# soham97/mellow

Hardware: AMD Instinct MI355X
Metric: audio-pair responses/sec (v0 167M, 2x10s clips, max_len=64, greedy) (higher is better)
Workload: dtype f32 (encoder/prefill GEMM operands split EXACTLY into 3 bf16 terms, 6 bf16 MFMA products per fp32 product, f32 accumulate: fp32-accurate, parity suite green; mel included, the STFT is an fp32 FFT; attentions and decode on exact fp32 MFMA / VALU)

## Files before the change

mellow_amd/csrc/beam.hip:

```cpp
#include "common.h"
#include "kernels.h"

namespace mellow {

namespace {

constexpr int BM_THREADS = 1024, BM_WAVES = BM_THREADS / 64;
constexpr int BM_NV4 = SAMPLE_MAX_V / 4 / BM_THREADS;
static_assert(BM_NV4 * 4 * BM_THREADS == SAMPLE_MAX_V, "row tiling");
static_assert(BEAM_MAX_K * BEAM_MAX_K <= 64, "one wave ranks an example's survivors");

__device__ __forceinline__ int64_t f32_idx(int rb, int K8, int m, int k) {
    return ((int64_t)rb * K8 + (k >> 3)) * 64 + m + 32 * ((k >> 2) & 1);
}

__device__ __forceinline__ uint32_t ckey(float c) {
    if (c != c) return 0xFFFFFFFFu;
    const uint32_t u = __float_as_uint(c);
    return (u & 0x80000000u) ? ~u : (u | 0x80000000u);
}

__device__ __forceinline__ float opaque(float x) {
    asm volatile("" : "+v"(x));
    return x;
}

template <typename T, typename Op>
__device__ __forceinline__ T block_reduce(T v, Op op, T* red) {
    const int tid = threadIdx.x;
#pragma unroll
    for (int off = 32; off > 0; off >>= 1) v = op(v, __shfl_xor(v, off, 64));
    if ((tid & 63) == 0) red[tid >> 6] = v;
    __syncthreads();
    T r = red[0];
    for (int w = 1; w < BM_WAVES; ++w) r = op(r, red[w]);
    __syncthreads();
    return r;
}

__global__ __launch_bounds__(BM_THREADS) void beam_rows_kernel(const BeamArgs g, const int32_t* __restrict__ params) {
    __shared__ float red_f[BM_WAVES];
    __shared__ unsigned long long red_u[BM_WAVES];
    const int r = blockIdx.x, tid = threadIdx.x;
    const float cum = g.cum_in[r];
    float* cc = g.cand_c + (int64_t)r * BEAM_MAX_K;
    float* cl = g.cand_lp + (int64_t)r * BEAM_MAX_K;
    int32_t* ct = g.cand_tok + (int64_t)r * BEAM_MAX_K;
    if (g.fin_in[r] != 0) {
        if (tid == 0) {
            g.cand_n[r] = 1;
            cc[0] = cum + 0.0f; ct[0] = params ? params[1] : g.stop_id; cl[0] = 0.f;
        }
        return;
    }
    const float* __restrict__ lrow = g.logits + (int64_t)r * g.ld;
    float l[BM_NV4][4];
    float m = -INFINITY;
#pragma unroll
    for (int k = 0; k < BM_NV4; ++k) {
        const float4 v = reinterpret_cast<const float4*>(lrow)[k * BM_THREADS + tid];
        l[k][0] = v.x; l[k][1] = v.y; l[k][2] = v.z; l[k][3] = v.w;
#pragma unroll
        for (int j = 0; j < 4; ++j) m = fmaxf(m, l[k][j]);
    }
    const float M = block_reduce(m, [](float a, float b) { return fmaxf(a, b); }, red_f);
    float s = 0.f;
#pragma unroll
    for (int k = 0; k < BM_NV4; ++k)
#pragma unroll
        for (int j = 0; j < 4; ++j) s += expf(l[k][j] - M);
    const float S = block_reduce(s, [](float a, float b) { return a + b; }, red_f);
    const float lse = (M - M == 0.f) ? M + (float)log((double)S) : __builtin_nanf("");
    unsigned long long prev = ~0ull;
    if (tid == 0) g.cand_n[r] = g.k;
#pragma unroll 1
    for (int jr = 0; jr < g.k; ++jr) {
        const uint32_t pkey = (uint32_t)(prev >> 32), pinv = (uint32_t)prev;
        uint32_t bkey = 0u, binv = 0u;
#pragma unroll
        for (int k = 0; k < BM_NV4; ++k)
#pragma unroll
            for (int j = 0; j < 4; ++j) {
                const uint32_t key = ckey(cum + (opaque(l[k][j]) - lse) + 0.0f);
                const uint32_t inv = (uint32_t)(0x7fffffff - (4 * (k * BM_THREADS + tid) + j));
                if ((key < pkey || (key == pkey && inv < pinv)) && (key > bkey || (key == bkey && inv > binv))) { bkey = key; binv = inv; }
            }
        unsigned long long best = ((unsigned long long)bkey << 32) | binv;
        best = block_reduce(best, [](unsigned long long a, unsigned long long b) { return a > b ? a : b; }, red_u);
        if (tid == 0) {
            int idx = 0x7fffffff - (int)(uint32_t)(best & 0xffffffffull);
            idx = min(max(idx, 0), SAMPLE_MAX_V - 1);
            const float lp = lrow[idx] - lse;
            cc[jr] = cum + lp + 0.0f; ct[jr] = idx; cl[jr] = lp;
        }
        prev = best;
    }
}

template <bool LOOP>
__global__ __launch_bounds__(64) void beam_merge_kernel(const BeamArgs g, const DecArgs a, int32_t* __restrict__ tokens,
                                                        const float* __restrict__ embed, const LoopArgs lp) {
    __shared__ int sel_par[BEAM_MAX_K], sel_tok[BEAM_MAX_K];
    __shared__ float sel_c[BEAM_MAX_K], sel_lp[BEAM_MAX_K];
    const int b = blockIdx.x, lane = threadIdx.x, k = g.k;
    const int par = lane / k, slot = lane - par * k;
    bool valid = false;
    float c = 0.f, inc = 0.f;
    int tok = 0;
    if (par < k) {
        const int row = b * k + par;
        valid = slot < g.cand_n[row];
        if (valid) {
            c = g.cand_c[(int64_t)row * BEAM_MAX_K + slot];
            tok = g.cand_tok[(int64_t)row * BEAM_MAX_K + slot];
            inc = g.cand_lp[(int64_t)row * BEAM_MAX_K + slot];
        }
    }
    const uint32_t key = ckey(c);
    int rank = 0;
    for (int t = 0; t < k * k; ++t) {
        const uint32_t ok = __shfl(key, t, 64);
        const int ot = __shfl(tok, t, 64), ov = __shfl((int)valid, t, 64), op = t / k;
        const bool before = ok > key || (ok == key && (op < par || (op == par && ot < tok)));
        rank += (ov && before) ? 1 : 0;
    }
    if (valid && rank < k) { sel_par[rank] = par; sel_tok[rank] = tok; sel_c[rank] = c; sel_lp[rank] = inc; }
    __syncthreads();
    if constexpr (!LOOP) {
        if (lane < k) {
            const int row = b * k + lane;
            g.out_parent[row] = sel_par[lane]; g.out_token[row] = sel_tok[lane]; g.out_cum[row] = sel_c[lane]; g.out_lp[row] = sel_lp[lane];
        }
        return;
    } else {
        const int max_len = lp.params[0], stop_id = lp.params[1];
        const int step = *a.d_pos - lp.T0 + 1;
        int fin = 0;
        if (lane < k) {
            const int row = b * k + lane;
            fin = sel_tok[lane] == stop_id ? 1 : 0;
            g.cum_state[row] = sel_c[lane];
            g.fin_state[row] = fin;
            tokens[row] = min(max(sel_tok[lane], 0), SAMPLE_MAX_V - 1);
            if (step >= 0 && step < max_len) {
                const int64_t o = (int64_t)step * g.N + row;
                g.out_parent[o] = sel_par[lane]; g.out_token[o] = sel_tok[lane]; g.out_lp[o] = sel_lp[lane]; g.out_cum[o] = sel_c[lane];
            }
        }
        const int nfin = __popcll(__ballot(fin));
        if (lane == 0) {
            if (nfin) atomicAdd(lp.n_seen, nfin);
            asm volatile("s_waitcnt vmcnt(0)" ::: "memory");
            if (atomicAdd(lp.arrive, 1) == (int)gridDim.x - 1) {
                *lp.arrive = 0;
                const int t = *lp.ticket + 1;
                *lp.ticket = t;
                const int ns = atomicExch(lp.n_seen, 0);
                __hip_atomic_store(lp.host_progress, ((unsigned long long)(unsigned)t << 32) | (unsigned)ns, __ATOMIC_RELAXED,
                                   __HIP_MEMORY_SCOPE_SYSTEM);
            }
        }
        for (int j = 0; j < k; ++j) {
            const int row = b * k + j, t = min(max(sel_tok[j], 0), SAMPLE_MAX_V - 1);
            for (int i = lane; i < 144; i += 64) {
                const float4 e = reinterpret_cast<const float4*>(embed + (int64_t)t * 576)[i];
                reinterpret_cast<float4*>(a.xmidF)[f32_idx(row >> 5, 72, row & 31, i * 4)] = e;
            }
        }
    }
}

template <bool GATHER>
__global__ __launch_bounds__(256) void beam_kv_move_kernel(float4* __restrict__ kpages, float4* __restrict__ vpages, float4* __restrict__ kst,
                                                           float4* __restrict__ vst, const int32_t* __restrict__ parent_tab,
                                                           const int32_t* __restrict__ d_pos, const int32_t* __restrict__ params, int T0,
                                                           int layers, int N, int k, int Bp, int Tmax) {
    const int max_len = params[0], step = *d_pos - T0 + 1;
    if (step <= 0 || step >= max_len || T0 + step > Tmax) return;
    const int64_t c16 = (int64_t)step * 16, ML16 = (int64_t)max_len * 16, Tmax16 = (int64_t)Tmax * 16;
    const int64_t total = (int64_t)layers * N * 3 * c16;
    const int32_t* __restrict__ par = parent_tab + (int64_t)step * N;
    for (int64_t i = (int64_t)blockIdx.x * 256 + threadIdx.x; i < total; i += (int64_t)gridDim.x * 256) {
        const int64_t pg = i / c16, q = i - pg * c16;
        const int64_t lr = pg / 3, h = pg - lr * 3, l = lr / N;
        const int r = (int)(lr - l * N);
        const int pr = r / k * k + min(max(par[r], 0), k - 1);
        if (pr == r) continue;
        const int64_t st = pg * ML16 + q;
        if constexpr (GATHER) {
            const int64_t src = ((l * Bp + pr) * 3 + h) * Tmax16 + (int64_t)T0 * 16 + q;
            kst[st] = kpages[src];
            vst[st] = vpages[src];
        } else {
            const int64_t dst = ((l * Bp + r) * 3 + h) * Tmax16 + (int64_t)T0 * 16 + q;
            kpages[dst] = kst[st];
            vpages[dst] = vst[st];
        }
    }
}

}

void launch_beam_select(const BeamArgs& g, int B, const DecArgs& a, int32_t* tokens, const float* embed, const LoopArgs* loop, hipStream_t s) {
    if (B <= 0 || g.k < 1 || g.k > BEAM_MAX_K || g.ld != SAMPLE_MAX_V) return;
    hipLaunchKernelGGL(beam_rows_kernel, dim3(B * g.k), dim3(BM_THREADS), 0, s, g, loop ? loop->params : nullptr);
    if (loop) hipLaunchKernelGGL(beam_merge_kernel<true>, dim3(B), dim3(64), 0, s, g, a, tokens, embed, *loop);
    else hipLaunchKernelGGL(beam_merge_kernel<false>, dim3(B), dim3(64), 0, s, g, a, tokens, embed, LoopArgs());
}

void launch_beam_reorder(float* k_pages, float* v_pages, float* k_stage, float* v_stage, const int32_t* parent_tab, const int32_t* d_pos,
                         const int32_t* params, int T0, int layers, int N, int k, int Bp, int Tmax, hipStream_t s) {
    if (layers <= 0 || N <= 0 || k < 2 || N % k != 0 || N > Bp) return;
    constexpr int blocks = 1024;
    hipLaunchKernelGGL(beam_kv_move_kernel<true>, dim3(blocks), dim3(256), 0, s, reinterpret_cast<float4*>(k_pages), reinterpret_cast<float4*>(v_pages),
                       reinterpret_cast<float4*>(k_stage), reinterpret_cast<float4*>(v_stage), parent_tab, d_pos, params, T0, layers, N, k, Bp, Tmax);
    hipLaunchKernelGGL(beam_kv_move_kernel<false>, dim3(blocks), dim3(256), 0, s, reinterpret_cast<float4*>(k_pages), reinterpret_cast<float4*>(v_pages),
                       reinterpret_cast<float4*>(k_stage), reinterpret_cast<float4*>(v_stage), parent_tab, d_pos, params, T0, layers, N, k, Bp, Tmax);
}

}
```

mellow_amd/csrc/build.py:

```python
#!/usr/bin/env python3
from __future__ import annotations

import argparse
import concurrent.futures as cf
import os
import subprocess
import sys

HERE = os.path.dirname(os.path.abspath(__file__))
PKG = os.path.dirname(HERE)
LIBDIR = os.path.join(PKG, "lib")
OBJDIR = os.path.join(HERE, "build")
LIB = os.path.join(LIBDIR, "libmellow_hip.so")
SOURCES = ["gemm_f32.hip", "gemm_fp8.hip", "gemm_bf16x3.hip", "decode.hip", "prefill_attn.hip", "encoder.hip", "stft_fft.hip", "sample.hip", "score.hip", "beam.hip", "logit_rules.hip", "guidance.hip", "engine.cpp", "engine_weights.cpp", "engine_encoder.cpp", "engine_lm.cpp", "engine_generate.cpp", "engine_dev.cpp"]
HEADERS = ["common.h", "kernels.h", "gemm_epilogue.h", "prefill_attn_f32.inc", "engine_internal.h", os.path.join("..", "..", "include", "mellow_hip.h")]
ARCH = "gfx950"
FLAGS = (["-DMELLOW_KDEBUG"] if os.environ.get("MELLOW_KDEBUG") else []) + os.environ.get("MELLOW_EXTRA_FLAGS", "").split() + ["-O3", "-std=c++17", "-fPIC", "-fvisibility=hidden", f"--offload-arch={ARCH}", "-Wall", "-Wno-unused-function",
         "-Wno-unused-variable", "-x", "hip"]


def _hipcc():
    for c in (os.environ.get("HIPCC"), "/opt/rocm/bin/hipcc", "hipcc"):
        if c and (os.path.isabs(c) and os.path.exists(c) or not os.path.isabs(c)):
            return c
    raise RuntimeError("hipcc not found")


def _stale(target, deps):
    if not os.path.exists(target):
        return True
    t = os.path.getmtime(target)
    return any(os.path.getmtime(d) > t for d in deps)


VGPR_FORM = ["-mllvm", "-amdgpu-mfma-vgpr-form=1"]
FILE_FLAGS = {name: VGPR_FORM for name in os.environ.get("MELLOW_VGPR_FORM_FILES", "gemm_bf16x3.hip gemm_fp8.hip prefill_attn.hip encoder.hip").split()}
KERNARG_PRELOAD = [] if os.environ.get("MELLOW_KERNARG_PRELOAD", "14") == "0" else ["-mllvm", "-amdgpu-kernarg-preload-count=" + os.environ.get("MELLOW_KERNARG_PRELOAD", "14")]
FILE_FLAGS["decode.hip"] = FILE_FLAGS.get("decode.hip", []) + KERNARG_PRELOAD


def build(force=False, verbose=False, out=None, objdir=None):
    lib = os.path.abspath(out) if out else LIB
    objdir = os.path.abspath(objdir) if objdir else OBJDIR
    os.makedirs(os.path.dirname(lib), exist_ok=True)
    os.makedirs(objdir, exist_ok=True)
    hipcc = _hipcc()
    hdrs = [os.path.join(HERE, h) for h in HEADERS] + [os.path.abspath(__file__)]
    jobs = []
    objs = []
    for src in SOURCES:
        sp = os.path.join(HERE, src)
        op = os.path.join(objdir, src + ".o")
        objs.append(op)
        if force or _stale(op, [sp] + hdrs):
            jobs.append((sp, op))

    def cc(job):
        sp, op = job
        cmd = [hipcc] + FLAGS + FILE_FLAGS.get(os.path.basename(sp), []) + ["-c", sp, "-o", op]
        if verbose:
            print(" ".join(cmd), flush=True)
        r = subprocess.run(cmd, capture_output=True, text=True)
        return sp, r

    with cf.ThreadPoolExecutor(max_workers=max(1, min(len(jobs), os.cpu_count() or 1))) as ex:
        for sp, r in ex.map(cc, jobs):
            if r.returncode != 0:
                sys.stderr.write(r.stdout + r.stderr)
                raise RuntimeError(f"hipcc failed on {sp}")
            if verbose and r.stderr.strip():
                sys.stderr.write(r.stderr)
    if force or jobs or _stale(lib, objs):
        cmd = [hipcc, "-shared", "-fPIC", f"--offload-arch={ARCH}", "-o", lib] + objs
        if verbose:
            print(" ".join(cmd), flush=True)
        r = subprocess.run(cmd, capture_output=True, text=True)
        if r.returncode != 0:
            sys.stderr.write(r.stdout + r.stderr)
            raise RuntimeError("link failed")
    return lib


if __name__ == "__main__":
    ap = argparse.ArgumentParser()
    ap.add_argument("--force", action="store_true")
    ap.add_argument("--verbose", action="store_true")
    ap.add_argument("--out", metavar="PATH", help="write the library here instead of mellow_amd/lib/libmellow_hip.so")
    ap.add_argument("--objdir", metavar="DIR", help="object cache of this build instead of mellow_amd/csrc/build/")
    a = ap.parse_args()
    print(build(a.force, a.verbose, a.out, a.objdir))
```

mellow_amd/csrc/decode.hip:

```cpp
#include "common.h"
#include "kernels.h"
#include <cstdio>
#include <mutex>
#include <set>
#include <type_traits>
#include <utility>

namespace mellow {

__device__ uint64_t* g_kdbg = nullptr;
#ifdef MELLOW_KDEBUG
__device__ __forceinline__ void kstamp(int slot, int idx, bool who) {
    if (g_kdbg && who) g_kdbg[slot * 8 + idx] = __builtin_readcyclecounter();
}
__device__ __forceinline__ void kspan(int seq, int end) {
    if (g_kdbg && seq >= 0 && seq < 480 && threadIdx.x == 0) {
        const unsigned long long t = wall_clock64();
        if (end) atomicMax(reinterpret_cast<unsigned long long*>(g_kdbg) + 64 + 2 * seq + 1, t);
        else atomicMin(reinterpret_cast<unsigned long long*>(g_kdbg) + 64 + 2 * seq, t);
    }
}
#else
#define kstamp(slot, idx, who) ((void)0)
#define kspan(seq, end) ((void)0)
#endif
void set_kernel_debug_buffer(uint64_t* p) { (void)hipMemcpyToSymbol(HIP_SYMBOL(g_kdbg), &p, sizeof(p)); }

__device__ __forceinline__ float fast_exp(float x) { return __builtin_amdgcn_exp2f(x * 1.44269504088896340736f); }
#ifdef MELLOW_NO_BLK_EXIT
#define MELLOW_BLK_EXIT(RB)
#else
#define MELLOW_BLK_EXIT(RB) if (BLK) { if (a.blk_live[RB] == 0) return; }
#endif
__device__ __forceinline__ float4 ldg_nt(const float4* p) {
#ifdef MELLOW_NO_NT
    return *p;
#else
    const f32x4 v = __builtin_nontemporal_load(reinterpret_cast<const f32x4*>(p));
    return make_float4(v[0], v[1], v[2], v[3]);
#endif
}
template <bool W8>
__device__ __forceinline__ float4 ldw(const float* __restrict__ Wp, int64_t slot) {
    if constexpr (W8) {
        const uint32_t u = __builtin_nontemporal_load(reinterpret_cast<const uint32_t*>(Wp) + slot);
        const auto lo = __builtin_amdgcn_cvt_pk_f32_fp8(u, false), hi = __builtin_amdgcn_cvt_pk_f32_fp8(u, true);
        return make_float4(lo[0], lo[1], hi[0], hi[1]);
    } else {
        return ldg_nt(reinterpret_cast<const float4*>(Wp) + slot);
    }
}
__device__ __forceinline__ uint32_t ldw8(const float* __restrict__ Wp, int64_t slot) {
    return __builtin_nontemporal_load(reinterpret_cast<const uint32_t*>(Wp) + slot);
}
__device__ __forceinline__ float f4amax(float4 v) { return fmaxf(fmaxf(fabsf(v.x), fabsf(v.y)), fmaxf(fabsf(v.z), fabsf(v.w))); }
__device__ __forceinline__ uint32_t q4_e4m3(float4 v, float inv) {
    int w = 0;
    w = __builtin_amdgcn_cvt_pk_fp8_f32(v.x * inv, v.y * inv, w, false);
    w = __builtin_amdgcn_cvt_pk_fp8_f32(v.z * inv, v.w * inv, w, true);
    return (uint32_t)w;
}
__device__ __forceinline__ long pk64(uint32_t lo, uint32_t hi) { return (long)(((uint64_t)hi << 32) | (uint64_t)lo); }
template <int N>
__device__ __forceinline__ f32x16 mfma8_32(f32x16 acc, const uint32_t (&w)[N], const uint32_t (&x)[N]) {
#pragma unroll
    for (int i = 0; i < N; i += 2)
        acc = __builtin_amdgcn_mfma_f32_32x32x16_fp8_fp8(pk64(w[i], i + 1 < N ? w[i + 1] : 0u), pk64(x[i], i + 1 < N ? x[i + 1] : 0u), acc, 0, 0, 0);
    return acc;
}
template <int N>
__device__ __forceinline__ f32x4 mfma8_16(f32x4 acc, const uint32_t (&w)[N], const uint32_t (&x)[N]) {
#pragma unroll
    for (int i = 0; i < N; i += 2)
        acc = __builtin_amdgcn_mfma_f32_16x16x32_fp8_fp8(pk64(w[i], i + 1 < N ? w[i + 1] : 0u), pk64(x[i], i + 1 < N ? x[i + 1] : 0u), acc, 0, 0, 0);
    return acc;
}
__device__ __forceinline__ void a8_scales(float amax, float& inv, float& sc) {
    inv = amax > 0.f ? 448.0f / amax : 0.f;
    sc = amax * (1.0f / 448.0f);
}
#ifndef MELLOW_ST_MODE
#define MELLOW_ST_MODE 0
#endif
__device__ __forceinline__ void st_out(float4* p, float4 v) {
// ... 149 lines not shown
        }
        if (nt == 0) {
            ssp = half_sum(ssp);
            if (lane < 32) ssq_s[wave * 32 + lane] = ssp;
        }
#pragma unroll
        for (int r = 0; r < 16; ++r) red[(wave * 16 + r) * 64 + lane] = acc[r];
    }
    __syncthreads();
    if (nt == 0 && tid < 32)
    {
        float ssum = ssq_s[tid & 31];
#pragma unroll
        for (int wv = 1; wv < QW; ++wv) ssum += ssq_s[wv * 32 + (tid & 31)];
        a.ssq1[((int64_t)rb * 32 + tid) * DEC_KC_QKV + kc] = ssum;
    }
    if (tid >= 256) return;
    const int mm = tid & 31, hh = (tid >> 5) & 1, gq = tid >> 6;
    float v[4];
#pragma unroll
    for (int j = 0; j < 4; ++j) {
        const int r = 4 * gq + j;
        float sacc = red[r * 64 + mm + 32 * hh];
#pragma unroll
        for (int wv = 1; wv < QW; ++wv) sacc += red[(wv * 16 + r) * 64 + mm + 32 * hh];
        v[j] = sacc;
    }
    const int n = nt * 32 + 8 * gq + 4 * hh;
    if (W8) {
#pragma unroll
        for (int j = 0; j < 4; ++j) v[j] *= wscale[n + j];
    }
    if (n < 960)
        *reinterpret_cast<float4*>(a.pq + ((int64_t)kc * a.rows + rb * 32 + mm) * 960 + n) = make_float4(v[0], v[1], v[2], v[3]);
    kspan(a.dbg_seq, 1);
}

#ifndef MELLOW_DA_ABL
#define MELLOW_DA_ABL 0
#endif
#ifndef MELLOW_DA_WAVES
#define MELLOW_DA_WAVES 8
#define MELLOW_DA_G 7
#endif
#ifndef MELLOW_DA_MINW
#define MELLOW_DA_MINW 4
#endif
constexpr int DA_MINW = MELLOW_DA_WAVES == 8 || MELLOW_DA_WAVES == 4 ? MELLOW_DA_MINW : 1;
constexpr int DA_WAVES = MELLOW_DA_WAVES;
constexpr int DA_G = MELLOW_DA_G;
#ifndef MELLOW_DA_G1
#define MELLOW_DA_G1 5
#endif
constexpr int DA_G1 = MELLOW_DA_G1 < DA_G ? MELLOW_DA_G1 : DA_G;
#ifndef MELLOW_DA16_MFMA
#define MELLOW_DA16_MFMA 1
#endif
constexpr int DA_GM = 8;
#ifndef MELLOW_DA16_KNT
#define MELLOW_DA16_KNT 0
#endif
#ifndef MELLOW_DA16_MINW
#define MELLOW_DA16_MINW MELLOW_DA_MINW
#endif
#ifndef MELLOW_DA16_NW
#define MELLOW_DA16_NW 8
#endif

template <bool KV16>
__device__ __forceinline__ float4 ld_kv(const float* page, int64_t elem) {
    if constexpr (KV16) {
        typedef unsigned u32x2 __attribute__((ext_vector_type(2)));
        const u32x2 r = __builtin_nontemporal_load(reinterpret_cast<const u32x2*>(reinterpret_cast<const uint16_t*>(page) + elem));
        return make_float4(__uint_as_float(r[0] << 16), __uint_as_float(r[0] & 0xffff0000u), __uint_as_float(r[1] << 16), __uint_as_float(r[1] & 0xffff0000u));
    } else {
        return ldg_nt(reinterpret_cast<const float4*>(page + elem));
    }
}
template <bool KV16>
__device__ __forceinline__ void st_kv(float* page, int64_t elem, float v) {
    if constexpr (KV16) reinterpret_cast<__bf16*>(page)[elem] = static_cast<__bf16>(v);
    else page[elem] = v;
}
template <bool BLK, bool FUSED, bool ONE, bool KV16, int NW, int TS>
__global__ __launch_bounds__(NW * 64, ONE ? 2 : (KV16 && MELLOW_DA16_MFMA && DA_MINW > 1 ? MELLOW_DA16_MINW : DA_MINW)) void dec_attn_kernel(float* __restrict__ k_cache, float* __restrict__ v_cache,
                                                                  const int32_t* __restrict__ d_pos_p, const float* __restrict__ pq_p,
                                                                  const float* __restrict__ xmidF_p, int Tmax_p, int gs_p, int rows_p,
                                                                  const DecArgs a) {
    kspan(a.dbg_seq, 0);
    __shared__ float ssq_part[3];
    __shared__ __attribute__((aligned(16))) float qs[3 * 64];
    __shared__ __attribute__((aligned(16))) float knew[64], vnew[64];
    __shared__ __attribute__((aligned(16))) float xs[320];
    __shared__ __attribute__((aligned(16))) float ored[DA_WAVES * 3 * 64];
    __shared__ float mred[DA_WAVES * 3], lred[DA_WAVES * 3];
    __shared__ float snew_s[3];
    constexpr bool MF = KV16 && MELLOW_DA16_MFMA != 0;
    __shared__ __attribute__((aligned(16))) float pl[MF ? DA_WAVES * 32 * 4 : 4];
    __shared__ __attribute__((aligned(16))) __bf16 qb[MF ? 10 * 64 : 8];
    constexpr int VPW = DA_WAVES / NW;
    static_assert(DA_WAVES % NW == 0 && (MF || NW == DA_WAVES), "the vector form runs one chunk stream per wave");
    auto mf_group = [&](int g0, int u) { return g0 + u * DA_WAVES; };

    static_assert(TS == DEC_TS || !(ONE || KV16), "one row block and the bf16 pages always run DEC_TS key splits (kernels.h dec_key_splits)");
    const int g = blockIdx.x, b = blockIdx.y, sp = blockIdx.z;
    int row = b;
    if (BLK) {
        const int live = a.blk_live[b >> 5];
        if (a.row_of_slot) row = a.row_of_slot[b];
        if (live == 0 || row < 0) return;
    }
    const int tid = threadIdx.x, lane = tid & 63, wave = tid >> 6;
    const int Tmax = Tmax_p;
    float* kpage = k_cache + (((int64_t)row * 3 + g) * Tmax * 64 >> (KV16 ? 1 : 0));
    float* vpage = v_cache + (((int64_t)row * 3 + g) * Tmax * 64 >> (KV16 ? 1 : 0));
    const int sub = lane >> 4, quad = lane & 15;

    const bool dbg = tid == 0 && g == 0 && b == 0 && sp == 0;
    kstamp(1, 0, dbg);
#ifdef MELLOW_POS_VECTOR_LOAD
    const int pos = __builtin_amdgcn_readfirstlane(*reinterpret_cast<const volatile int*>(d_pos_p));
#else
    const int pos = *d_pos_p;
#endif
    const int hsel = (tid >> 5) & 3, i = tid & 31;
    const int r = tid < 80 ? tid : 0;
    const int pcol = r < 48 ? (3 * g + (r >> 4)) * 64 + 4 * (r & 15) : r < 64 ? 576 + g * 64 + 4 * (r - 48) : 768 + g * 64 + 4 * (r - 64);
    const float* prow = pq_p + (int64_t)b * 960 + pcol;
    constexpr int NPQ = FUSED ? Q2_NPQ : DEC_KC_QKV;
    float4 sl4[NPQ], sq4[2];
    if (tid < 80) {
#pragma unroll
        for (int s = 0; s < NPQ; ++s)
            sl4[s] = (MELLOW_DA_ABL & 4) ? make_float4(0.1f * s, 0.2f, 0.3f, 0.4f) : *reinterpret_cast<const float4*>(prow + (int64_t)s * rows_p * 960);
        if (!FUSED) {
            sq4[0] = reinterpret_cast<const float4*>(a.ssq1 + (int64_t)b * DEC_KC_QKV)[0];
            sq4[1] = reinterpret_cast<const float4*>(a.ssq1 + (int64_t)b * DEC_KC_QKV)[1];
        }
    }
    float4 xr4 = make_float4(0.f, 0.f, 0.f, 0.f), xd4[FUSED ? Q2_HC : 1];
    if (FUSED && tid < 144) {
        const int64_t fi = ((int64_t)(b >> 5) * 72 + (tid >> 1)) * 64 + (b & 31) + 32 * (tid & 1);
        xr4 = reinterpret_cast<const float4*>(xmidF_p)[fi];
#pragma unroll
        for (int s = 0; s < Q2_HC; ++s) xd4[s] = reinterpret_cast<const float4*>(a.dslabF)[(int64_t)s * a.slabF_stride4 + fi];
    }
    const float c = a.rope_cur[i], sn = a.rope_cur[32 + i];
    const int gbeg = sp * gs_p;
    const int gend_fixed = sp == TS - 1 ? 0x3fffffff : gbeg + gs_p;
    typedef unsigned u32x2 __attribute__((ext_vector_type(2)));
    const int kk = lane & 31, hf = lane >> 5;
    i32x4 kq[4];
    u32x2 vq[DA_GM];
    auto load_ktile = [&](int g0) {
        const int gi = g0 + (kk >> 2) * DA_WAVES;
        const int tc = min(gi * 4 + (kk & 3), Tmax - 1);
        const i32x4* kp = reinterpret_cast<const i32x4*>(reinterpret_cast<const uint16_t*>(kpage) + (int64_t)tc * 64 + hf * 32);
#pragma unroll
        for (int st = 0; st < 4; ++st)
            kq[st] = (MELLOW_DA_ABL & 1) ? i32x4{tc, 0x3c003c00, st, 0x3c003c00} : (MELLOW_DA16_KNT ? __builtin_nontemporal_load(kp + st) : kp[st]);
    };
    auto load_vgroup = [&](int g0, int u) {
        const int gi = mf_group(g0, u);
        const int tc = min(gi * 4 + sub, Tmax - 1);
        vq[u] = (MELLOW_DA_ABL & 1) ? u32x2{0x3c003c00u, (unsigned)tc}
                                    : __builtin_nontemporal_load(reinterpret_cast<const u32x2*>(reinterpret_cast<const uint16_t*>(vpage) + (int64_t)tc * 64 + quad * 4));
    };
    float4 k4[MF ? 1 : DA_G], v4[MF ? 1 : DA_G];
    auto load_group = [&](int u) {
        const int gi = gbeg + wave + u * DA_WAVES;
        const int tc = min(gi * 4 + sub, Tmax - 1);
        if (MELLOW_DA_ABL & 1) {
            k4[u] = make_float4(0.01f * tc, 0.02f, 0.03f, 0.04f);
            v4[u] = make_float4(0.01f, 0.02f * tc, 0.03f, 0.04f);
        } else {
            k4[u] = ld_kv<KV16>(kpage, (int64_t)tc * 64 + quad * 4);
            v4[u] = ld_kv<KV16>(vpage, (int64_t)tc * 64 + quad * 4);
        }
    };
    const int g_first_mf = gbeg + wave;
    if constexpr (MF) {
        load_ktile(g_first_mf);
#pragma unroll
        for (int u = 0; u < DA_GM / 2; ++u) load_vgroup(g_first_mf, u);
    } else {
#pragma unroll
        for (int u = 0; u < DA_G1; ++u) load_group(u);
    }
    MELLOW_HOIST(a.attF16); MELLOW_HOIST(a.att_ml); MELLOW_HOIST(a.RB); MELLOW_HOIST(a.eps);
    if (FUSED) MELLOW_HOIST(a.xnewR);
    __builtin_amdgcn_sched_barrier(0);
    kstamp(1, 1, dbg);

    const int ngroups = (pos + 3) >> 2;
    const int gend = min(ngroups, gend_fixed);
    static_assert(DEC_KC_QKV == 8, "fixed summation order below");
    if (FUSED) {
        if (tid < 192) {
            float4 x = xr4;
#pragma unroll
            for (int s = 0; s < Q2_HC; ++s) x = f4add(x, xd4[s]);
            const float ss = wave_sum(tid < 144 ? f4ssq(x) : 0.f);
            if (lane == 0) ssq_part[wave] = ss;
            if (g == 0 && sp == 0 && tid < 144) reinterpret_cast<float4*>(a.xnewR + (int64_t)b * 576)[tid] = x;
        }
        if (tid < 80) {
            float4 x = sl4[0];
#pragma unroll
            for (int s = 1; s < NPQ; ++s) x = f4add(x, sl4[s]);
            *reinterpret_cast<float4*>(xs + 4 * tid) = x;
        }
    } else if (tid < 80) {
        float4 x = sl4[0];
#pragma unroll
        for (int s = 1; s < DEC_KC_QKV; ++s) x = f4add(x, sl4[s]);
        const float ssum = ((sq4[0].x + sq4[0].y) + (sq4[0].z + sq4[0].w)) + ((sq4[1].x + sq4[1].y) + (sq4[1].z + sq4[1].w));
        const float rscale = 1.0f / sqrtf(ssum / 576.0f + a.eps);
        *reinterpret_cast<float4*>(xs + 4 * tid) = make_float4(x.x * rscale, x.y * rscale, x.z * rscale, x.w * rscale);
    }
    __syncthreads();
    kstamp(1, 2, dbg);
    const float rs2 = FUSED ? 1.0f / sqrtf(((ssq_part[0] + ssq_part[1]) + ssq_part[2]) / 576.0f + a.eps) : 1.0f;
    if (tid < 128) {
        const int base = hsel < 3 ? hsel * 64 : 192;
        const float x1 = xs[base + i] * rs2, x2 = xs[base + i + 32] * rs2;
        const float o1 = __fadd_rn(__fmul_rn(x1, c), __fmul_rn(-x2, sn));
        const float o2 = __fadd_rn(__fmul_rn(x2, c), __fmul_rn(x1, sn));
        if (hsel < 3) {
            qs[hsel * 64 + i] = o1 * 0.125f;
            qs[hsel * 64 + i + 32] = o2 * 0.125f;
            if constexpr (MF) {
                __bf16 p0, p1, p2;
                split3(o1 * 0.125f, p0, p1, p2);
                qb[(0 * 3 + hsel) * 64 + i] = p0; qb[(1 * 3 + hsel) * 64 + i] = p1; qb[(2 * 3 + hsel) * 64 + i] = p2;
                split3(o2 * 0.125f, p0, p1, p2);
                qb[(0 * 3 + hsel) * 64 + i + 32] = p0; qb[(1 * 3 + hsel) * 64 + i + 32] = p1; qb[(2 * 3 + hsel) * 64 + i + 32] = p2;
            }
        } else {
            knew[i] = o1; knew[i + 32] = o2;
            if (sp == 0) { st_kv<KV16>(kpage, (int64_t)pos * 64 + i, o1); st_kv<KV16>(kpage, (int64_t)pos * 64 + i + 32, o2); }
        }
    } else if (tid < 192) {
        const float x1 = xs[256 + tid - 128] * rs2;
        vnew[tid - 128] = x1;
        if (sp == 0) st_kv<KV16>(vpage, (int64_t)pos * 64 + (tid - 128), x1);
    } else if (MF && tid < 256) {
        qb[9 * 64 + tid - 192] = static_cast<__bf16>(0.f);
    }
    __syncthreads();
    __builtin_amdgcn_sched_barrier(0);
    if constexpr (MF) {
#pragma unroll
        for (int u = DA_GM / 2; u < DA_GM; ++u) load_vgroup(g_first_mf, u);
    } else {
#pragma unroll
        for (int u = DA_G1; u < DA_G; ++u) load_group(u);
    }
    __builtin_amdgcn_sched_barrier(0);
    kstamp(1, 3, dbg);

    if (wave < 3) {
        const float sn_ = wave_sum(qs[wave * 64 + lane] * knew[lane]);
        if (lane == 0) snew_s[wave] = sn_;
    }
    float4 q4[3];
    const int aq_off = ((kk >> 2) < 3 && (kk & 3) < 3 ? (kk >> 2) * 3 + (kk & 3) : 9) * 64 + hf * 32;
    if constexpr (!MF) {
#pragma unroll
        for (int hh = 0; hh < 3; ++hh) q4[hh] = *reinterpret_cast<const float4*>(qs + hh * 64 + quad * 4);
    }
    float m_run[3] = {-INFINITY, -INFINITY, -INFINITY};
    float l_run[3] = {0.f, 0.f, 0.f};
    float4 acc[3];
#pragma unroll
    for (int hh = 0; hh < 3; ++hh) acc[hh] = make_float4(0.f, 0.f, 0.f, 0.f);

#define MELLOW_DA_CHUNK(g0)                                                                                              \
    {                                                                                                                    \
        float sc[DA_G][3];                                                                                               \
        float cmax[3] = {-INFINITY, -INFINITY, -INFINITY};                                                               \
_Pragma("unroll")                                                                                                        \
        for (int u = 0; u < DA_G; ++u) {                                                                                 \
            const int gi = g0 + u * DA_WAVES;                                                                            \
            const int t = gi * 4 + sub;                                                                                  \
            const bool ok = gi < gend && t < pos;                                                                        \
_Pragma("unroll")                                                                                                        \
            for (int hh = 0; hh < 3; ++hh) {                                                                             \
                float sv = q4[hh].x * k4[u].x + q4[hh].y * k4[u].y + q4[hh].z * k4[u].z + q4[hh].w * k4[u].w;            \
                sv = row16_sum(sv);                                                                                      \
                sv = ok ? sv : -INFINITY;                                                                                \
                sc[u][hh] = sv;                                                                                          \
                cmax[hh] = fmaxf(cmax[hh], sv);                                                                          \
            }                                                                                                            \
        }                                                                                                                \
_Pragma("unroll")                                                                                                        \
        for (int hh = 0; hh < 3; ++hh) {                                                                                 \
            float cm = cmax[hh];                                                                                         \
            cm = fmaxf(cm, swz_xor16(cm));                                                                               \
            cm = half_max(cm);                                                                                           \
// ... 1111 lines not shown
        kstamp(7, 2, dbg && acc[0] == acc[0]);
        if (side) nt -= 30;
    }
#pragma unroll
    for (int r = 0; r < 16; ++r) red[(wave * 16 + r) * 64 + lane] = acc[r];
    __syncthreads();
    kstamp(7, 3, dbg);
    if (tid < 256) {
        const int mm = tid & 31, hh = (tid >> 5) & 1, gq = tid >> 6;
        float v[4];
#pragma unroll
        for (int j = 0; j < 4; ++j) {
            const int q = 4 * gq + j;
            float sacc = red[q * 64 + mm + 32 * hh];
#pragma unroll
            for (int wv = 1; wv < Q2W; ++wv) sacc += red[(wv * 16 + q) * 64 + mm + 32 * hh];
            v[j] = sacc;
        }
        const int n = nt * 32 + 8 * gq + 4 * hh;
        if (W8) {
#pragma unroll
            for (int j = 0; j < 4; ++j) v[j] *= wsc[n + j];
        }
        const float4 o = make_float4(v[0], v[1], v[2], v[3]);
        if (side) st_out(reinterpret_cast<float4*>(a.dslabF) + (int64_t)slab * a.slabF_stride4 + f32_idx(rb, 72, mm, n), o);
        else st_out(reinterpret_cast<float4*>(a.pq + ((int64_t)slab * a.rows + rb * 32 + mm) * 960 + n), o);
    }
    kstamp(7, 4, dbg);
    kspan(a.dbg_seq, 1);
}

template <int KCD, bool BLK>
__global__ __launch_bounds__(192) void dec_final_norm_kernel(const float* __restrict__ norm_w, const float* __restrict__ xmidF_p,
                                                             const float* __restrict__ dslabF_p, int64_t stride4_p, const DecArgs a) {
    kspan(a.dbg_seq, 0);
    __shared__ float part[3];
    const int b = blockIdx.x, tid = threadIdx.x;
    if (BLK && b == 0 && tid < 32) a.blk_snap[tid] = a.blk_live[tid];
    MELLOW_BLK_EXIT(b >> 5)
    const int xi = tid < 144 ? tid : 0;
    const int64_t fi = f32_idx(b >> 5, 72, b & 31, xi * 4);
    float4 v = reinterpret_cast<const float4*>(xmidF_p)[fi];
    float4 xs[KCD > 0 ? KCD : 1];
#pragma unroll
    for (int s = 0; s < KCD; ++s) xs[s] = reinterpret_cast<const float4*>(dslabF_p)[(int64_t)s * stride4_p + fi];
    const float4 wv = reinterpret_cast<const float4*>(norm_w)[xi];
#pragma unroll
    for (int s = 0; s < KCD; ++s) v = f4add(v, xs[s]);
    float ss = tid < 144 ? f4ssq(v) : 0.f;
    ss = wave_sum(ss);
    if ((tid & 63) == 0) part[tid >> 6] = ss;
    __syncthreads();
    const float r = 1.0f / sqrtf((part[0] + part[1] + part[2]) / 576.0f + a.eps);
    if (tid < 144) {
        float4 y;
        y.x = __fmul_rn(wv.x, __fmul_rn(v.x, r)); y.y = __fmul_rn(wv.y, __fmul_rn(v.y, r));
        y.z = __fmul_rn(wv.z, __fmul_rn(v.z, r)); y.w = __fmul_rn(wv.w, __fmul_rn(v.w, r));
        if (!a.xn3) reinterpret_cast<float4*>(a.xnF)[fi] = y;
    }
    if (a.xn3) {
        float4 y = make_float4(0.f, 0.f, 0.f, 0.f);
        if (tid < 144) {
            y.x = __fmul_rn(wv.x, __fmul_rn(v.x, r)); y.y = __fmul_rn(wv.y, __fmul_rn(v.y, r));
            y.z = __fmul_rn(wv.z, __fmul_rn(v.z, r)); y.w = __fmul_rn(wv.w, __fmul_rn(v.w, r));
        }
        const F3Quad mine = f3_split4(y), other = f3_partner(mine);
        if (tid < 144 && !(tid & 1)) f3_store8(a.xn3, f3_32_slot(b >> 5, 36, b & 31, tid * 4), mine, other);
    }
    kspan(a.dbg_seq, 1);
}

template <bool LSE>
__global__ __launch_bounds__(256) void dec_argmax_kernel(const float* __restrict__ cand_val_p, const int32_t* __restrict__ cand_idx_p, int n,
                                                         const DecArgs a, int32_t* __restrict__ tokens,
                                                         const float* __restrict__ embed, int write_x, const LoopArgs lp) {
    kspan(a.dbg_seq, 0);
    __shared__ float bv[4];
    __shared__ int bi[4];
    __shared__ int tok_s;
    __shared__ float lse_sh[4];
    const int b = blockIdx.x, tid = threadIdx.x;
    const int row = lp.row_of_slot ? lp.row_of_slot[b] : b;
    const bool dead = (lp.blk_snap && lp.blk_snap[b >> 5] == 0) || row < 0;
    float best = -INFINITY;
    int idx = 0x7fffffff;
    if (!dead) {
        for (int i = tid; i < n; i += 256) {
            const float v = cand_val_p[(int64_t)b * n + i];
            const int id = cand_idx_p[(int64_t)b * n + i];
            if (arg_better(v, id, best, idx)) { best = v; idx = id; }
        }
#pragma unroll
        for (int off = 32; off > 0; off >>= 1) {
            const float ov = __shfl_xor(best, off, 64);
            const int oi = __shfl_xor(idx, off, 64);
            if (arg_better(ov, oi, best, idx)) { best = ov; idx = oi; }
        }
        if ((tid & 63) == 0) { bv[tid >> 6] = best; bi[tid >> 6] = idx; }
    }
    __syncthreads();
    float S = 0.f;
    if constexpr (LSE) {
        if (!dead) {
            float M = bv[0];
            int mi = bi[0];
            for (int w = 1; w < 4; ++w)
                if (arg_better(bv[w], bi[w], M, mi)) { M = bv[w]; mi = bi[w]; }
            S = dec_lse_sum(cand_val_p + (int64_t)b * n, a.cand_sum + (int64_t)b * n, n, M, lse_sh);
            S = (M - M == 0.f) ? S : __builtin_nanf("");
        }
    }
    if (tid == 0) {
        if (!dead) {
            for (int w = 1; w < 4; ++w)
                if (arg_better(bv[w], bi[w], best, idx)) { best = bv[w]; idx = bi[w]; }
            idx = min(max(idx, 0), n * 32 - 1);
            tokens[b] = idx;
            tok_s = idx;
        }
        if (lp.out_tokens) {
            if (!dead) {
                const int max_len = lp.params[0], stop_id = lp.params[1];
                const int step = *a.d_pos - lp.T0 + 1;
                if (step >= 0 && step < max_len) lp.out_tokens[(int64_t)row * max_len + step] = idx;
                if constexpr (LSE) {
                    if (step >= 0 && step < max_len) lp.out_logprob[(int64_t)row * max_len + step] = -dec_lse_log(S);
                }
                if (idx == stop_id && lp.seen_stop[row] == 0) {
                    lp.seen_stop[row] = 1;
                    atomicAdd(lp.n_seen, 1);
                    if (lp.blk_left && atomicSub(lp.blk_left + (b >> 5), 1) == 1) lp.blk_live[b >> 5] = 0;
                }
            }
            asm volatile("s_waitcnt vmcnt(0)" ::: "memory");
            if (atomicAdd(lp.arrive, 1) == (int)gridDim.x - 1) {
                *lp.arrive = 0;
                const int t = *lp.ticket + 1;
                *lp.ticket = t;
                const int ns = atomicAdd(lp.n_seen, 0);
                __hip_atomic_store(lp.host_progress, ((unsigned long long)(unsigned)t << 32) | (unsigned)ns, __ATOMIC_RELAXED,
                                   __HIP_MEMORY_SCOPE_SYSTEM);
            }
        }
    }
    if (dead) return;
    if (write_x) {
        __syncthreads();
        if (tid < 144) {
            const float4 e = reinterpret_cast<const float4*>(embed + (int64_t)tok_s * 576)[tid];
            reinterpret_cast<float4*>(a.xmidF)[f32_idx(b >> 5, 72, b & 31, tid * 4)] = e;
        }
    }
    kspan(a.dbg_seq, 1);
}

__global__ __launch_bounds__(256) void dec_lse_tap_kernel(const float* __restrict__ cand_val_p, const float* __restrict__ cand_sum_p, int n,
                                                          float* __restrict__ out_lse, float* __restrict__ out_max) {
    __shared__ float sh[4];
    const int b = blockIdx.x;
    const float M = dec_lse_max(cand_val_p + (int64_t)b * n, n, sh);
    const float S = dec_lse_sum(cand_val_p + (int64_t)b * n, cand_sum_p + (int64_t)b * n, n, M, sh);
    if (threadIdx.x == 0) {
        out_lse[b] = dec_lse_value(M, S);
        out_max[b] = M;
    }
}

__global__ __launch_bounds__(1024) void dec_compact_kernel(const DecArgs a, int B, const LoopArgs lp) {
    __shared__ int src_of[1024];
    __shared__ int row_new[1024];
    __shared__ int wsum[16];
    __shared__ int n_act_s, n_live_s;
    const int tid = threadIdx.x, lane = tid & 63, wave = tid >> 6;
    const int nblk = (B + 31) >> 5;
    int row = -1, active = 0;
    if (tid < B) {
        row = lp.row_of_slot[tid];
        active = row >= 0 && lp.blk_live[tid >> 5] != 0 && lp.seen_stop[row] == 0;
    }
    const unsigned long long m = __ballot(active);
    const int before = __popcll(m & ((1ull << lane) - 1ull));
    if (lane == 0) wsum[wave] = __popcll(m);
    if (tid == 0) {
        int live = 0;
        for (int k = 0; k < nblk; ++k) live += lp.blk_live[k] != 0;
        n_live_s = live;
    }
    src_of[tid] = -1;
    row_new[tid] = -1;
    __syncthreads();
    int base = 0;
    for (int w = 0; w < wave; ++w) base += wsum[w];
    if (tid == 0) {
        int n = 0;
        for (int w = 0; w < 16; ++w) n += wsum[w];
        n_act_s = n;
    }
    __syncthreads();
    const int n_act = n_act_s;
    if ((n_act + 31) / 32 >= n_live_s) return;
    if (active) { src_of[base + before] = tid; row_new[base + before] = row; }
    __syncthreads();
    float4* x = reinterpret_cast<float4*>(a.xmidF);
    for (int d0 = 0; d0 < n_act; d0 += 7) {
        const int d = d0 + tid / 144, c = tid % 144;
        const bool mv = tid < 1008 && d < n_act && src_of[d] != d;
        float4 v = make_float4(0.f, 0.f, 0.f, 0.f);
        if (mv) v = x[f32_idx(src_of[d] >> 5, 72, src_of[d] & 31, c * 4)];
        __syncthreads();
        if (mv) x[f32_idx(d >> 5, 72, d & 31, c * 4)] = v;
        __syncthreads();
    }
    if (tid < B) lp.row_of_slot[tid] = row_new[tid];
    if (tid < 32) {
        const int left = tid < nblk ? min(max(n_act - 32 * tid, 0), 32) : 0;
        lp.blk_left[tid] = left;
        lp.blk_live[tid] = left > 0;
    }
    if (tid == 0) *lp.n_compactions += 1;
}
__global__ __launch_bounds__(256) void kv_to_bf16_kernel(const float4* __restrict__ src, uint4* __restrict__ dst, int64_t n8) {
    for (int64_t i = (int64_t)blockIdx.x * 256 + threadIdx.x; i < n8; i += (int64_t)gridDim.x * 256) {
        const float4 a = src[2 * i], b = src[2 * i + 1];
        typedef __bf16 bf16x8v __attribute__((ext_vector_type(8)));
        const bf16x8v o = {static_cast<__bf16>(a.x), static_cast<__bf16>(a.y), static_cast<__bf16>(a.z), static_cast<__bf16>(a.w),
                           static_cast<__bf16>(b.x), static_cast<__bf16>(b.y), static_cast<__bf16>(b.z), static_cast<__bf16>(b.w)};
        dst[i] = __builtin_bit_cast(uint4, o);
    }
}
void launch_kv_to_bf16(const float* src, void* dst, int64_t n, hipStream_t s) {
    const int64_t n8 = n >> 3;
    const int blocks = (int)((n8 + 255) / 256 < 8192 ? (n8 + 255) / 256 : 8192);
    hipLaunchKernelGGL(kv_to_bf16_kernel, dim3(blocks), dim3(256), 0, s, reinterpret_cast<const float4*>(src), reinterpret_cast<uint4*>(dst), n8);
}
__global__ __launch_bounds__(256) void kv_fanout_kernel(const float4* __restrict__ ksrc, const float4* __restrict__ vsrc,
                                                        float4* __restrict__ kdst, float4* __restrict__ vdst, int64_t total,
                                                        int B, int n, int Bp, int T16, int64_t Tp16, int64_t Tmax16) {
    for (int64_t i = (int64_t)blockIdx.x * 256 + threadIdx.x; i < total; i += (int64_t)gridDim.x * 256) {
        const int64_t pg = i / T16, q = i - pg * T16;
        const int64_t lb = pg / 3, h = pg - lb * 3, l = lb / B, b = lb - l * B;
        const float4 k = ksrc[pg * Tp16 + q], v = vsrc[pg * Tp16 + q];
        int64_t d = ((l * Bp + b * n) * 3 + h) * Tmax16 + q;
        for (int j = 0; j < n; ++j, d += 3 * Tmax16) {
            kdst[d] = k;
            vdst[d] = v;
        }
    }
}
void launch_kv_fanout(const float* k_prefix, const float* v_prefix, float* k_pages, float* v_pages, int layers, int B, int n, int Bp,
                      int T, int Tp, int Tmax, hipStream_t s) {
    if (layers <= 0 || B <= 0 || n <= 0 || T <= 0 || T > Tp || T > Tmax || (int64_t)B * n > Bp) return;
    const int64_t total = (int64_t)layers * B * 3 * T * 16;
    const int blocks = (int)((total + 255) / 256 < 2048 ? (total + 255) / 256 : 2048);
    hipLaunchKernelGGL(kv_fanout_kernel, dim3(blocks), dim3(256), 0, s, reinterpret_cast<const float4*>(k_prefix),
                       reinterpret_cast<const float4*>(v_prefix), reinterpret_cast<float4*>(k_pages), reinterpret_cast<float4*>(v_pages),
                       total, B, n, Bp, T * 16, (int64_t)Tp * 16, (int64_t)Tmax * 16);
}
void launch_dec_compact(const DecArgs& a, int B, const LoopArgs& loop, hipStream_t s) {
    hipLaunchKernelGGL(dec_compact_kernel, dim3(1), dim3(1024), 0, s, a, B, loop);
}

__global__ __launch_bounds__(192) void dec_load_rows_kernel(const DecArgs a, const float* __restrict__ in, int64_t ld,
                                                            const int32_t* __restrict__ row_ids, int T_last, int n_src) {
    const int b = blockIdx.x, tid = threadIdx.x;
    const int64_t src = row_ids ? (int64_t)min(max(row_ids[b], 0), n_src - 1) : (int64_t)b * T_last + (T_last - 1);
    if (tid < 144) {
        const float4 e = reinterpret_cast<const float4*>(in + src * ld)[tid];
        reinterpret_cast<float4*>(a.xmidF)[f32_idx(b >> 5, 72, b & 31, tid * 4)] = e;
    }
}

void set_max_dynamic_lds(const void* fn, size_t bytes) {
    if (bytes <= 64 * 1024) return;
    static std::mutex mu;
    static std::set<std::pair<const void*, int>> done;
    int dev = 0;
    (void)hipGetDevice(&dev);
    std::lock_guard<std::mutex> lk(mu);
    if (done.insert({fn, dev}).second) {
        const hipError_t e = hipFuncSetAttribute(fn, hipFuncAttributeMaxDynamicSharedMemorySize, (int)bytes);
        if (e != hipSuccess) fprintf(stderr, "mellow: hipFuncSetAttribute(max dynamic LDS %zu) failed: %s\n", bytes, hipGetErrorString(e));
    }
}
template <class F> static inline void with_bool(bool v, F&& f) {
    if (v) f(std::true_type{}); else f(std::false_type{});
}
template <int V0, int... Vs, class F> static inline void with_int(int v, F&& f) {
    if constexpr (sizeof...(Vs) == 0) f(std::integral_constant<int, V0>{});
    else if (v == V0) f(std::integral_constant<int, V0>{});
    else with_int<Vs...>(v, f);
}
static inline int w8_mode(const DecArgs& a, const float* wscale) { return wscale ? (a.a8 ? 2 : 1) : 0; }
template <class F> static inline void with_blk_w8(const DecArgs& a, const float* wscale, F&& f) {
    with_bool(a.blk_live != nullptr, [&](auto blk) { with_int<2, 1, 0>(w8_mode(a, wscale), [&](auto w8) { f(blk, w8); }); });
}
void launch_dec_qkv(const DecArgs& a, const float* Wp, int K8p, int kcd, hipStream_t s, const float* wscale) {
    const dim3 grid(30, DEC_KC_QKV, a.RB);
    with_int<0, DEC_KC_DOWN>(kcd, [&](auto kcd_c) { with_bool(a.first != 0, [&](auto first) { with_blk_w8(a, wscale, [&](auto blk, auto w8) {
        hipLaunchKernelGGL((dec_qkv_kernel<kcd_c.value, blk.value, first.value, w8.value>), grid, dim3(QKV_THREADS), 0, s, Wp, (const float*)a.xmidF,
                           (const float*)a.dslabF, K8p, a, wscale);
    }); }); });
}
void launch_dec_attn(const DecArgs& a, float* k_cache, float* v_cache, bool fused, hipStream_t s) {
    const dim3 grid(3, a.rows, a.ts);
    const bool one = a.RB == 1 && !a.blk_live;
    if (a.ts != DEC_TS && (one || a.kv16 || a.ts != DEC_TS_MULTI)) {
        fprintf(stderr, "mellow: decode attention launched with %d key splits at RB = %d\n", a.ts, a.RB);
        abort();
    }
    auto launch = [&](auto blk, auto one_c) { with_bool(fused, [&](auto fused_c) { with_bool(a.kv16 != 0, [&](auto kv16) {
        constexpr bool ONE = one_c.value, KV16 = kv16.value;
        constexpr int NW = !KV16 ? DA_WAVES : MELLOW_DA16_MFMA && DA_WAVES == 8 && !ONE ? MELLOW_DA16_NW : DA_WAVES;
        constexpr int TSM = ONE || KV16 ? DEC_TS : DEC_TS_MULTI;
        with_int<DEC_TS, TSM>(a.ts, [&](auto ts) {
            hipLaunchKernelGGL((dec_attn_kernel<blk.value, fused_c.value, ONE, KV16, NW, ts.value>), grid, dim3(NW * 64), 0, s, k_cache, v_cache,
                               (const int32_t*)a.d_pos, (const float*)a.pq, (const float*)a.xmidF, a.Tmax, a.gs, a.rows, a);
        });
    }); }); };
    if (one) launch(std::false_type{}, std::true_type{});
    else with_bool(a.blk_live != nullptr, [&](auto blk) { launch(blk, std::false_type{}); });
}
static void launch_dec_qkv2_any(const DecArgs& a, const float* Wx, int K8x, const float* Wh, int K8h, const float* Wd,
                                const float* sc_x, const float* sc_h, const float* sc_d, hipStream_t s) {
    const dim3 grid(Q2_BLOCKS, a.RB);
#ifdef MELLOW_Q2_WAVES_FORCED
    bool few = false;
#else
    bool few = a.RB == 1;
#endif
    if (w8_mode(a, sc_x) == 2) few = false;
    with_bool(few, [&](auto few_c) { with_blk_w8(a, sc_x, [&](auto blk, auto w8) {
        constexpr int WV = few_c.value ? 4 : Q2_WAVES;
        hipLaunchKernelGGL((dec_qkv2_kernel<blk.value, WV, w8.value>), grid, dim3(WV * 64), 0, s, Wx, Wh, Wd, (const float*)a.xmidF,
                           (const float*)a.guF, K8x, K8h, a, sc_x, sc_h, sc_d);
    }); });
}
constexpr size_t dec_qkv2x3_lds(int rbm) { return (size_t)Q3W * rbm * 16 * 64 * 4; }
constexpr size_t dec_gateup3_lds(int rbm) { return (size_t)GU3W * rbm * 8 * 64 * 4; }
constexpr size_t dec_head3r_lds() { return (size_t)36 * 3 * 64 * 16; }
template <class F> static inline void with_qkv2x3(int rb, bool blk, F&& f) {
    with_int<1, 2, 4>(rb, [&](auto rbm) { with_bool(blk, [&](auto b) { f(&dec_qkv2x3_kernel<b.value, rbm.value>, dec_qkv2x3_lds(rbm.value)); }); });
}
template <class F> static inline void with_gateup3(int rb, bool blk, F&& f) {
    with_int<1, 2, 4>(rb, [&](auto rbm) { with_bool(blk, [&](auto b) { f(&dec_gateup3_kernel<b.value, rbm.value>, dec_gateup3_lds(rbm.value)); }); });
}
template <class F> static inline void with_head3r(int rb, bool blk, bool lse, F&& f) {
    with_int<1, 2, 4>(rb, [&](auto g) { with_bool(blk, [&](auto b) { with_bool(lse, [&](auto l) {
        constexpr int G = g.value, D = G == 1 ? MELLOW_H3R_D1 : G == 2 ? MELLOW_H3R_D2 : MELLOW_H3R_D4;
        f(&dec_head3r_kernel<G, D, b.value, l.value>, dec_head3r_lds());
    }); }); });
}
void launch_dec_qkv2x3(const DecArgs& a, const float* Wq2, const float* Wd, hipStream_t s) {
    const float* Wh = Wq2 + (size_t)72 * 64 * 4;
    const i32x4 *x3 = reinterpret_cast<const i32x4*>(a.xmid3_32), *h3 = reinterpret_cast<const i32x4*>(a.h3);
    with_qkv2x3(a.RB, a.blk_live != nullptr, [&](auto* kernel, size_t lds) {
        set_max_dynamic_lds(reinterpret_cast<const void*>(kernel), lds);
        hipLaunchKernelGGL(kernel, dim3(Q2_BLOCKS), dim3(Q3W * 64), lds, s, Wq2, Wh, Wd, x3, h3, Q2_K8, Q2_K8, a.RB, a);
    });
}
void launch_dec_gateup3(const DecArgs& a, const float* Wp16, hipStream_t s) {
    const i32x4* x3 = reinterpret_cast<const i32x4*>(a.xmid3_16);
    with_gateup3(a.RB, a.blk_live != nullptr, [&](auto* kernel, size_t lds) {
        set_max_dynamic_lds(reinterpret_cast<const void*>(kernel), lds);
        hipLaunchKernelGGL(kernel, dim3(192), dim3(GU3W * 64), lds, s, Wp16, x3, (const float*)a.ssq, a.RB, a);
    });
}
void launch_dec_qkv2(const DecArgs& a, const float* Wq2, const float* Wd, hipStream_t s) {
    launch_dec_qkv2_any(a, Wq2, Q2_K8, Wq2 + (size_t)72 * 64 * 4, Q2_K8, Wd, nullptr, nullptr, nullptr, s);
}
void launch_dec_qkv2_w8(const DecArgs& a, const float* Wx8, const float* sc_x, const float* Wh8, const float* sc_h,
                        const float* Wd8, const float* sc_d, hipStream_t s) {
    launch_dec_qkv2_any(a, Wx8, 72, Wh8, 192, Wd8, sc_x, sc_h, sc_d, s);
}
__global__ __launch_bounds__(256) void compose_f64_kernel(const float* __restrict__ A, const float* __restrict__ B, float* __restrict__ C,
                                                          int M, int N, int K) {
    __shared__ double as[16][17], bs[16][17];
    const int tx = threadIdx.x & 15, ty = threadIdx.x >> 4;
    const int m = blockIdx.y * 16 + ty, n = blockIdx.x * 16 + tx;
    double acc = 0.0;
    for (int k0 = 0; k0 < K; k0 += 16) {
        as[ty][tx] = (m < M && k0 + tx < K) ? (double)A[(int64_t)m * K + k0 + tx] : 0.0;
        bs[ty][tx] = (k0 + ty < K && n < N) ? (double)B[(int64_t)(k0 + ty) * N + n] : 0.0;
        __syncthreads();
#pragma unroll
        for (int kk = 0; kk < 16; ++kk) acc += as[ty][kk] * bs[kk][tx];
        __syncthreads();
    }
    if (m < M && n < N) C[(int64_t)m * N + n] = (float)acc;
}
void launch_compose_f64(const float* A, const float* B, float* C, int M, int N, int K, hipStream_t s) {
    hipLaunchKernelGGL(compose_f64_kernel, dim3((N + 15) / 16, (M + 15) / 16), dim3(256), 0, s, A, B, C, M, N, K);
}
int dec_attn_chunk_groups(bool kv16) { return DA_WAVES * (kv16 && MELLOW_DA16_MFMA ? DA_GM : DA_G); }
void launch_dec_oproj(const DecArgs& a, const float* Wp16, hipStream_t s, const float* wscale) {
#ifdef MELLOW_OPROJ_ROWS
    const int rows = MELLOW_OPROJ_ROWS;
#else
// ... 10 lines not shown
        hipLaunchKernelGGL((dec_gateup16_kernel<blk.value, w8.value>), dim3(192, a.RB), dim3(GU_WAVES * 64), 0, s, Wp16, a.xmidF16, a.ssq, a, wscale);
    });
}
void launch_dec_down(const DecArgs& a, const float* Wp, int K8p, hipStream_t s, const float* wscale) {
    with_blk_w8(a, wscale, [&](auto blk, auto w8) {
        hipLaunchKernelGGL((dec_down_kernel<blk.value, w8.value>), dim3(18, DEC_KC_DOWN, a.RB), dim3(DN_WAVES * 64), 0, s, Wp, (const float*)a.guF,
                           K8p, a, wscale);
    });
}
void launch_dec_final_norm(const DecArgs& a, const float* norm_w, int kcd, hipStream_t s) {
    with_int<0, DEC_KC_DOWN>(kcd, [&](auto kcd_c) { with_bool(a.blk_live != nullptr, [&](auto blk) {
        hipLaunchKernelGGL((dec_final_norm_kernel<kcd_c.value, blk.value>), dim3(a.rows), dim3(192), 0, s, norm_w, (const float*)a.xmidF,
                           (const float*)a.dslabF, a.slabF_stride4, a);
    }); });
}
bool dec_head3r_fits(int vocab) { return vocab % 32 == 0 && (vocab / 32) % H3_NW == 0; }
void launch_dec_lm_head(const DecArgs& a, const float* Wp, int K8p, int vocab, hipStream_t s, const float* wscale) {
    if ((a.x3 & DEC_X3_HEAD) && !wscale && a.xn3 && (vocab / 32) % H3_NW == 0) {
        const i32x4* X3 = reinterpret_cast<const i32x4*>(a.xn3);
        with_head3r(a.RB, a.blk_live != nullptr, a.cand_sum != nullptr, [&](auto* kernel, size_t lds) {
            set_max_dynamic_lds(reinterpret_cast<const void*>(kernel), lds);
            hipLaunchKernelGGL(kernel, dim3(vocab / 32 / H3_NW), dim3(H3_NW * 64), lds, s, Wp, X3, K8p, vocab, a.RB, a);
        });
        return;
    }
    with_blk_w8(a, wscale, [&](auto blk, auto w8) { with_bool(a.cand_sum != nullptr, [&](auto lse) {
        hipLaunchKernelGGL((dec_fullk_kernel<OUT_LOGITS, blk.value, w8.value, lse.value>), dim3(vocab / 32, 1, a.RB), dim3(LM_WAVES * 64), 0, s, Wp,
                           (const float*)a.xnF, K8p, vocab, a, wscale);
    }); });
}
void dec_prepare_lds_attributes() {
    const auto raise = [](auto* kernel, size_t lds) { set_max_dynamic_lds(reinterpret_cast<const void*>(kernel), lds); };
    for (const int rb : {1, 2, 4})
        for (const bool blk : {false, true}) {
            for (const bool lse : {false, true}) with_head3r(rb, blk, lse, raise);
            with_qkv2x3(rb, blk, raise);
            with_gateup3(rb, blk, raise);
        }
}
__global__ __launch_bounds__(256) void pack_dec_fp8_kernel(const float4* __restrict__ Wp, int slots, int rows, uint32_t* __restrict__ out,
                                                           float* __restrict__ scale) {
    __shared__ unsigned amax_s[32];
    __shared__ float inv_s[32];
    const int tile = blockIdx.x, tid = threadIdx.x;
    if (tid < 32) amax_s[tid] = 0u;
    __syncthreads();
    const float4* src = Wp + (int64_t)tile * slots;
    for (int i = tid; i < slots; i += 256) {
        const float4 v = src[i];
        const float m = fmaxf(fmaxf(fabsf(v.x), fabsf(v.y)), fmaxf(fabsf(v.z), fabsf(v.w)));
        atomicMax(&amax_s[(i & 63) & (rows - 1)], __float_as_uint(m));
    }
    __syncthreads();
    if (tid < rows) {
        const float am = __uint_as_float(amax_s[tid]);
        const float sc = am > 0.f ? am / 448.0f : 1.0f;
        scale[(int64_t)tile * rows + tid] = sc;
        inv_s[tid] = 1.0f / sc;
    }
    __syncthreads();
    for (int i = tid; i < slots; i += 256) {
        const float4 v = src[i];
        const float inv = inv_s[(i & 63) & (rows - 1)];
        int w = 0;
        w = __builtin_amdgcn_cvt_pk_fp8_f32(v.x * inv, v.y * inv, w, false);
        w = __builtin_amdgcn_cvt_pk_fp8_f32(v.z * inv, v.w * inv, w, true);
        out[(int64_t)tile * slots + i] = (uint32_t)w;
    }
}
void launch_pack_dec_fp8(const float* Wp, int tiles, int slots_per_tile, int rows_per_tile, void* out, float* scale, hipStream_t s) {
    hipLaunchKernelGGL(pack_dec_fp8_kernel, dim3(tiles), dim3(256), 0, s, reinterpret_cast<const float4*>(Wp), slots_per_tile,
                       rows_per_tile, reinterpret_cast<uint32_t*>(out), scale);
}
void launch_dec_argmax(const DecArgs& a, int B, int n_tiles, int32_t* tokens, const float* embed, int write_x,
                       const LoopArgs& loop, hipStream_t s) {
    with_bool(loop.out_logprob != nullptr && a.cand_sum != nullptr, [&](auto lse) {
        hipLaunchKernelGGL(dec_argmax_kernel<lse.value>, dim3(B), dim3(256), 0, s, (const float*)a.cand_val, (const int32_t*)a.cand_idx, n_tiles, a,
                           tokens, embed, write_x, loop);
    });
}
void launch_dec_lse_tap(const DecArgs& a, int B, int n_tiles, float* out_lse, float* out_max, hipStream_t s) {
    hipLaunchKernelGGL(dec_lse_tap_kernel, dim3(B), dim3(256), 0, s, (const float*)a.cand_val, (const float*)a.cand_sum, n_tiles, out_lse, out_max);
}
void launch_dec_load_rows(const DecArgs& a, int B, const float* in, int64_t ld, const int32_t* row_ids, int T_last,
                          int n_src, hipStream_t s) {
    hipLaunchKernelGGL(dec_load_rows_kernel, dim3(B), dim3(192), 0, s, a, in, ld, row_ids, T_last, n_src);
}

__global__ __launch_bounds__(1024) void argmax_kernel(const float* __restrict__ logits, int V, int64_t ld,
                                                      int32_t* __restrict__ tokens) {
    __shared__ float bv[16];
    __shared__ int bi[16];
    const int b = blockIdx.x, tid = threadIdx.x;
    const float4* row = reinterpret_cast<const float4*>(logits + (int64_t)b * ld);
    float best = -INFINITY;
    int idx = 0x7fffffff;
    for (int i = tid; i < (V >> 2); i += 1024) {
        const float4 v = row[i];
        const float vv[4] = {v.x, v.y, v.z, v.w};
#pragma unroll
        for (int j = 0; j < 4; ++j)
            if (arg_better(vv[j], 4 * i + j, best, idx)) { best = vv[j]; idx = 4 * i + j; }
    }
#pragma unroll
    for (int off = 32; off > 0; off >>= 1) {
        const float ov = __shfl_xor(best, off, 64);
        const int oi = __shfl_xor(idx, off, 64);
        if (arg_better(ov, oi, best, idx)) { best = ov; idx = oi; }
    }
    if ((tid & 63) == 0) { bv[tid >> 6] = best; bi[tid >> 6] = idx; }
    __syncthreads();
    if (tid == 0) {
        for (int w = 1; w < 16; ++w)
            if (arg_better(bv[w], bi[w], best, idx)) { best = bv[w]; idx = bi[w]; }
        tokens[b] = min(max(idx, 0), V - 1);
    }
}
void launch_argmax(const float* logits, int B, int V, int64_t ld, int32_t* tokens, hipStream_t s) {
    hipLaunchKernelGGL(argmax_kernel, dim3(B), dim3(1024), 0, s, logits, V, ld, tokens);
}

__global__ void pack_weight16_kernel(const float* __restrict__ w, int N, int K, float* __restrict__ out) {
    const int64_t total = (int64_t)(N / 16) * (K / 16) * 64;
    for (int64_t i = (int64_t)blockIdx.x * blockDim.x + threadIdx.x; i < total; i += (int64_t)gridDim.x * blockDim.x) {
        const int lane = (int)(i & 63);
        const int64_t tile = i >> 6;
        const int k16 = (int)(tile % (K / 16)), nt = (int)(tile / (K / 16));
        const int n = nt * 16 + (lane & 15), k0 = k16 * 16 + 4 * (lane >> 4);
        reinterpret_cast<float4*>(out)[i] = *reinterpret_cast<const float4*>(w + (int64_t)n * K + k0);
    }
}
__global__ void pack_weight16n_kernel(const float* __restrict__ w, int N, int K, float* __restrict__ out) {
    const int64_t total = (int64_t)(N / 16) * (K / 32) * 128;
    for (int64_t i = (int64_t)blockIdx.x * blockDim.x + threadIdx.x; i < total; i += (int64_t)gridDim.x * blockDim.x) {
        const int lane = (int)(i & 63), half = (int)((i >> 6) & 1);
        const int64_t tile = i >> 7;
        const int T = (int)(tile % (K / 32)), nt = (int)(tile / (K / 32));
        const int n = nt * 16 + (lane & 15), k0 = T * 32 + 8 * (lane >> 4) + 4 * half;
        reinterpret_cast<float4*>(out)[i] = *reinterpret_cast<const float4*>(w + (int64_t)n * K + k0);
    }
}
void launch_pack_weight16n(const float* w, int N, int K, float* out, hipStream_t s) {
    const int64_t total = (int64_t)(N / 16) * (K / 32) * 128;
    const int blocks = (int)((total + 255) / 256 < 4096 ? (total + 255) / 256 : 4096);
    hipLaunchKernelGGL(pack_weight16n_kernel, dim3(blocks), dim3(256), 0, s, w, N, K, out);
}
void launch_pack_weight16(const float* w, int N, int K, float* out, hipStream_t s) {
    const int64_t total = (int64_t)(N / 16) * (K / 16) * 64;
    const int blocks = (int)((total + 255) / 256 < 4096 ? (total + 255) / 256 : 4096);
    hipLaunchKernelGGL(pack_weight16_kernel, dim3(blocks), dim3(256), 0, s, w, N, K, out);
}

}
```

mellow_amd/csrc/engine.cpp:

```cpp
#include "engine_internal.h"

static thread_local std::string g_err;
int fail(const char* fmt, ...) {
    char buf[1024];
    va_list ap;
    va_start(ap, fmt);
    vsnprintf(buf, sizeof(buf), fmt, ap);
    va_end(ap);
    g_err = buf;
    return 1;
}
int ensure(mellow_engine* e, mellow_engine::Buf& b, size_t floats) {
    if (b.cap >= floats) return 0;
    if (b.p) HIPCHK(hipFree(b.p));
    b.p = nullptr;
    b.cap = 0;
    HIPCHK(hipMalloc(&b.p, floats * sizeof(float)));
    b.cap = floats;
    return 0;
}
int dev_alloc(mellow_engine* e, float** out, size_t floats) {
    const size_t bytes = (floats * sizeof(float) + 4095) / 4096 * 4096;
    if (!e->arena) {
        const size_t want = (size_t)(e->opt.arena_mb < 0 ? 0 : e->opt.arena_mb) << 20;
// ... 248 lines not shown

}

int alloc_state_words(mellow_engine* e) {
    HIPCHK(hipMalloc(&e->d_tokens, 4096 * sizeof(int32_t)));
    HIPCHK(hipMemset(e->d_tokens, 0, 4096 * sizeof(int32_t)));
    e->d_step = e->d_tokens + 1024;
    e->d_pos = e->d_tokens + 1025;
    e->d_nseen = e->d_tokens + 1026;
    e->d_arrive = e->d_tokens + 1027;
    e->d_ticket = e->d_tokens + 1028;
    e->d_params = e->d_tokens + 1032;
    e->d_sparams = reinterpret_cast<uint32_t*>(e->d_tokens + 1536);
    e->d_rparams = reinterpret_cast<uint32_t*>(e->d_tokens + 1552);
    e->d_gparams = reinterpret_cast<uint32_t*>(e->d_tokens + 1560);
    e->d_blk_left = e->d_tokens + 1040;
    e->d_blk_live = e->d_tokens + 1072;
    e->d_seen = e->d_tokens + 2048;
    e->d_row_of_slot = e->d_tokens + 3072;
    e->d_ncompact = e->d_tokens + 1029;
    HIPCHK(hipHostMalloc(reinterpret_cast<void**>(&e->h_progress), 64, hipHostMallocMapped | hipHostMallocCoherent));
    *e->h_progress = 0;
    HIPCHK(hipHostGetDevicePointer(reinterpret_cast<void**>(&e->d_progress), e->h_progress, 0));
    return 0;
}

__global__ void stream_probe_kernel(unsigned long long* out, unsigned long long ticks) {
    const unsigned long long t0 = wall_clock64();
    out[0] = t0;
    while (wall_clock64() - t0 < ticks) __builtin_amdgcn_s_sleep(8);
    out[1] = wall_clock64();
}
static int streams_overlap(mellow_engine* e, hipStream_t a, hipStream_t b, bool* yes) {
    unsigned long long* d = nullptr;
    HIPCHK(hipMalloc(&d, 4 * sizeof(unsigned long long)));
    HIPCHK(hipMemsetAsync(d, 0, 4 * sizeof(unsigned long long), a));
    HIPCHK(hipStreamSynchronize(a));
    HIPCHK(hipStreamSynchronize(b));
    hipLaunchKernelGGL(stream_probe_kernel, dim3(1), dim3(1), 0, a, d, 20000ull);
    hipLaunchKernelGGL(stream_probe_kernel, dim3(1), dim3(1), 0, b, d + 2, 2000ull);
    HIPCHK(hipStreamSynchronize(a));
    HIPCHK(hipStreamSynchronize(b));
    unsigned long long h[4];
    HIPCHK(hipMemcpy(h, d, sizeof(h), hipMemcpyDeviceToHost));
    HIPCHK(hipFree(d));
    *yes = h[2] < h[1];
    return 0;
}
int ensure_prefill_streams(mellow_engine* e) {
    if (e->n_forks > 0 || e->parent) return 0;
    if (e->streams_probed) {
        if (++e->probe_backoff < 16) { e->prefill_parts = e->prefill_parts_ok; return 0; }
        e->streams_probed = false;
        e->probe_backoff = 0;
        e->prefill_parts = e->prefill_parts_want;
    }
    int nh = e->prefill_parts < 1 ? 1 : (e->prefill_parts > 4 ? 4 : e->prefill_parts);
    for (int h = 1; h < nh; ++h) {
        if (e->stream2[h - 1]) continue;
        bool ok = false;
        for (int attempt = 0; attempt < 8 && !ok; ++attempt) {
            hipStream_t st = nullptr;
            HIPCHK(hipStreamCreateWithFlags(&st, hipStreamNonBlocking));
            int rc = streams_overlap(e, e->stream, st, &ok);
            for (int k = 1; k < h && ok && !rc; ++k) rc = streams_overlap(e, e->stream2[k - 1], st, &ok);
            if (rc) { hipStreamDestroy(st); return rc; }
            if (ok) e->stream2[h - 1] = st; else hipStreamDestroy(st);
        }
        if (!ok) {
            e->prefill_parts_want = e->prefill_parts;
            e->prefill_parts = e->prefill_parts_ok = h;
            e->streams_probed = true;
            break;
        }
    }
    return 0;
}
struct OptDesc { const char* key; const char* dflt; bool answers; const char* what; };
static const OptDesc kOptions[] = {
    {"prefill_split", "2", false, "f32x3: parts of the split LM prefill (1..4); bit-identical for every value"},
    {"prefill_fuse_norm", "1", true, "f32x3: norm-free LM prefill (GEMM epilogues emit split output + RMS partials); 0 = a normalisation launch per GEMM input"},
    {"decode_fuse", "1", true, "down projection of layer l fused with q/k/v of layer l + 1 through the load-time product W'Wd; 0 = five launches per layer"},
    {"decode_fuse_max_rb", "1", true, "largest number of 32-row blocks that runs the fused down + q/k/v launch on fp32 weights"},
    {"splitk", "8", true, "f32x3 encoder: largest split count of the split-K launches (0 = never split; a summation order)"},
    {"enc_apb", "0x1CC", false, "f32x3 encoder: Swin stages whose producers hand over pre-split (bit st, 4 + st, 8 + st); bit-identical"},
    {"graph", "1", false, "decode steps as hipGraph replays (0 = eager launches)"},
    {"fp8_decode", "1", true, "fp8 mode: e4m3 weights in the decode kernels"},
    {"fp8_prefill", "1", true, "fp8 mode: e4m3 GEMMs in encoder + LM prefill"},
    {"fp8_decode_act", "1", true, "fp8 mode: e4m3 activations in the decode GEMM kernels (fp8 matrix pipe)"},
    {"fp8_kv16", "1", true, "fp8 mode: bf16 shadow of the K/V pages for the decode step"},
    {"fp8_attn_bf16", "1", true, "fp8 mode: q / k / v stored once as bf16 (LM: bf16 K/V pages + bf16-once prefill attention; Swin: bf16 q/k/v rows into the exact window attention); 0 = fp32 q/k/v, the 3-way split attention"},
    {"decode_x3", "7", true, "f32x3: mask of decode GEMM launches on the bf16 pipe (1 lm_head, 2 gate/up, 4 fused down + q/k/v)"},
    {"decode_x3_min_rb", "2", true, "f32x3: fewest 32-row blocks at which the layer launches take their f32x3 forms"},
    {"x3_stft", "1", true, "f32x3: STFT / mel GEMMs on the split kernel (0 = exact fp32 kernel)"},
    {"stft_fft", "1", true, "f32x3: STFT as a 1024-point FFT when the checkpoint's conv weights are the windowed DFT basis"},
    {"x3_apb", "1", true, "f32x3 LM prefill: producers hand over pre-split, GEMMs staged by LDS-DMA (0 = register-staged kernel on fp32 activations)"},
    {"x3_attn", "1", true, "f32x3: prefill attention on exact bf16 splits (0 = exact fp32 MFMA kernel)"},
    {"x3w", "1", false, "f32x3: K = 96 GEMMs on the weight-stationary persistent kernel; bit-identical"},
    {"row_migration", "1", false, "reference-semantics loop, B > 32: rows still running are packed into the lowest 32-row blocks; tokens unchanged"},
    {"arena_mb", "3400", false, "size of the weight arena in MiB (before the first tensor is loaded)"},
};
static const OptDesc* find_opt(const char* key) {
    for (const auto& o : kOptions)
        if (!strcmp(o.key, key)) return &o;
    return nullptr;
}
static long opt_val(const mellow_engine* e, const char* key) {
    auto it = e->opt.given.find(key);
    return strtol(it != e->opt.given.end() ? it->second.c_str() : find_opt(key)->dflt, nullptr, 0);
}
int apply_options(mellow_engine* e) {
    const int mode = e->opt.mode;
    e->prefill_parts = (int)opt_val(e, "prefill_split");
    e->opt.prefill_fuse_norm = opt_val(e, "prefill_fuse_norm") != 0;
    e->opt.decode_fuse = opt_val(e, "decode_fuse") != 0;
    e->opt.dec_fuse_max_rb = (int)opt_val(e, "decode_fuse_max_rb");
    e->opt.sk_max = (int)opt_val(e, "splitk");
    e->opt.enc_apb_stages = (int)opt_val(e, "enc_apb");
    e->use_graph = opt_val(e, "graph") != 0;
    e->opt.x3_stft = opt_val(e, "x3_stft") != 0;
    e->opt.stft_fft = opt_val(e, "stft_fft") != 0 && e->opt.x3_stft;
    e->opt.x3_apb = opt_val(e, "x3_apb") != 0;
    e->opt.x3_attn = opt_val(e, "x3_attn") != 0;
    e->opt.x3w = opt_val(e, "x3w") != 0;
    e->opt.row_migration = opt_val(e, "row_migration") != 0;
    e->opt.arena_mb = (int)opt_val(e, "arena_mb");
    e->opt.fp8 = mode == MELLOW_PRECISION_FP8;
    e->opt.fp8_decode = e->opt.fp8 && opt_val(e, "fp8_decode") != 0;
    e->opt.fp8_decode_act = e->opt.fp8_decode && opt_val(e, "fp8_decode_act") != 0;
    e->opt.fp8_prefill = opt_val(e, "fp8_prefill") != 0;
    e->opt.fp8_attn_bf16 = opt_val(e, "fp8_attn_bf16") != 0;
    e->opt.kv16 = e->opt.fp8_decode && opt_val(e, "fp8_kv16") != 0;
    e->opt.f32x3_terms = mode == MELLOW_PRECISION_F32X3 ? 6 : 0;
    e->opt.dec_x3 = mode == MELLOW_PRECISION_F32X3 ? ((int)opt_val(e, "decode_x3") & DEC_X3_ALL) : 0;
    e->opt.dec_x3_min_rb = (int)opt_val(e, "decode_x3_min_rb") < 1 ? 1 : (int)opt_val(e, "decode_x3_min_rb");
    return 0;
}

extern "C" {

int mellow_engine_set_option(mellow_engine_t* e, const char* key, const char* value) {
    if (!e || !key || !value) return fail("null argument");
    if (e->finalized) return fail("options must be set before mellow_engine_finalize");
    const OptDesc* o = find_opt(key);
    if (!o) return fail("unknown option \"%s\" (mellow_engine_describe lists them)", key);
    char* end = nullptr;
    const long v = strtol(value, &end, 0);
    if (end == value || *end) return fail("option \"%s\": \"%s\" is not an integer", key, value);
    if (!strcmp(key, "prefill_split") && (v < 1 || v > 4)) return fail("option prefill_split must be 1..4");
    if (!strcmp(key, "arena_mb") && e->arena) return fail("option arena_mb must be set before the first tensor is loaded");
    e->opt.given[key] = value;
    return apply_options(e);
}

int64_t mellow_engine_describe(mellow_engine_t* e, char* buf, int64_t capacity) {
    if (!e) return -1;
    std::string s = "{\"abi\": [" + std::to_string(MELLOW_ABI_VERSION) + ", " + std::to_string(MELLOW_ABI_MINOR) + "], \"precision\": \"";
    s += e->opt.mode == MELLOW_PRECISION_F32 ? "f32" : e->opt.mode == MELLOW_PRECISION_FP8 ? "fp8" : "f32x3";
    s += "\", \"reads_environment\": false, \"finalized\": ";
    s += e->finalized ? "true" : "false";
    s += ", \"stft_is_fft\": ";
    s += e->w.fft_win ? "true" : "false";
    s += ", \"non_default\": [";
    bool first = true;
    for (const auto& o : kOptions)
        if (opt_val(e, o.key) != strtol(o.dflt, nullptr, 0)) { s += std::string(first ? "" : ", ") + "\"" + o.key + "\""; first = false; }
    s += "], \"options\": {";
    first = true;
    for (const auto& o : kOptions) {
        s += std::string(first ? "" : ", ") + "\"" + o.key + "\": {\"value\": " + std::to_string(opt_val(e, o.key)) + ", \"default\": " +
             std::to_string(strtol(o.dflt, nullptr, 0)) + ", \"changes_answers\": " + (o.answers ? "true" : "false") + "}";
        first = false;
    }
    s += "}}";
    if (buf && capacity > (int64_t)s.size()) memcpy(buf, s.c_str(), s.size() + 1);
    return (int64_t)s.size() + 1;
}

int mellow_last_steps_enqueued(mellow_engine_t* e) { return e ? e->last_steps_enqueued : -1; }

int mellow_last_row_repacks(mellow_engine_t* e) { return e ? e->last_compactions : -1; }

int mellow_stft_is_fft(mellow_engine_t* e) { return e && e->w.fft_win ? 1 : 0; }

int mellow_abi_minor(void) { return MELLOW_ABI_MINOR; }
int mellow_prefill_parts(mellow_engine_t* e) {
    if (!e) return -1;
    if (!e->opt.f32x3_terms && !(e->opt.fp8 && e->opt.fp8_prefill)) return 1;
    if (hipSetDevice(e->device) != hipSuccess) return -1;
    if (ensure_prefill_streams(e) != 0) return -1;
    return e->prefill_parts < 1 ? 1 : (e->prefill_parts > 4 ? 4 : e->prefill_parts);
}

int mellow_prof_enable(mellow_engine_t* e, int on) {
    if (!e) return fail("null engine");
    e->prof_on = on != 0;
    return 0;
}

int mellow_prof_reset(mellow_engine_t* e) {
    if (!e) return fail("null engine");
    hipStreamSynchronize(e->stream);
    e->prof.clear();
    e->ev_used = 0;
    return 0;
}

int mellow_prof_get(mellow_engine_t* e, int i, int64_t* launches, double* ms, double* flops, double* bytes) {
    if (!e || i < 0 || i >= PF_COUNT) return fail("bad argument");
    HIPCHK(hipSetDevice(e->device));
    HIPCHK(hipStreamSynchronize(e->stream));
    int64_t n = 0;
    double t = 0, f = 0, by = 0;
    for (const auto& r : e->prof)
        if (r.fam == i) {
            float m = 0.f;
            HIPCHK(hipEventElapsedTime(&m, r.a, r.b));
            t += m; f += r.flops; by += r.bytes; ++n;
        }
    if (launches) *launches = n;
    if (ms) *ms = t;
    if (flops) *flops = f;
    if (bytes) *bytes = by;
    return 0;
}

int mellow_last_phase_ms(mellow_engine_t* e, float* encode_ms, float* prefill_ms, float* decode_ms) {
    if (!e) return fail("null engine");
    if (encode_ms) *encode_ms = e->phase_ms[0];
    if (prefill_ms) *prefill_ms = e->phase_ms[1];
    if (decode_ms) *decode_ms = e->phase_ms[2];
    return 0;
}

int mellow_engine_set_precision(mellow_engine_t* e, int mode) {
    if (!e) return fail("null engine");
    if (e->finalized) return fail("precision must be chosen before mellow_engine_finalize");
    if (mode != MELLOW_PRECISION_F32 && mode != MELLOW_PRECISION_FP8 && mode != MELLOW_PRECISION_F32X3)
        return fail("unknown precision mode %d", mode);
    e->opt.mode = mode;
    return apply_options(e);
}

int mellow_engine_fork(mellow_engine_t* parent, mellow_engine_t** out) {
    if (!parent || !out) return fail("null argument");
// ... 31 lines not shown
```

mellow_amd/csrc/engine_internal.h:

```cpp
#pragma once
#include <hip/hip_runtime.h>

#include <array>
#include <chrono>
#include <cmath>
#include <cstdarg>
#include <cstdio>
#include <cstdlib>
#include <cstring>
#include <map>
#include <unordered_map>
#include <string>
#include <thread>
#include <type_traits>
#include <utility>
#include <vector>

#include "../../include/mellow_hip.h"
#include "kernels.h"

using namespace mellow;

int fail(const char* fmt, ...);
struct mellow_engine;
// ... 51 lines not shown
    float* bias_exp;
    float* mask;
};
struct MergeW {
    float *nw, *nb;
    Packed red;
};
struct DecW {
    const float *p, *scale;
};
struct LMLayerW {
    Packed qkv, o, gateup, down;
    Packed qkv_f, gateup_f;
    float* o16 = nullptr;
    float* gu16n = nullptr;
    float* gu16 = nullptr;
    float* qkv2 = nullptr;
    float *q2h8 = nullptr, *q2h_sc = nullptr;
    float *qkv8 = nullptr, *qkv_sc = nullptr, *o8 = nullptr, *o_sc = nullptr, *gu8 = nullptr, *gu_sc = nullptr, *dn8 = nullptr,
          *dn_sc = nullptr;
    float *in_ln, *post_ln;
    DecW qkv_w() const { return qkv8 ? DecW{qkv8, qkv_sc} : DecW{qkv_f.p, nullptr}; }
    DecW o_w() const { return o8 ? DecW{o8, o_sc} : DecW{o16, nullptr}; }
    DecW gateup_w() const { return gu8 ? DecW{gu8, gu_sc} : DecW{gu16, nullptr}; }
    DecW down_w() const { return dn8 ? DecW{dn8, dn_sc} : DecW{down.p, nullptr}; }
};

struct ProfRec {
    int fam;
    hipEvent_t a, b;
    double flops, bytes;
    int M = 0, N = 0, K = 0, epi = 0;
};

struct StepMode {
    bool logits = true;
    bool sample = false;
    bool logprob = false;
    bool early_exit = false;
    bool migrate = false;
    int beam = 0;
    bool rules = false;
    bool guide = false;
};
struct Guidance {
    bool on = false;
    float scale = 1.f;
};
struct LogitRules {
    bool on = false;
    float theta = 1.f;
    int ngram = 0, min_new = 0;
    bool bias = false;
};

#define LOCAL __attribute__((visibility("hidden")))
struct mellow_engine {
    struct Buf {
        float* p = nullptr;
        size_t cap = 0;
        Buf() = default; Buf(const Buf&) = delete; Buf& operator=(const Buf&) = delete;
        Buf(Buf&& o) noexcept : p(o.p), cap(o.cap) { o.p = nullptr; o.cap = 0; }
        Buf& operator=(Buf&& o) noexcept { std::swap(p, o.p); std::swap(cap, o.cap); return *this; }
        LOCAL ~Buf() { if (p) (void)hipFree(p); }
    };
    struct LOCAL Options {
        std::map<std::string, std::string> given;
        int mode = MELLOW_PRECISION_F32X3;
        bool x3_stft = true, stft_fft = true, x3_apb = true, x3_attn = true, x3w = true, row_migration = true, decode_fuse = true;
        int arena_mb = 3400;
        bool kv16 = false;
        bool fp8 = false;
        bool fp8_decode = false;
        bool fp8_decode_act = false;
        bool fp8_attn_bf16 = true;
        bool fp8_prefill = true;
        int dec_x3_min_rb = 2;
        int dec_x3 = 0;
        int f32x3_terms = 0;
        bool prefill_fuse_norm = true;
        int enc_apb_stages = 0x1CC;
        int sk_max = 8;
        int dec_fuse_max_rb = 1;
    };
    struct Fp8W { uint8_t* w8; float* scale; };
    struct LOCAL Weights {
        Packed dft, mel;
        float *fft_win = nullptr, *fft_tw1 = nullptr, *fft_tw2 = nullptr;
        float *bn_alpha = nullptr, *bn_beta = nullptr;
        float *pe_w = nullptr, *pe_b = nullptr, *pe_nw = nullptr, *pe_nb = nullptr;
        std::vector<SwinBlockW> blocks[4];
        MergeW merge[3];
        int32_t* win_map[4][2] = {{nullptr}};
        float *fn_w = nullptr, *fn_b = nullptr;
        Packed tscam, c2l, lin1, lin2;
        float *tscam_b = nullptr, *c2l_b = nullptr, *pln_w = nullptr, *pln_b = nullptr;
        int32_t* emb_row_map = nullptr;
        float* embed = nullptr;
        Packed lm_head;
        std::vector<LMLayerW> layers;
        float* final_norm = nullptr;
        float *rope_cos = nullptr, *rope_sin = nullptr;
        float *head8 = nullptr, *head_sc = nullptr;
        DecW head_w() const { return head8 ? DecW{head8, head_sc} : DecW{lm_head.p, nullptr}; }
        std::unordered_map<const float*, void*> bf_w;
        std::unordered_map<const float*, Fp8W> fp8_w;
    };
    struct LOCAL StepGraphs {
        struct Key {
            std::array<uintptr_t, 18> v{};
            static Key of(const mellow_engine* e, int B);
            bool operator==(const Key& k) const { return v == k.v; }
        };
        hipGraphExec_t one = nullptr, eight = nullptr;
        Key key;
        StepGraphs() = default; StepGraphs(const StepGraphs&) = delete; StepGraphs& operator=(const StepGraphs&) = delete;
        void reset() {
            for (hipGraphExec_t* x : {&one, &eight}) if (*x) { (void)hipGraphExecDestroy(*x); *x = nullptr; }
        }
        ~StepGraphs() { reset(); }
    };

    mellow_config_t cfg;
    int device = 0;
    hipStream_t stream = nullptr;
    Options opt;
    Weights w;
    bool use_graph = true;
    int prefill_parts = 2;
    bool streams_probed = false;
    int probe_backoff = 0, prefill_parts_ok = 1, prefill_parts_want = 2;
    hipStream_t stream2[3] = {nullptr, nullptr, nullptr};
    hipEvent_t ev_fork = nullptr, ev_join[3] = {nullptr, nullptr, nullptr};
    bool finalized = false;
    bool owns_weights = true;
    std::map<std::string, HostTensor> host;
    std::vector<void*> allocs;
    char* arena = nullptr;
    size_t arena_size = 0, arena_used = 0;
    bool decode_only_weight = false;

    Buf wavcat, wpad, power, logmel, X0, X1, T, QKV, H, ats, fpx, fpxavg, latv, emb33, e1, gbuf, sbuf, proj33;
    Buf lm_x, lm_xn, lm_q, lm_o, lm_h, kcache, vcache;
    Buf kcache16, vcache16;
    bool kv16_direct = false;
    Buf lm_xn3, lm_o3, lm_h3;
    Buf lm_ssq;
    Buf dec;
    Buf dlogits, cand;
    Buf sc_prefix, sc_part, sc_ws;
    Buf sk_ws;
    bool sk_enable = false;
    Buf enc_a3, enc_h3;
    Buf a8, a8_scale;
    DecArgs da;
    int32_t *d_tokens = nullptr, *d_step = nullptr, *d_pos = nullptr, *d_seen = nullptr, *d_nseen = nullptr;
    int32_t *d_arrive = nullptr, *d_ticket = nullptr, *d_params = nullptr;
    int32_t *d_blk_left = nullptr, *d_blk_live = nullptr;
    int32_t *d_row_of_slot = nullptr, *d_ncompact = nullptr;
    int last_compactions = 0;
    unsigned long long* h_progress = nullptr;
    unsigned long long* d_progress = nullptr;
    std::map<std::pair<int, int>, float*> resample_banks;
    int32_t h_params[2] = {0, 0};
    uint32_t* d_sparams = nullptr;
    uint32_t h_sparams[SMP_WORDS] = {0};
    uint32_t* d_rparams = nullptr;
    uint32_t h_rparams[RUL_WORDS] = {0};
    uint32_t* d_gparams = nullptr;
    uint32_t h_gparams[GDN_WORDS] = {0};
    Guidance guide_armed;
    LogitRules rules_armed;
    Buf rules_bias, rules_hist;
    StepMode mode;
    int32_t h_blk[64] = {0};
    std::vector<int32_t> h_ident;
    int last_steps_enqueued = 0;
    Buf out_tok;
    Buf cand_sum, out_lp;
    Buf kprefix, vprefix, nseq_rows;
    Buf beam_ws, kstage, vstage;
    int beam_max_len = 0;
    std::vector<float> h_beam;
    Buf lm_xq;
    std::vector<int32_t> h_nseq_rows;
    int kv_B = 0, kv_Tmax = 0;
    int cur_B = 0, cur_pos = 0;
    int32_t h_pos_word = 0;
    StepGraphs graphs;

    bool taps_on = false;
    std::map<std::string, Buf> taps;
    std::map<std::string, int64_t> tap_numel;

    uint64_t dbg_spans[960] = {};
    int dbg_seq0 = -1;
    mellow_engine* parent = nullptr;
    int n_forks = 0, prefill_parts_saved = 2;

    bool prof_on = false;
    std::vector<ProfRec> prof;
    std::vector<hipEvent_t> ev_pool;
    size_t ev_used = 0;
    hipEvent_t ev_phase[4] = {nullptr, nullptr, nullptr, nullptr};
    float phase_ms[3] = {0, 0, 0};
};

#undef LOCAL
inline mellow_engine::StepGraphs::Key mellow_engine::StepGraphs::Key::of(const mellow_engine* e, int B) {
    return Key{{(uintptr_t)B,
                (uintptr_t)e->kv_Tmax,
                (uintptr_t)e->mode.sample,
                (uintptr_t)e->out_tok.p,
                (uintptr_t)e->da.blk_live,
                (uintptr_t)e->da.row_of_slot,
                (uintptr_t)e->mode.logprob,
                (uintptr_t)e->da.cand_sum,
                (uintptr_t)(e->mode.logprob ? e->out_lp.p : nullptr),
                (uintptr_t)e->mode.beam,
                (uintptr_t)(e->mode.beam ? e->beam_ws.p : nullptr),
                (uintptr_t)(e->mode.beam ? e->beam_max_len : 0),
                (uintptr_t)(e->mode.beam > 1 ? e->kstage.p : nullptr),
                (uintptr_t)(e->mode.beam > 1 ? e->vstage.p : nullptr),
                (uintptr_t)e->mode.rules,
                (uintptr_t)(e->mode.rules ? e->rules_bias.p : nullptr),
                (uintptr_t)(e->mode.rules && e->mode.beam ? e->rules_hist.p : nullptr),
                (uintptr_t)e->mode.guide}};
}
static_assert(!std::is_copy_constructible<mellow_engine::Buf>::value, "a Buf owns its device memory: it moves, it is never copied");
static_assert(std::is_copy_assignable<mellow_engine::Weights>::value && std::is_copy_assignable<mellow_engine::Options>::value, "a fork copies these by assignment: no owning member (Buf, StepGraphs) belongs in them");

int ensure(mellow_engine* e, mellow_engine::Buf& b, size_t floats);
int dev_alloc(mellow_engine* e, float** out, size_t floats);
int upload(mellow_engine* e, float** out, const float* src, size_t floats, size_t alloc_floats = 0);
hipEvent_t next_event(mellow_engine* e);
int tap(mellow_engine* e, const char* name, const float* src, int64_t n);
std::vector<std::string> build_required(const mellow_config_t* cfg);
const std::vector<std::string>& default_required();
bool is_ignored_key(const std::string& k);
void window_map_host(int R, int shift, int32_t* out);
void pack_weight_host(const float* w, int N, int K, int NP, int KP, float* out);
void rope_tables_host(float theta, int head_dim, int P, float* c, float* s);
int alloc_state_words(mellow_engine* e);
struct ProfScope {
    mellow_engine* e;
    ProfRec r;
    bool on;
    ProfScope(mellow_engine* e_, int fam, double flops, double bytes) : e(e_), on(e_->prof_on) {
        if (on) {
            r.fam = fam;
            r.flops = flops;
            r.bytes = bytes;
            r.a = next_event(e);
            r.b = next_event(e);
            hipEventRecord(r.a, e->stream);
        }
    }
    ~ProfScope() {
        if (on) {
            hipEventRecord(r.b, e->stream);
            e->prof.push_back(r);
        }
    }
};
int run_gemm(mellow_engine* e, const GemmArgs& a);
int run_gemm_apb(mellow_engine* e, const GemmArgs& a, const void* a3, hipStream_t st = nullptr, const void* a3_scales = nullptr);
GemmArgs lin(const float* A, int64_t lda, int M, const Packed& w, float* C, int64_t ldc, const float* bias);
int run_encoder(mellow_engine* e, const float* wav, int n, int64_t n_samples, int want_logmel_only, int apply_bn, float* logmel_out);
static inline int rb_of(int B) { return (B + 31) / 32; }
static inline size_t kv_layer_floats(const mellow_engine* e) { return (size_t)e->kv_B * 3 * e->kv_Tmax * 64; }
struct RecordArgs {
    bool embed_next = false;
};
int ensure_lm(mellow_engine* e, int B, int T, int Tmax, int ctx_end = 0, int prefill_B = 0, size_t prefill_rows = 0);
static inline int prefix_page_len(int T) { return rup(T, 64); }
int clear_page_tails(mellow_engine* e, int T, int t_end);
LoopArgs loop_args(mellow_engine* e);
void apply_step_mode(mellow_engine* e, const StepMode& m);
int run_lm_head(mellow_engine* e, int B, int pending_kcd, const RecordArgs* rec);
BeamArgs beam_args(mellow_engine* e, int N, int k);
RulesArgs rules_args(mellow_engine* e, int B);
GuideArgs guide_args(mellow_engine* e);
int run_prefill(mellow_engine* e, int B, int T, const RecordArgs* rec, bool all_positions = false, int n = 1);
struct PrefillSpan {
    int rows;
    int pos0;
    float* x;
    bool to_prefix;
    bool all_layers;
};
int run_prefill_q(mellow_engine* e, int B, int Q, int T, int P, const RecordArgs* rec);
int enqueue_decode_layer_range(mellow_engine* e, int B, int l_begin, int l_end, bool inc_pos);
int enqueue_decode_layers(mellow_engine* e, int B, const RecordArgs* rec);
int ensure_prefill_streams(mellow_engine* e);
int encode_pair_to_prefix(mellow_engine* e, const float* a1, const float* a2, int64_t n_samples, const int32_t* ids, int B, float* prefix_out);
int encode_pair_to_head_tail(mellow_engine* e, const float* a1, const float* a2, int64_t n_samples, const int32_t* ids, int B, int Q,
                             int P, float* head_out, float* tail_out);
int run_score_head(mellow_engine* e, int B, int T, int from_pos, int n, const int32_t* targets, float* out_logprob,
                   int32_t* out_argmax, float* out_lse, float* out_max);
void clear_bad_id(mellow_engine* e);
int check_bad_id(mellow_engine* e);
```

mellow_amd/csrc/engine_lm.cpp:

```cpp
#include "engine_internal.h"

int ensure_lm(mellow_engine* e, int B, int T, int Tmax, int ctx_end, int prefill_B, size_t prefill_rows) {
    if (B > 1024) return fail("batch of %d exceeds the 1024 rows one pass takes (mellow_generate chunks larger batches itself; the decode state block is sized for 32 row blocks)", B);
    if (ctx_end <= 0 || ctx_end > Tmax) ctx_end = Tmax;
    if (Tmax > e->cfg.max_positions) return fail("prefix + max_len = %d exceeds max_positions %d", Tmax, e->cfg.max_positions);
    const size_t Mp = prefill_rows > 0 ? prefill_rows : (size_t)(prefill_B > 0 ? prefill_B : B) * T;
    CHK(ensure(e, e->lm_x, Mp * 576));
    CHK(ensure(e, e->lm_xn, Mp * 576));
    CHK(ensure(e, e->lm_q, Mp * 576));
    CHK(ensure(e, e->lm_o, Mp * 576));
    CHK(ensure(e, e->lm_h, Mp * 1536));
    if (e->opt.f32x3_terms || (e->opt.fp8 && e->opt.fp8_prefill)) {
        const size_t Mq = (size_t)rup((int)Mp, 128) + 3 * 128;
        CHK(ensure(e, e->lm_xn3, Mq * 576 * 6 / 4));
        CHK(ensure(e, e->lm_o3, Mq * 576 * 6 / 4));
        CHK(ensure(e, e->lm_h3, Mq * 1536 * 6 / 4));
        CHK(ensure(e, e->lm_ssq, Mq * 2 * 16));
    }
    e->kv16_direct = e->opt.kv16 && e->opt.fp8 && e->opt.fp8_prefill && e->opt.fp8_attn_bf16 && e->opt.x3_apb && e->opt.x3_attn && !e->w.layers.empty() &&
                     e->w.fp8_w.count(e->w.layers[0].qkv.p) != 0;
    dec_prepare_lds_attributes();
    const int Bp = rb_of(B) * 32;
    if (e->kv_B != Bp || e->kv_Tmax != Tmax) {
        e->kv_B = Bp;
        e->kv_Tmax = Tmax;
        CHK(ensure(e, e->kcache, kv_layer_floats(e) * e->cfg.num_layers));
        CHK(ensure(e, e->vcache, kv_layer_floats(e) * e->cfg.num_layers));
        if (e->opt.kv16) {
            CHK(ensure(e, e->kcache16, kv_layer_floats(e) * e->cfg.num_layers / 2));
            CHK(ensure(e, e->vcache16, kv_layer_floats(e) * e->cfg.num_layers / 2));
        }
        HIPCHK(hipMemsetAsync(e->kcache.p, 0, kv_layer_floats(e) * e->cfg.num_layers * sizeof(float), e->stream));
        HIPCHK(hipMemsetAsync(e->vcache.p, 0, kv_layer_floats(e) * e->cfg.num_layers * sizeof(float), e->stream));
        if (e->opt.kv16) {
            HIPCHK(hipMemsetAsync(e->kcache16.p, 0, kv_layer_floats(e) * e->cfg.num_layers * sizeof(float) / 2, e->stream));
            HIPCHK(hipMemsetAsync(e->vcache16.p, 0, kv_layer_floats(e) * e->cfg.num_layers * sizeof(float) / 2, e->stream));
        }
        e->graphs.reset();
    }
    {
        const size_t RB = (size_t)Bp / 32, V = (size_t)e->cfg.vocab_size;
        const size_t n_x = (size_t)Bp * 576;
        size_t off = 0;
        auto take = [&](size_t n) { size_t o = off; off += (n + 63) / 64 * 64; return o; };
        const size_t o_xmidF = take(n_x), o_xnewR = take(n_x), o_xnF = take(n_x * 3 / 2);
        const size_t o_dslabF = take(DEC_KC_DOWN * n_x), o_ssq1 = take((size_t)Bp * DEC_KC_QKV), o_rope = take(64);
        const size_t o_pq = take((size_t)DEC_KC_QKV * Bp * 960);
        const size_t o_att = take((size_t)DEC_TS * n_x), o_aml = take((size_t)DEC_TS * 9 * Bp * 2);
        const size_t o_ssq = take((size_t)Bp * 40), o_gu = take(RB * 192 * 256), o_xmidF16 = take(n_x);
        const bool x3l = (e->opt.dec_x3 & DEC_X3_GATEUP) && (e->opt.dec_x3 & DEC_X3_QKV) && (int)RB >= e->opt.dec_x3_min_rb && !e->opt.fp8_decode &&
                         e->w.layers.size() > 1 && e->w.layers[1].qkv2 != nullptr && e->w.layers[1].gu16n != nullptr;
        const size_t o_x3a = take(x3l ? n_x * 3 / 2 : 0), o_x3b = take(x3l ? n_x * 3 / 2 : 0), o_h3 = take(x3l ? RB * 192 * 256 * 3 / 2 : 0);
        const bool fresh = e->dec.cap < off;
        CHK(ensure(e, e->dec, off));
        CHK(ensure(e, e->dlogits, (size_t)Bp * V));
        CHK(ensure(e, e->cand, (size_t)2 * Bp * (V / 32)));
        if (fresh) {
            HIPCHK(hipMemsetAsync(e->dec.p, 0, off * sizeof(float), e->stream));
            e->graphs.reset();
        }
        float* p = e->dec.p;
        DecArgs& a = e->da;
        a.rows = Bp; a.RB = (int)RB; a.Tmax = Tmax; a.eps = e->cfg.rms_norm_eps; a.d_pos = e->d_pos; a.inc_pos = 0; a.first = 0;
        a.a8 = e->opt.fp8_decode_act ? 1 : 0;
        a.kv16 = e->opt.kv16 ? 1 : 0;
        a.x3 = e->opt.dec_x3;
        a.rope_cos = e->w.rope_cos; a.rope_sin = e->w.rope_sin;
        a.xmidF = p + o_xmidF; a.xnewR = p + o_xnewR; a.xnF = p + o_xnF;
        a.xn3 = (a.x3 & DEC_X3_HEAD) && !e->w.head8 && dec_head3r_fits(e->cfg.vocab_size) ? (void*)(p + o_xnF) : nullptr;
        a.xmid3_32 = x3l ? (void*)(p + o_x3a) : nullptr; a.xmid3_16 = x3l ? (void*)(p + o_x3b) : nullptr; a.h3 = x3l ? (void*)(p + o_h3) : nullptr;
        a.dslabF = p + o_dslabF; a.slabF_stride4 = (int64_t)(n_x / 4); a.ssq1 = p + o_ssq1; a.rope_cur = p + o_rope;
        {
            const int ng_end = (ctx_end - 1 + 3) / 4, chunk = dec_attn_chunk_groups(e->opt.kv16);
            a.ts = dec_key_splits((int)RB, e->opt.kv16 || e->opt.mode != MELLOW_PRECISION_F32X3);
            int gs = (ng_end + a.ts - 1) / a.ts;
            if (gs > chunk && gs % chunk <= 4) gs -= gs % chunk;
            gs = gs < 1 ? 1 : gs;
            if (gs != a.gs) e->graphs.reset();
            a.gs = gs;
        }
        a.pq = p + o_pq; a.attF16 = p + o_att; a.att_ml = p + o_aml; a.ssq = p + o_ssq; a.guF = p + o_gu; a.xmidF16 = p + o_xmidF16;
        a.cand_val = e->cand.p; a.cand_idx = reinterpret_cast<int32_t*>(e->cand.p + (size_t)Bp * (V / 32));
        apply_step_mode(e, StepMode());
    }
    return 0;
}

void apply_step_mode(mellow_engine* e, const StepMode& m) {
    e->mode = m;
    DecArgs& a = e->da;
    e->mode.logits = m.logits || m.rules || m.guide;
    a.logits = e->mode.logits ? e->dlogits.p : nullptr;
    a.cand_sum = m.logprob ? e->cand_sum.p : nullptr;
    a.blk_live = m.early_exit ? e->d_blk_live : nullptr;
    a.blk_snap = e->d_blk_live + 32;
    a.row_of_slot = m.migrate ? e->d_row_of_slot : nullptr;
}

int clear_page_tails(mellow_engine* e, int T, int t_end) {
    const int Tmax = e->kv_Tmax;
    if (t_end > Tmax) t_end = Tmax;
    if (T >= t_end) return 0;
    if (e->kv16_direct) launch_clear_page_slots(e->vcache16.p, (int64_t)e->cfg.num_layers * e->kv_B * 3, Tmax, T, t_end, e->stream, true);
    else launch_clear_page_slots(e->vcache.p, (int64_t)e->cfg.num_layers * e->kv_B * 3, Tmax, T, t_end, e->stream);
    HIPCHK(hipGetLastError());
    return 0;
}

LoopArgs loop_args(mellow_engine* e) {
    LoopArgs lp;
    lp.out_tokens = reinterpret_cast<int32_t*>(e->out_tok.p);
    lp.params = e->d_params; lp.seen_stop = e->d_seen; lp.n_seen = e->d_nseen; lp.arrive = e->d_arrive; lp.ticket = e->d_ticket;
    lp.host_progress = e->d_progress; lp.T0 = e->cfg.prefix_len;
    if (e->da.blk_live) { lp.blk_left = e->d_blk_left; lp.blk_live = e->d_blk_live; lp.blk_snap = e->d_blk_live + 32; }
    if (e->da.row_of_slot) { lp.row_of_slot = e->d_row_of_slot; lp.n_compactions = e->d_ncompact; }
    if (e->mode.logprob) lp.out_logprob = e->out_lp.p;
    return lp;
}

BeamArgs beam_args(mellow_engine* e, int N, int k) {
    float* w = e->beam_ws.p;
    int32_t* wi = reinterpret_cast<int32_t*>(w);
    const size_t tab = (size_t)e->beam_max_len * N, t0 = 3 * 1024 + 3 * 1024 * BEAM_MAX_K;
    BeamArgs g;
    g.logits = e->da.logits; g.ld = e->cfg.vocab_size; g.k = k; g.N = N;
    g.cum_in = g.cum_state = w; g.fin_in = g.fin_state = wi + 1024; g.cand_n = wi + 2048;
    g.cand_c = w + 3 * 1024; g.cand_tok = wi + 3 * 1024 + 1024 * BEAM_MAX_K; g.cand_lp = w + 3 * 1024 + 2 * 1024 * BEAM_MAX_K;
    g.out_parent = wi + t0; g.out_token = wi + t0 + tab; g.out_lp = w + t0 + 2 * tab; g.out_cum = w + t0 + 3 * tab;
    return g;
}

RulesArgs rules_args(mellow_engine* e, int B) {
    const LoopArgs lp = loop_args(e);
    RulesArgs g;
    g.logits = e->da.logits; g.ld = e->cfg.vocab_size; g.prm = e->d_rparams; g.bias = e->rules_bias.p;
    g.cand_val = e->da.cand_val; g.cand_idx = e->da.cand_idx; g.cand_sum = e->da.cand_sum;
    g.d_pos = e->d_pos; g.params = lp.params; g.T0 = lp.T0;
    g.row_of_slot = lp.row_of_slot; g.blk_snap = lp.blk_snap;
    if (e->mode.beam) {
        const BeamArgs bm = beam_args(e, B, e->mode.beam);
        g.beam_hist = reinterpret_cast<int32_t*>(e->rules_hist.p); g.hist_ld = e->beam_max_len;
        g.parent_tab = bm.out_parent; g.token_tab = bm.out_token; g.N = B; g.k = e->mode.beam;
    } else {
        g.hist = lp.out_tokens;
    }
    return g;
}

GuideArgs guide_args(mellow_engine* e) {
    const LoopArgs lp = loop_args(e);
    GuideArgs g;
    g.logits = e->da.logits; g.ld = e->cfg.vocab_size; g.prm = e->d_gparams;
    g.cand_val = e->da.cand_val; g.cand_idx = e->da.cand_idx; g.cand_sum = e->da.cand_sum;
    g.blk_snap = lp.blk_snap;
    return g;
}

int run_lm_head(mellow_engine* e, int B, int pending_kcd, const RecordArgs* rec) {
    const int NT = e->cfg.vocab_size / 32, Bp = e->da.rows;
    auto dh = [&](int k) { DecArgs x = e->da; x.dbg_seq = e->dbg_seq0 >= 0 ? e->dbg_seq0 + 5 * e->cfg.num_layers + k : -1000; return x; };
    { ProfScope ps(e, PF_NORM, 0, (double)(pending_kcd + 2) * Bp * 576 * 4);
      launch_dec_final_norm(dh(0), e->w.final_norm, pending_kcd, e->stream); }
    { ProfScope ps(e, PF_SKINNY, 2.0 * Bp * 576.0 * e->cfg.vocab_size, 576.0 * e->cfg.vocab_size * 4);
      const DecW h = e->w.head_w();
      launch_dec_lm_head(dh(1), h.p, e->w.lm_head.KP / 8, e->cfg.vocab_size, e->stream, h.scale); }
    if (e->mode.guide && rec) {
        ProfScope ps(e, PF_MISC, 0, 6.0 * B * e->cfg.vocab_size * 4);
        launch_dec_guidance(guide_args(e), B / 2, e->stream);
    }
    if (e->mode.rules && rec) {
        ProfScope ps(e, PF_MISC, 0, 2.0 * B * e->cfg.vocab_size * 4);
        launch_dec_logit_rules(rules_args(e, B), B, e->stream);
    }
    { ProfScope ps(e, PF_MISC, 0, 0);
      if (e->mode.beam) {
          const LoopArgs lp = loop_args(e);
          launch_beam_select(beam_args(e, B, e->mode.beam), B / e->mode.beam, dh(2), e->d_tokens, e->w.embed, &lp, e->stream);
      } else if (e->mode.sample) {
          SampleArgs sa;
// ... 124 lines not shown
                if (fz) { g.C3 = xn3; g.ssq_out = ssq_in; g.ssq_parts = 9; c3_amx(g, xn3s, 9); }
                if (apb) CHK(run_gemm_apb(e, g, h3, st, h3s)); else CHK(run_gemm(e, g));
            }
        }
        if (last) break;
    }
    CHK(join.run());
    HIPCHK(hipGetLastError());
    return 0;
}

static int finish_prefill(mellow_engine* e, int N, int T, const float* x, const int32_t* row_ids, int n_src, const RecordArgs* rec) {
    hipStream_t s = e->stream;
    const int NL = e->cfg.num_layers;
    { ProfScope ps(e, PF_MISC, 0, 0);
      launch_dec_load_rows(e->da, N, x, 576, row_ids, T, row_ids ? n_src : 0, s); }
    e->cur_B = N;
    e->cur_pos = T;
    e->h_pos_word = T - 1;
    HIPCHK(hipMemcpyAsync(e->d_pos, &e->h_pos_word, sizeof(int32_t), hipMemcpyHostToDevice, s));
    CHK(enqueue_decode_layer_range(e, N, NL - 1, NL, false));
    CHK(run_lm_head(e, N, DEC_KC_DOWN, rec));
    HIPCHK(hipGetLastError());
    return 0;
}

int run_prefill(mellow_engine* e, int B, int T, const RecordArgs* rec, bool all_positions, int n) {
    hipStream_t s = e->stream;
    const int NL = e->cfg.num_layers;
    const bool fan = n > 1;
    if (fan && (all_positions || T != e->cfg.prefix_len || e->opt.kv16 || !e->kprefix.p || !e->vprefix.p || !e->nseq_rows.p || B * n > e->kv_B))
        return fail("internal: the fan-out prefill needs fp32 pages for %d rows and its prefix buffer", B * n);
    CHK(run_prefill_span(e, B, PrefillSpan{T, 0, e->lm_x.p, fan, all_positions}));
    if (e->opt.kv16 && !e->kv16_direct && !all_positions) {
        ProfScope ps(e, PF_MISC, 0, 3.0 * kv_layer_floats(e) * NL * 4);
        launch_kv_to_bf16(e->kcache.p, e->kcache16.p, (int64_t)(kv_layer_floats(e) * NL), s);
        launch_kv_to_bf16(e->vcache.p, e->vcache16.p, (int64_t)(kv_layer_floats(e) * NL), s);
    }
    if (all_positions) return 0;
    if (fan) {
        ProfScope ps(e, PF_MISC, 0, (1.0 + n) * 2.0 * NL * B * 3 * T * 64 * 4);
        launch_kv_fanout(e->kprefix.p, e->vprefix.p, e->kcache.p, e->vcache.p, NL, B, n, e->kv_B, T, prefix_page_len(T), e->kv_Tmax, s);
    }
    return finish_prefill(e, B * n, T, e->lm_x.p, fan ? reinterpret_cast<const int32_t*>(e->nseq_rows.p) : nullptr, B * T, rec);
}

int run_prefill_q(mellow_engine* e, int B, int Q, int T, int P, const RecordArgs* rec) {
    const int NL = e->cfg.num_layers, N = B * Q, Tt = T - P;
    if (Q < 2 || P <= 0 || P >= T || P % 32 != 0 || T != e->cfg.prefix_len || e->opt.fp8 || e->opt.kv16 || !e->kprefix.p || !e->vprefix.p ||
        !e->nseq_rows.p || !e->lm_xq.p || N > e->kv_B)
        return fail("internal: the question prefill needs fp32 pages for %d rows, its prefix buffer and its tail input", N);
    CHK(run_prefill_span(e, B, PrefillSpan{P, 0, e->lm_x.p, true, false}));
    { ProfScope ps(e, PF_MISC, 0, (1.0 + Q) * 2.0 * NL * B * 3 * P * 64 * 4);
      launch_kv_fanout(e->kprefix.p, e->vprefix.p, e->kcache.p, e->vcache.p, NL, B, Q, e->kv_B, P, prefix_page_len(T), e->kv_Tmax, e->stream); }
    CHK(run_prefill_span(e, N, PrefillSpan{Tt, P, e->lm_xq.p, false, false}));
    return finish_prefill(e, N, T, e->lm_xq.p, reinterpret_cast<const int32_t*>(e->nseq_rows.p), N * Tt, rec);
}

int enqueue_decode_layer_range(mellow_engine* e, int B, int l_begin, int l_end, bool inc_pos) {
    hipStream_t s = e->stream;
    const int Bp = e->da.rows;
#ifdef MELLOW_DEVPROBE
    static const bool same_w = getenv("MELLOW_DEV_SAME_WEIGHTS") != nullptr, same_kv = getenv("MELLOW_DEV_SAME_KV") != nullptr;
    static const int skip = getenv("MELLOW_DEV_SKIP") ? atoi(getenv("MELLOW_DEV_SKIP")) : 0;
#else
    constexpr bool same_w = false, same_kv = false;
    constexpr int skip = 0;
#endif
    for (int l = l_begin; l < l_end; ++l) {
        const LMLayerW& w = e->w.layers[same_w ? 0 : l];
        const DecW qkv = w.qkv_w(), o = w.o_w(), gu = w.gateup_w(), dn = w.down_w();
        float* kc = e->opt.kv16 ? e->kcache16.p + kv_layer_floats(e) / 2 * (same_kv ? 0 : l) : e->kcache.p + kv_layer_floats(e) * (same_kv ? 0 : l);
        float* vc = e->opt.kv16 ? e->vcache16.p + kv_layer_floats(e) / 2 * (same_kv ? 0 : l) : e->vcache.p + kv_layer_floats(e) * (same_kv ? 0 : l);
        const int kcd = l == l_begin ? 0 : DEC_KC_DOWN;
        const bool x3l = e->da.xmid3_32 != nullptr;
        const bool fuse_rb = x3l || e->da.RB <= e->opt.dec_fuse_max_rb;
        const bool fused_in = l > l_begin && ((w.qkv2 != nullptr && fuse_rb) || w.q2h8 != nullptr) && !same_w;
        DecArgs a = e->da;
        const int sq = e->dbg_seq0 >= 0 ? e->dbg_seq0 + 5 * (l - l_begin) : -1000;
        auto da = [&](int k) { DecArgs x = e->da; x.dbg_seq = sq + k; return x; };
        a.dbg_seq = sq;
        a.first = l == l_begin ? 1 : 0;
        a.inc_pos = (inc_pos && l == l_begin) ? 1 : 0;
        if (!(skip & 1) && !fused_in)
        { ProfScope ps(e, PF_SKINNY, 2.0 * Bp * 576.0 * 960.0, 576.0 * 960.0 * 4);
          launch_dec_qkv(a, qkv.p, w.qkv_f.KP / 8, kcd, s, qkv.scale); }
        if (!(skip & 2))
        { ProfScope ps(e, PF_DECODE_ATTN, 4.0 * 64 * 9 * (double)B * (e->cur_pos + 1), 2.0 * (double)B * 3 * 64 * 4 * (e->cur_pos + 1));
          launch_dec_attn(da(1), kc, vc, fused_in, s); }
        if (!(skip & 4))
        { ProfScope ps(e, PF_SKINNY, 2.0 * Bp * 576.0 * 576.0, 576.0 * 576.0 * 4);
          launch_dec_oproj(da(2), o.p, s, o.scale); }
        if (!(skip & 8))
        { ProfScope ps(e, PF_SKINNY, 2.0 * Bp * 576.0 * 3072.0, 576.0 * 3072.0 * 4);
          if (x3l && !w.gu8) launch_dec_gateup3(da(3), w.gu16n, s);
          else launch_dec_gateup(da(3), gu.p, s, gu.scale); }
        const LMLayerW* nx = (l + 1 < l_end && !same_w) ? &e->w.layers[l + 1] : nullptr;
        if (nx && ((nx->qkv2 && fuse_rb) || nx->q2h8)) {
            if (!(skip & 16))
            { ProfScope ps(e, PF_SKINNY, 2.0 * Bp * (2112.0 * 960.0 + 1536.0 * 576.0), (2112.0 * 960.0 + 1536.0 * 576.0) * (nx->q2h8 ? 1 : 4));
              if (nx->q2h8) launch_dec_qkv2_w8(da(4), nx->qkv8, nx->qkv_sc, nx->q2h8, nx->q2h_sc, w.dn8, w.dn_sc, s);
              else if (x3l) launch_dec_qkv2x3(da(4), nx->qkv2, w.down.p, s);
              else launch_dec_qkv2(da(4), nx->qkv2, w.down.p, s); }
        } else if (!(skip & 16))
        { ProfScope ps(e, PF_SKINNY, 2.0 * Bp * 576.0 * 1536.0, 576.0 * 1536.0 * 4);
          launch_dec_down(da(4), dn.p, w.down.KP / 8, s, dn.scale); }
    }
    return 0;
}
int enqueue_decode_layers(mellow_engine* e, int B, const RecordArgs* rec) {
    CHK(enqueue_decode_layer_range(e, B, 0, e->cfg.num_layers, true));
    CHK(run_lm_head(e, B, DEC_KC_DOWN, rec));
    if (e->mode.beam > 1) {
        ProfScope ps(e, PF_MISC, 0, 0);
        launch_beam_reorder(e->kcache.p, e->vcache.p, e->kstage.p, e->vstage.p, beam_args(e, B, e->mode.beam).out_parent, e->d_pos, e->d_params,
                            e->cfg.prefix_len, e->cfg.num_layers, B, e->mode.beam, e->kv_B, e->kv_Tmax, e->stream);
    }
    return 0;
}

static int encode_pair(mellow_engine* e, const float* a1, const float* a2, int64_t n_samples, int B) {
    mellow_engine::Buf& cat = e->wavcat;
    CHK(ensure(e, cat, (size_t)2 * B * n_samples));
    HIPCHK(hipMemcpyAsync(cat.p, a1, (size_t)B * n_samples * 4, hipMemcpyDeviceToDevice, e->stream));
    HIPCHK(hipMemcpyAsync(cat.p + (size_t)B * n_samples, a2, (size_t)B * n_samples * 4, hipMemcpyDeviceToDevice, e->stream));
    return run_encoder(e, cat.p, 2 * B, n_samples, 0, 1, nullptr);
}
int encode_pair_to_prefix(mellow_engine* e, const float* a1, const float* a2, int64_t n_samples, const int32_t* ids,
                                 int B, float* prefix_out) {
    CHK(encode_pair(e, a1, a2, n_samples, B));
    { ProfScope ps(e, PF_MISC, 0, 0);
      launch_prefix_assemble(e->proj33.p, e->w.embed, ids, B, e->cfg.text_len, e->cfg.sep_token_id, e->cfg.vocab_size, prefix_out,
                             e->d_progress + 1, e->stream); }
    HIPCHK(hipGetLastError());
    return 0;
}
int encode_pair_to_head_tail(mellow_engine* e, const float* a1, const float* a2, int64_t n_samples, const int32_t* ids, int B, int Q,
                             int P, float* head_out, float* tail_out) {
    CHK(encode_pair(e, a1, a2, n_samples, B));
    { ProfScope ps(e, PF_MISC, 0, 0);
      launch_prefix_assemble_q(e->proj33.p, e->w.embed, ids, B, Q, e->cfg.text_len, P, e->cfg.sep_token_id, e->cfg.vocab_size, head_out,
                               tail_out, e->d_progress + 1, e->stream); }
    HIPCHK(hipGetLastError());
    return 0;
}

void clear_bad_id(mellow_engine* e) { __atomic_store_n(e->h_progress + 1, 0ull, __ATOMIC_RELEASE); }

int check_bad_id(mellow_engine* e) {
    const unsigned long long w = __atomic_load_n(e->h_progress + 1, __ATOMIC_ACQUIRE);
    if (!w) return 0;
    return fail("index out of range in self: prompt id %d of example %u is outside the vocabulary [0, %d)", (int)(unsigned)(w & 0xffffffffu),
                (unsigned)((w >> 32) & 0x7fffffffu), e->cfg.vocab_size);
}

static void clear_bad_target(mellow_engine* e) { __atomic_store_n(e->h_progress + 2, 0ull, __ATOMIC_RELEASE); }
static int check_bad_target(mellow_engine* e, const char* what, int lo) {
    const unsigned long long w = __atomic_load_n(e->h_progress + 2, __ATOMIC_ACQUIRE);
    if (!w) return 0;
    return fail("index out of range in self: %s id %d of row %u is outside [%d, %d)", what, (int)(unsigned)(w & 0xffffffffu),
                (unsigned)((w >> 32) & 0x7fffffffu), lo, e->cfg.vocab_size);
}

int run_score_head(mellow_engine* e, int B, int T, int from_pos, int n, const int32_t* targets, float* out_logprob,
                   int32_t* out_argmax, float* out_lse, float* out_max) {
    hipStream_t s = e->stream;
    const int V = e->cfg.vocab_size, rows = B * n, groups = V / 64;
    if (V % 64 != 0 || e->w.lm_head.Nw != V) return fail("the scoring head tiles the vocabulary in groups of 64 columns (vocab %d)", V);
    const size_t ld = (size_t)rup(rows, 64);
    CHK(ensure(e, e->sc_part, (size_t)groups * ld * 3));
    float2* part_ms = reinterpret_cast<float2*>(e->sc_part.p);
    int32_t* part_arg = reinterpret_cast<int32_t*>(e->sc_part.p + (size_t)groups * ld * 2);
    float* tgt_logit = e->sc_ws.p;
    GemmArgs g = lin(e->lm_xn.p, 576, rows, e->w.lm_head, nullptr, 0, nullptr);
    g.epi = EPI_LSE;
    g.lse_target = targets; g.lse_ms = part_ms; g.lse_arg = part_arg; g.lse_tgt = tgt_logit; g.lse_ld = (int64_t)ld;
    ProfScope ps(e, PF_LM_HEAD, gemm_flops(g), 576.0 * V * 4 + (double)rows * 576 * 4 + 3.0 * rows * groups * 12);
    launch_gather_span(e->lm_x.p, B, T, from_pos, n, e->lm_o.p, s);
    launch_rmsnorm(e->lm_o.p, e->lm_xn.p, rows, 576, e->w.final_norm, e->cfg.rms_norm_eps, s);
    launch_gemm(g, s);
    launch_lse_merge(part_ms, part_arg, (int64_t)ld, groups, rows, targets, tgt_logit, V, out_logprob, out_argmax, out_lse, out_max,
                     e->d_progress + 2, s);
    HIPCHK(hipGetLastError());
    return 0;
}

extern "C" {

int mellow_prefix(mellow_engine_t* e, const float* audio1, const float* audio2, int64_t n_samples, const int32_t* input_ids,
                  int B, float* out) {
    if (!e || !e->finalized) return fail("engine not finalized");
    if (!audio1 || !audio2 || !input_ids || !out) return fail("null argument");
    if (B <= 0) return fail("B must be positive");
    HIPCHK(hipSetDevice(e->device));
    clear_bad_id(e);
    CHK(encode_pair_to_prefix(e, audio1, audio2, n_samples, input_ids, B, out));
    HIPCHK(hipStreamSynchronize(e->stream));
    return check_bad_id(e);
}

int mellow_lm_prefill(mellow_engine_t* e, const float* prefix, int B, int T, int reserve, float* logits) {
    if (!e || !e->finalized) return fail("engine not finalized");
    if (!prefix || B <= 0 || T <= 0 || reserve < 0) return fail("bad argument");
    HIPCHK(hipSetDevice(e->device));
    CHK(ensure_lm(e, B, T, T + reserve + 1));
    HIPCHK(hipMemcpyAsync(e->lm_x.p, prefix, (size_t)B * T * 576 * 4, hipMemcpyDeviceToDevice, e->stream));
    CHK(clear_page_tails(e, T, e->kv_Tmax));
    CHK(run_prefill(e, B, T, nullptr));
    if (logits)
        HIPCHK(hipMemcpyAsync(logits, e->dlogits.p, (size_t)B * e->cfg.vocab_size * 4, hipMemcpyDeviceToDevice, e->stream));
    HIPCHK(hipStreamSynchronize(e->stream));
    return 0;
}

int mellow_lm_decode_step(mellow_engine_t* e, const int32_t* token_ids, float* logits) {
    if (!e || !e->finalized) return fail("engine not finalized");
    if (!token_ids) return fail("null argument");
    if (e->cur_B <= 0) return fail("decode step without a prefill");
    if (e->cur_pos + 1 > e->kv_Tmax) return fail("KV pages exhausted (reserve too small)");
    HIPCHK(hipSetDevice(e->device));
    const int B = e->cur_B;
    launch_dec_load_rows(e->da, B, e->w.embed, 576, token_ids, 0, e->cfg.vocab_size, e->stream);
    CHK(enqueue_decode_layers(e, B, nullptr));
    e->cur_pos += 1;
    if (logits)
        HIPCHK(hipMemcpyAsync(logits, e->dlogits.p, (size_t)B * e->cfg.vocab_size * 4, hipMemcpyDeviceToDevice, e->stream));
    HIPCHK(hipGetLastError());
    HIPCHK(hipStreamSynchronize(e->stream));
    return 0;
}

int mellow_debug_dec_head(mellow_engine_t* e, const float* x, int B, int act_fp8, float* logits) {
    if (!e || !e->finalized) return fail("engine not finalized");
    if (!x || !logits || B <= 0 || B > 1024) return fail("bad argument");
    if (e->cfg.hidden_size != 576) return fail("the decode kernels are built for hidden size 576");
    HIPCHK(hipSetDevice(e->device));
    CHK(ensure_lm(e, B, 1, 2));
    DecArgs a = e->da;
    a.blk_live = nullptr; a.row_of_slot = nullptr;
    a.a8 = (act_fp8 && e->w.head8) ? 1 : 0;
    a.xnF = a.xmidF;
    a.xn3 = nullptr;
    launch_dec_load_rows(a, B, x, 576, nullptr, 1, 0, e->stream);
    const DecW h = e->w.head_w();
    launch_dec_lm_head(a, h.p, e->w.lm_head.KP / 8, e->cfg.vocab_size, e->stream, h.scale);
    HIPCHK(hipMemcpyAsync(logits, e->dlogits.p, (size_t)B * e->cfg.vocab_size * 4, hipMemcpyDeviceToDevice, e->stream));
    HIPCHK(hipGetLastError());
    HIPCHK(hipStreamSynchronize(e->stream));
    e->cur_B = 0;
    return 0;
}

int mellow_debug_dec_head_lse(mellow_engine_t* e, const float* x, int B, int act_fp8, float* logits, float* out_lse, float* out_max,
                              int32_t* out_argmax) {
    if (!e || !e->finalized) return fail("engine not finalized");
    if (!x || !out_lse || !out_max || !out_argmax || B <= 0 || B > 1024) return fail("bad argument");
    if (e->cfg.hidden_size != 576) return fail("the decode kernels are built for hidden size 576");
    HIPCHK(hipSetDevice(e->device));
    CHK(ensure_lm(e, B, 1, 2));
    const int NT = e->cfg.vocab_size / 32;
    CHK(ensure(e, e->cand_sum, (size_t)e->da.rows * NT));
    DecArgs a = e->da;
    a.blk_live = nullptr; a.row_of_slot = nullptr;
    a.a8 = (act_fp8 && e->w.head8) ? 1 : 0;
    a.xnF = a.xmidF;
    a.xn3 = nullptr;
    a.cand_sum = e->cand_sum.p;
    if (!logits) a.logits = nullptr;
    launch_dec_load_rows(a, B, x, 576, nullptr, 1, 0, e->stream);
    const DecW h = e->w.head_w();
    launch_dec_lm_head(a, h.p, e->w.lm_head.KP / 8, e->cfg.vocab_size, e->stream, h.scale);
    launch_dec_argmax(a, B, NT, e->d_tokens, e->w.embed, 0, LoopArgs(), e->stream);
    launch_dec_lse_tap(a, B, NT, out_lse, out_max, e->stream);
    HIPCHK(hipMemcpyAsync(out_argmax, e->d_tokens, (size_t)B * sizeof(int32_t), hipMemcpyDeviceToDevice, e->stream));
    if (logits) HIPCHK(hipMemcpyAsync(logits, e->dlogits.p, (size_t)B * e->cfg.vocab_size * 4, hipMemcpyDeviceToDevice, e->stream));
    HIPCHK(hipGetLastError());
    HIPCHK(hipStreamSynchronize(e->stream));
    e->cur_B = 0;
    return 0;
}

int mellow_embed_tokens(mellow_engine_t* e, const int32_t* token_ids, int n, float* out) {
    if (!e || !e->finalized) return fail("engine not finalized");
    if (!token_ids || !out || n <= 0) return fail("bad argument");
    HIPCHK(hipSetDevice(e->device));
    launch_gather_rows(e->w.embed, 576, token_ids, n, e->cfg.vocab_size, out, e->stream);
    HIPCHK(hipGetLastError());
    HIPCHK(hipStreamSynchronize(e->stream));
    return 0;
}

int mellow_lm_forward_logits(mellow_engine_t* e, const float* embeds, int B, int T, int from_pos, float* logits) {
    if (!e || !e->finalized) return fail("engine not finalized");
    if (!embeds || !logits || B <= 0 || T <= 0 || from_pos < 0 || from_pos >= T) return fail("bad argument");
    HIPCHK(hipSetDevice(e->device));
    hipStream_t s = e->stream;
    CHK(ensure_lm(e, B, T, T + 1));
    HIPCHK(hipMemcpyAsync(e->lm_x.p, embeds, (size_t)B * T * 576 * 4, hipMemcpyDeviceToDevice, s));
    CHK(run_prefill(e, B, T, nullptr, true));
    e->cur_B = 0;
    const int n = T - from_pos;
    GemmArgs g = lin(e->lm_xn.p, 576, B * n, e->w.lm_head, logits, e->cfg.vocab_size, nullptr);
    { ProfScope ps(e, PF_LM_HEAD, gemm_flops(g), (576.0 + (double)B * n) * e->cfg.vocab_size * 4 + (double)B * n * 576 * 4);
      launch_gather_span(e->lm_x.p, B, T, from_pos, n, e->lm_o.p, s);
      launch_rmsnorm(e->lm_o.p, e->lm_xn.p, B * n, 576, e->w.final_norm, e->cfg.rms_norm_eps, s);
      launch_gemm(g, s); }
// ... 68 lines not shown
```

mellow_amd/csrc/engine_weights.cpp:

```cpp
#include "engine_internal.h"

static const HostTensor* get(mellow_engine* e, const std::string& k) {
    auto it = e->host.find(k);
    return it == e->host.end() ? nullptr : &it->second;
}
static int expect_shape(const HostTensor* t, const std::string& k, std::initializer_list<int64_t> shp) {
    if (!t) return fail("missing key in state_dict: %s", k.c_str());
    if (t->dtype != MELLOW_F32) return fail("%s: expected float32", k.c_str());
    if (t->shape.size() != shp.size())
        return fail("size mismatch for %s: rank %d in the checkpoint, %d expected", k.c_str(), (int)t->shape.size(), (int)shp.size());
    size_t i = 0;
    for (auto d : shp) {
        if (t->shape[i] != d)
            return fail("size mismatch for %s: dimension %d is %lld in the checkpoint, %lld expected", k.c_str(), (int)i,
                        (long long)t->shape[i], (long long)d);
        ++i;
    }
    return 0;
}
static int up_vec(mellow_engine* e, const std::string& k, int64_t n, float** out, int64_t pad_to = 0) {
    const HostTensor* t = get(e, k);
    CHK(expect_shape(t, k, {n}));
    return upload(e, out, t->f(), (size_t)n, (size_t)pad_to);
}
// ... 3 lines not shown
    p.K = K;
    p.KP = rup(K, 32);
    p.Nw = w1 ? 64 * ((N + 31) / 32) : N;
    p.NP = rup(p.Nw, 128);
    {
        mellow_engine::Buf d0, d1;
        CHK(ensure(e, d0, (size_t)N * K));
        HIPCHK(hipMemcpy(d0.p, w0, (size_t)N * K * sizeof(float), hipMemcpyHostToDevice));
        if (w1) {
            CHK(ensure(e, d1, (size_t)N * K));
            HIPCHK(hipMemcpy(d1.p, w1, (size_t)N * K * sizeof(float), hipMemcpyHostToDevice));
        }
        CHK(dev_alloc(e, &p.p, (size_t)p.NP * p.KP));
        if (w1) launch_pack_weight_pairs(d0.p, d1.p, N, K, K, p.p, p.NP, p.KP, e->stream);
        else launch_pack_weight(d0.p, N, K, K, p.p, p.NP, p.KP, e->stream);
        HIPCHK(hipGetLastError());
        HIPCHK(hipStreamSynchronize(e->stream));
    }
    if (e->opt.f32x3_terms && p.KP % 16 == 0 && !e->decode_only_weight) {
        float* pb = nullptr;
        CHK(dev_alloc(e, &pb, ((size_t)p.NP * p.KP * 6 + 3) / 4));
        launch_pack_bf16x3(p.p, p.NP, p.KP, pb, e->stream);
        HIPCHK(hipGetLastError());
        HIPCHK(hipStreamSynchronize(e->stream));
        e->w.bf_w[p.p] = pb;
    }
    if (e->opt.fp8 && e->opt.fp8_prefill && !e->decode_only_weight) {
        float *w8f = nullptr, *sc = nullptr;
        CHK(dev_alloc(e, &w8f, ((size_t)p.NP * rup(p.KP, 64) + 3) / 4));
        CHK(dev_alloc(e, &sc, (size_t)p.NP));
        launch_pack_fp8(p.p, p.NP, p.KP, reinterpret_cast<uint8_t*>(w8f), sc, e->stream);
        HIPCHK(hipGetLastError());
        HIPCHK(hipStreamSynchronize(e->stream));
        e->w.fp8_w[p.p] = {reinterpret_cast<uint8_t*>(w8f), sc};
    }
    *out = p;
    return 0;
}
static int make_w8(mellow_engine* e, const Packed& p) {
    if (!e->opt.fp8 || !e->opt.fp8_prefill || e->w.fp8_w.count(p.p)) return 0;
    float *w8f = nullptr, *sc = nullptr;
    CHK(dev_alloc(e, &w8f, ((size_t)p.NP * rup(p.KP, 64) + 3) / 4));
    CHK(dev_alloc(e, &sc, (size_t)p.NP));
    launch_pack_fp8(p.p, p.NP, p.KP, reinterpret_cast<uint8_t*>(w8f), sc, e->stream);
    HIPCHK(hipGetLastError());
    HIPCHK(hipStreamSynchronize(e->stream));
    e->w.fp8_w[p.p] = {reinterpret_cast<uint8_t*>(w8f), sc};
    return 0;
}
static int make_pb(mellow_engine* e, const Packed& p) {
    if (!e->opt.f32x3_terms || p.KP % 16 != 0 || e->w.bf_w.count(p.p)) return 0;
    float* pb = nullptr;
    CHK(dev_alloc(e, &pb, ((size_t)p.NP * p.KP * 6 + 3) / 4));
    launch_pack_bf16x3(p.p, p.NP, p.KP, pb, e->stream);
    HIPCHK(hipGetLastError());
    HIPCHK(hipStreamSynchronize(e->stream));
    e->w.bf_w[p.p] = pb;
    return 0;
}
static int make_dec_fp8(mellow_engine* e, const float* Wp, int tiles, int slots, int rows, float** out8, float** scale) {
    CHK(dev_alloc(e, out8, (size_t)tiles * slots));
    CHK(dev_alloc(e, scale, (size_t)tiles * rows));
    launch_pack_dec_fp8(Wp, tiles, slots, rows, *out8, *scale, e->stream);
    HIPCHK(hipGetLastError());
    HIPCHK(hipStreamSynchronize(e->stream));
    return 0;
}
static int make_packed16(mellow_engine* e, const float* w, int N, int K, float** out, bool natural = false) {
    if (N % 16 || K % (natural ? 32 : 16)) return fail("P16 packing needs N and K multiples of 16 (32 for the P16N order)");
    mellow_engine::Buf d0;
    CHK(ensure(e, d0, (size_t)N * K));
    HIPCHK(hipMemcpy(d0.p, w, (size_t)N * K * sizeof(float), hipMemcpyHostToDevice));
    CHK(dev_alloc(e, out, (size_t)N * K));
    if (natural) launch_pack_weight16n(d0.p, N, K, *out, e->stream);
    else launch_pack_weight16(d0.p, N, K, *out, e->stream);
    HIPCHK(hipGetLastError());
    HIPCHK(hipStreamSynchronize(e->stream));
    return 0;
}
static int pack_key(mellow_engine* e, const std::string& k, int N, int K, Packed* out) {
    const HostTensor* t = get(e, k);
    CHK(expect_shape(t, k, {N, K}));
    return make_packed(e, t->f(), nullptr, N, K, out);
}

extern "C" int mellow_engine_finalize(mellow_engine_t* e) {
    if (!e) return fail("null engine");
    if (e->finalized) return 0;
    HIPCHK(hipSetDevice(e->device));
    for (const auto& k : build_required(&e->cfg))
        if (!get(e, k)) return fail("missing key in state_dict: %s", k.c_str());
    const std::string E = ENC;
    {
        const std::string kr = E + "spectrogram_extractor.stft.conv_real.weight", ki = E + "spectrogram_extractor.stft.conv_imag.weight";
        CHK(expect_shape(get(e, kr), kr, {kNfreq, 1, kNfft}));
        CHK(expect_shape(get(e, ki), ki, {kNfreq, 1, kNfft}));
        CHK(make_packed(e, get(e, kr)->f(), get(e, ki)->f(), kNfreq, kNfft, &e->w.dft));
        const bool no_fft = !e->opt.stft_fft;
        if ((e->opt.f32x3_terms || (e->opt.fp8 && e->opt.fp8_prefill)) && !no_fft && kNfft == 1024) {
            const float *wr = get(e, kr)->f(), *wi = get(e, ki)->f();
            double wmax = 0.0, dev = 0.0;
            for (int n = 0; n < kNfft; ++n) wmax = std::max(wmax, (double)fabsf(wr[n]));
            for (int k = 0; k < kNfreq; ++k)
                for (int n = 0; n < kNfft; ++n) {
                    const double a = 2.0 * M_PI * (double)((int64_t)k * n % kNfft) / kNfft, w0 = wr[n];
                    dev = std::max(dev, fabs((double)wr[(size_t)k * kNfft + n] - w0 * cos(a)));
                    dev = std::max(dev, fabs(fabs((double)wi[(size_t)k * kNfft + n]) - fabs(w0 * sin(a))));
                }
            if (wmax > 0.0 && dev <= 1e-6 * wmax) {
                std::vector<float> t1((size_t)16 * 64 * 2), t2((size_t)4 * 16 * 2);
                for (int k1 = 0; k1 < 16; ++k1)
                    for (int b = 0; b < 64; ++b) {
                        const double a = -2.0 * M_PI * (double)(b * k1) / 1024.0;
                        t1[((size_t)k1 * 64 + b) * 2] = (float)cos(a); t1[((size_t)k1 * 64 + b) * 2 + 1] = (float)sin(a);
                    }
                for (int d = 0; d < 4; ++d)
                    for (int q = 0; q < 16; ++q) {
                        const double a = -2.0 * M_PI * (double)(d * q) / 64.0;
                        t2[((size_t)d * 16 + q) * 2] = (float)cos(a); t2[((size_t)d * 16 + q) * 2 + 1] = (float)sin(a);
                    }
                CHK(upload(e, &e->w.fft_win, wr, kNfft));
                CHK(upload(e, &e->w.fft_tw1, t1.data(), t1.size()));
                CHK(upload(e, &e->w.fft_tw2, t2.data(), t2.size()));
            }
        }
        const std::string km = E + "logmel_extractor.melW";
        CHK(expect_shape(get(e, km), km, {kNfreq, kMel}));
        std::vector<float> mt((size_t)kMel * kNfreq);
        const float* mw = get(e, km)->f();
        for (int k = 0; k < kNfreq; ++k)
            for (int n = 0; n < kMel; ++n) mt[(size_t)n * kNfreq + k] = mw[(size_t)k * kMel + n];
        CHK(make_packed(e, mt.data(), nullptr, kMel, kNfreq, &e->w.mel));
        const HostTensor *w = get(e, E + "bn0.weight"), *b = get(e, E + "bn0.bias"), *rm = get(e, E + "bn0.running_mean"),
                         *rv = get(e, E + "bn0.running_var");
        for (const char* nm : {"bn0.weight", "bn0.bias", "bn0.running_mean", "bn0.running_var"})
            CHK(expect_shape(get(e, E + nm), E + nm, {kMel}));
        std::vector<float> al(kMel), be(kMel);
        for (int i = 0; i < kMel; ++i) {
            const float invstd = 1.0f / sqrtf(rv->f()[i] + 1e-5f);
            al[i] = invstd * w->f()[i];
            be[i] = b->f()[i] - rm->f()[i] * al[i];
        }
        CHK(upload(e, &e->w.bn_alpha, al.data(), kMel));
        CHK(upload(e, &e->w.bn_beta, be.data(), kMel));
    }
    {
        const std::string k = E + "patch_embed.proj.weight";
        CHK(expect_shape(get(e, k), k, {96, 1, 4, 4}));
        CHK(upload(e, &e->w.pe_w, get(e, k)->f(), 96 * 16));
        CHK(up_vec(e, E + "patch_embed.proj.bias", 96, &e->w.pe_b));
        CHK(up_vec(e, E + "patch_embed.norm.weight", 96, &e->w.pe_nw));
        CHK(up_vec(e, E + "patch_embed.norm.bias", 96, &e->w.pe_nb));
    }
    for (int s = 0; s < 4; ++s) {
        const int C = 96 << s, nH = kHeads[s], R = 64 >> s, nW = (R / kWin) * (R / kWin);
        for (int sh = 0; sh < 2; ++sh) {
            if (R <= kWin) continue;
            std::vector<int32_t> m((size_t)R * R);
            window_map_host(R, sh ? kWin / 2 : 0, m.data());
            float* d = nullptr;
            CHK(upload(e, &d, reinterpret_cast<const float*>(m.data()), m.size()));
            e->w.win_map[s][sh] = reinterpret_cast<int32_t*>(d);
        }
        for (int b = 0; b < kDepths[s]; ++b) {
            const std::string p = E + "layers." + std::to_string(s) + ".blocks." + std::to_string(b) + ".";
            SwinBlockW w{};
// ... 99 lines not shown
        CHK(make_packed(e, qkv.data(), nullptr, 960, H, &w.qkv));
        CHK(pack_key(e, p + "self_attn.o_proj.weight", H, 576, &w.o));
        const HostTensor *g = get(e, p + "mlp.gate_proj.weight"), *u = get(e, p + "mlp.up_proj.weight");
        CHK(expect_shape(g, p + "mlp.gate_proj.weight", {I, H}));
        CHK(expect_shape(u, p + "mlp.up_proj.weight", {I, H}));
        CHK(make_packed(e, g->f(), u->f(), I, H, &w.gateup));
        CHK(pack_key(e, p + "mlp.down_proj.weight", H, I, &w.down));
        CHK(up_vec(e, p + "input_layernorm.weight", H, &w.in_ln));
        CHK(up_vec(e, p + "post_attention_layernorm.weight", H, &w.post_ln));
        {
            const HostTensor *l1 = get(e, p + "input_layernorm.weight"), *l2 = get(e, p + "post_attention_layernorm.weight");
            std::vector<float> f(qkv);
            for (int n = 0; n < 960; ++n)
                for (int kk = 0; kk < H; ++kk) f[(size_t)n * H + kk] = qkv[(size_t)n * H + kk] * l1->f()[kk];
            e->decode_only_weight = true;
            CHK(make_packed(e, f.data(), nullptr, 960, H, &w.qkv_f));
            e->decode_only_weight = false;
            if (e->opt.prefill_fuse_norm) { CHK(make_pb(e, w.qkv_f)); CHK(make_w8(e, w.qkv_f)); }
            if (fuse && l > 0) {
                const std::string kd = L + "model.layers." + std::to_string(l - 1) + ".mlp.down_proj.weight";
                CHK(expect_shape(get(e, kd), kd, {H, I}));
                HIPCHK(hipMemcpyAsync(cmpF.p, f.data(), (size_t)960 * 576 * 4, hipMemcpyHostToDevice, e->stream));
                HIPCHK(hipMemcpyAsync(cmpD.p, get(e, kd)->f(), (size_t)576 * 1536 * 4, hipMemcpyHostToDevice, e->stream));
                launch_compose_f64(cmpF.p, cmpD.p, cmpQ.p, 960, 1536, 576, e->stream);
                if (e->opt.fp8_decode) {
                    launch_pack_weight(cmpQ.p, 960, 1536, 1536, cmpCat.p, 1024, 1536, e->stream);
                    HIPCHK(hipGetLastError());
                    CHK(make_dec_fp8(e, cmpCat.p, 32, (1536 / 8) * 64, 32, &w.q2h8, &w.q2h_sc));
                } else {
                    HIPCHK(hipMemcpy2DAsync(cmpCat.p, (size_t)2112 * 4, cmpF.p, (size_t)576 * 4, (size_t)576 * 4, 960, hipMemcpyDeviceToDevice, e->stream));
                    HIPCHK(hipMemcpy2DAsync(cmpCat.p + 576, (size_t)2112 * 4, cmpQ.p, (size_t)1536 * 4, (size_t)1536 * 4, 960, hipMemcpyDeviceToDevice, e->stream));
                    CHK(dev_alloc(e, &w.qkv2, (size_t)1024 * 2112));
                    launch_pack_weight(cmpCat.p, 960, 2112, 2112, w.qkv2, 1024, 2112, e->stream);
                    HIPCHK(hipGetLastError());
                    HIPCHK(hipStreamSynchronize(e->stream));
                }
            }
            std::vector<float> gf((size_t)I * H), uf((size_t)I * H);
            for (int n = 0; n < I; ++n)
                for (int kk = 0; kk < H; ++kk) {
                    gf[(size_t)n * H + kk] = g->f()[(size_t)n * H + kk] * l2->f()[kk];
                    uf[(size_t)n * H + kk] = u->f()[(size_t)n * H + kk] * l2->f()[kk];
                }
            if (e->opt.prefill_fuse_norm && (e->opt.f32x3_terms || (e->opt.fp8 && e->opt.fp8_prefill))) {
                e->decode_only_weight = true;
                CHK(make_packed(e, gf.data(), uf.data(), I, H, &w.gateup_f));
                e->decode_only_weight = false;
                CHK(make_pb(e, w.gateup_f));
                CHK(make_w8(e, w.gateup_f));
            }
            {
                std::vector<float> il((size_t)2 * I * H);
                for (int t = 0; t < I / 8; ++t) {
                    memcpy(il.data() + (size_t)(2 * t) * 8 * H, gf.data() + (size_t)t * 8 * H, (size_t)8 * H * 4);
                    memcpy(il.data() + (size_t)(2 * t + 1) * 8 * H, uf.data() + (size_t)t * 8 * H, (size_t)8 * H * 4);
                }
                CHK(make_packed16(e, il.data(), 2 * I, H, &w.gu16));
                if (e->opt.f32x3_terms && fuse && !e->opt.fp8_decode) CHK(make_packed16(e, il.data(), 2 * I, H, &w.gu16n, true));
            }
            CHK(make_packed16(e, get(e, p + "self_attn.o_proj.weight")->f(), H, 576, &w.o16));
        }
        if (e->opt.fp8_decode) {
            CHK(make_dec_fp8(e, w.qkv_f.p, w.qkv_f.NP / 32, (w.qkv_f.KP / 8) * 64, 32, &w.qkv8, &w.qkv_sc));
            CHK(make_dec_fp8(e, w.o16, H / 16, (576 / 16) * 64, 16, &w.o8, &w.o_sc));
            CHK(make_dec_fp8(e, w.gu16, 2 * I / 16, (H / 16) * 64, 16, &w.gu8, &w.gu_sc));
            CHK(make_dec_fp8(e, w.down.p, w.down.NP / 32, (w.down.KP / 8) * 64, 32, &w.dn8, &w.dn_sc));
        }
        e->w.layers.push_back(w);
    }
    CHK(up_vec(e, L + "model.norm.weight", H, &e->w.final_norm));
    {
        const int P = e->cfg.max_positions;
        const HostTensor *tc = get(e, "mellow.rope_cos"), *ts = get(e, "mellow.rope_sin");
        std::vector<float> c((size_t)P * 32), s((size_t)P * 32);
        if (tc && ts && tc->numel() == (int64_t)P * 32 && ts->numel() == (int64_t)P * 32) {
            memcpy(c.data(), tc->f(), c.size() * 4);
            memcpy(s.data(), ts->f(), s.size() * 4);
        } else {
            rope_tables_host(e->cfg.rope_theta, 64, P, c.data(), s.data());
        }
        CHK(upload(e, &e->w.rope_cos, c.data(), c.size()));
        CHK(upload(e, &e->w.rope_sin, s.data(), s.size()));
    }
    CHK(alloc_state_words(e));
    e->host.clear();
    e->finalized = true;
    return 0;
}
```

mellow_amd/csrc/kernels.h:

```cpp
#pragma once
#include <hip/hip_runtime.h>
#include <stdint.h>

namespace mellow {

void launch_pack_weight(const float* w, int N, int K, int64_t ldw, float* out, int NP, int KP, hipStream_t s);
void launch_pack_weight_pairs(const float* w0, const float* w1, int N, int K, int64_t ldw, float* out, int NP,
                              int KP, hipStream_t s);

enum { ACT_NONE = 0, ACT_GELU = 1, ACT_SIGMOID = 2 };
enum { EPI_LINEAR = 0, EPI_POWER = 1, EPI_LOGMEL = 2, EPI_SWIGLU = 3, EPI_QKV_ROPE = 4, EPI_LSE = 5, EPI_QKV_ROPE_AT = 6 };
enum { A_PLAIN = 0, A_FRAMES = 1 };

struct GemmArgs {
    const float* A = nullptr;
    int64_t lda = 0;
    int M = 0;
    int K = 0;
    int a_mode = A_PLAIN;
    int fpc = 1;
    int64_t clip_stride = 0;
    int hop = 0;
    const float* Wp = nullptr;
    int Nw = 0;
// ... 38 lines not shown
    int c3_kt64 = 0;
    const int32_t* lse_target = nullptr;
    float2* lse_ms = nullptr;
    int32_t* lse_arg = nullptr;
    float* lse_tgt = nullptr;
    int64_t lse_ld = 0;
};
void launch_gemm(const GemmArgs& a, hipStream_t s);
void launch_quant_mx8(const float* A, int64_t lda, int M, int K, void* img, void* sc, hipStream_t s);
void launch_pack_fp8(const float* Wp, int NP, int KP, uint8_t* W8, float* w_scale, hipStream_t s);
void launch_gemm_fp8(const GemmArgs& a, hipStream_t s);
void launch_pack_bf16x3(const float* Wp, int NP, int KP, void* PB, hipStream_t s);
void launch_gemm_bf16x3_fused(const GemmArgs& a, hipStream_t s);
void launch_split_rows_apb(const float* A, int64_t lda, int M, int K, void* out, hipStream_t s);
void launch_gemm_bf16x3_apb(const GemmArgs& a, hipStream_t s);
double gemm_flops(const GemmArgs& a);

void set_max_dynamic_lds(const void* fn, size_t bytes);

constexpr int DEC_KC_QKV = 8;
#ifndef MELLOW_DEC_KC_DOWN
#define MELLOW_DEC_KC_DOWN 8
#endif
constexpr int DEC_KC_DOWN = MELLOW_DEC_KC_DOWN;
#ifndef MELLOW_DEC_TS
#define MELLOW_DEC_TS 2
#endif
constexpr int DEC_TS = MELLOW_DEC_TS;
#ifndef MELLOW_DEC_TS_MULTI
#define MELLOW_DEC_TS_MULTI 1
#endif
constexpr int DEC_TS_MULTI = MELLOW_DEC_TS_MULTI;
inline int dec_key_splits(int RB, bool fixed) { return RB <= 1 || fixed ? DEC_TS : DEC_TS_MULTI; }
#ifndef MELLOW_Q2_HC
#define MELLOW_Q2_HC 4
#endif
#ifndef MELLOW_Q2_WAVES
#define MELLOW_Q2_WAVES 12
#else
#define MELLOW_Q2_WAVES_FORCED 1
#endif
constexpr int Q2_HC = MELLOW_Q2_HC, Q2_WAVES = MELLOW_Q2_WAVES;
constexpr int Q2_NPQ = 2 + Q2_HC;
constexpr int Q2_K8 = 72 + 192;
constexpr int Q2_BLOCKS = 60 + 48 * Q2_HC;
static_assert(Q2_NPQ <= DEC_KC_QKV && Q2_HC <= DEC_KC_DOWN, "the fused kernel reuses the slab buffers of the split-K kernels");
enum { DEC_X3_HEAD = 1, DEC_X3_GATEUP = 2, DEC_X3_QKV = 4, DEC_X3_ALL = 7 };
struct DecArgs {
    int rows = 0, RB = 0;
    int Tmax = 0;
    float eps = 1e-5f;
    int32_t* d_pos = nullptr;
    int first = 0;
    int inc_pos = 0;
    int gs = 1;
    int ts = DEC_TS;
    float* rope_cur = nullptr;
    float* ssq1 = nullptr;
    const float* rope_cos = nullptr;
    const float* rope_sin = nullptr;
    float* xmidF = nullptr;
    float* xnewR = nullptr;
    float* dslabF = nullptr;
    int64_t slabF_stride4 = 0;
    float* pq = nullptr;
    float* attF16 = nullptr;
    float* att_ml = nullptr;
    float* ssq = nullptr;
    float* xmidF16 = nullptr;
    float* guF = nullptr;
    float* xnF = nullptr;
    void *xmid3_32 = nullptr, *xmid3_16 = nullptr, *h3 = nullptr;
    void* xn3 = nullptr;
    const int32_t* blk_live = nullptr;
    int32_t* blk_snap = nullptr;
    const int32_t* row_of_slot = nullptr;
    int kv16 = 0;
    int a8 = 0;
    int x3 = 0;
    int dbg_seq = -1;
    float* logits = nullptr;
    float* cand_val = nullptr; int32_t* cand_idx = nullptr;
    float* cand_sum = nullptr;
};
void launch_dec_qkv(const DecArgs& a, const float* Wp_folded, int K8p, int kcd, hipStream_t s, const float* wscale = nullptr);
void launch_pack_dec_fp8(const float* Wp, int tiles, int slots_per_tile, int rows_per_tile, void* out, float* scale, hipStream_t s);
void launch_dec_attn(const DecArgs& a, float* k_cache, float* v_cache, bool fused, hipStream_t s);
void launch_kv_to_bf16(const float* src, void* dst, int64_t n, hipStream_t s);
void launch_kv_fanout(const float* k_prefix, const float* v_prefix, float* k_pages, float* v_pages, int layers, int B, int n, int Bp,
                      int T, int Tp, int Tmax, hipStream_t s);
void launch_dec_qkv2(const DecArgs& a, const float* Wq2, const float* Wd, hipStream_t s);
void launch_dec_qkv2x3(const DecArgs& a, const float* Wq2, const float* Wd, hipStream_t s);
void dec_prepare_lds_attributes();
void launch_dec_gateup3(const DecArgs& a, const float* Wp16n_folded_pairs, hipStream_t s);
void launch_dec_qkv2_w8(const DecArgs& a, const float* Wx8, const float* sc_x, const float* Wh8, const float* sc_h,
                        const float* Wd8, const float* sc_d, hipStream_t s);
void launch_compose_f64(const float* A, const float* B, float* C, int M, int N, int K, hipStream_t s);
int dec_attn_chunk_groups(bool kv16);
void launch_dec_oproj(const DecArgs& a, const float* Wp16, hipStream_t s, const float* wscale = nullptr);
void launch_dec_gateup(const DecArgs& a, const float* Wp16_folded_pairs, hipStream_t s, const float* wscale = nullptr);
void launch_dec_down(const DecArgs& a, const float* Wp, int K8p, hipStream_t s, const float* wscale = nullptr);
void launch_dec_final_norm(const DecArgs& a, const float* norm_w, int kcd, hipStream_t s);
bool dec_head3r_fits(int vocab);
void launch_dec_lm_head(const DecArgs& a, const float* Wp, int K8p, int vocab, hipStream_t s, const float* wscale = nullptr);
struct LoopArgs {
    int32_t* out_tokens = nullptr;
    const int32_t* params = nullptr;
    int32_t* seen_stop = nullptr;
    int32_t* n_seen = nullptr;
    int32_t* arrive = nullptr;
    int32_t* ticket = nullptr;
    int32_t* blk_left = nullptr;
    int32_t* blk_live = nullptr;
    const int32_t* blk_snap = nullptr;
    int32_t* row_of_slot = nullptr;
    int32_t* n_compactions = nullptr;
    unsigned long long* host_progress = nullptr;
    int T0 = 0;
    float* out_logprob = nullptr;
};
void launch_dec_argmax(const DecArgs& a, int B, int n_tiles, int32_t* tokens, const float* embed, int write_x,
                       const LoopArgs& loop, hipStream_t s);
void launch_dec_lse_tap(const DecArgs& a, int B, int n_tiles, float* out_lse, float* out_max, hipStream_t s);
enum { SMP_SEED_LO = 0, SMP_SEED_HI, SMP_ROW_OFF, SMP_TOP_P, SMP_TEMP, SMP_STEP, SMP_WORDS = 8 };
struct SampleArgs {
    const float* logits = nullptr;
    int64_t ld = 0;
    const uint32_t* prm = nullptr;
    const int32_t* row_ids = nullptr;
    int row_shift = 0;
};
constexpr int SAMPLE_MAX_V = 49152;
void launch_dec_sample(const SampleArgs& sa, const DecArgs& a, int B, int32_t* tokens, const float* embed, int write_x,
                       const LoopArgs& loop, hipStream_t s);
void launch_sample_logits(const SampleArgs& sa, int B, int32_t* tokens, hipStream_t s);
constexpr int BEAM_MAX_K = 8;
struct BeamArgs {
    const float* logits = nullptr;
    int64_t ld = 0;
    const float* cum_in = nullptr;
    const int32_t* fin_in = nullptr;
    float* cum_state = nullptr;
    int32_t* fin_state = nullptr;
    int k = 1, N = 0;
    int stop_id = 0;
    float* cand_c = nullptr; int32_t* cand_tok = nullptr; float* cand_lp = nullptr; int32_t* cand_n = nullptr;
    int32_t* out_parent = nullptr; int32_t* out_token = nullptr; float* out_lp = nullptr; float* out_cum = nullptr;
};
void launch_beam_select(const BeamArgs& g, int B, const DecArgs& a, int32_t* tokens, const float* embed, const LoopArgs* loop, hipStream_t s);
void launch_beam_reorder(float* k_pages, float* v_pages, float* k_stage, float* v_stage, const int32_t* parent_tab, const int32_t* d_pos,
                         const int32_t* params, int T0, int layers, int N, int k, int Bp, int Tmax, hipStream_t s);
enum { RUL_THETA = 0, RUL_NGRAM, RUL_MIN_NEW, RUL_BIAS_ON, RUL_STOP, RUL_WORDS = 8 };
constexpr int RULES_MAX_HIST = 8192;
struct RulesArgs {
    float* logits = nullptr;
    int64_t ld = 0;
    const uint32_t* prm = nullptr;
    const float* bias = nullptr;
    float* cand_val = nullptr; int32_t* cand_idx = nullptr;
    float* cand_sum = nullptr;
    const int32_t* hist = nullptr;
    int hist_ld = 0;
    const int32_t* hist_len = nullptr;
    const int32_t* d_pos = nullptr;
    const int32_t* params = nullptr;
    int T0 = 0;
    const int32_t* row_of_slot = nullptr;
    const int32_t* blk_snap = nullptr;
    int32_t* beam_hist = nullptr;
    const int32_t* parent_tab = nullptr; const int32_t* token_tab = nullptr;
    int N = 0, k = 1;
};
void launch_dec_logit_rules(const RulesArgs& g, int B, hipStream_t s);
enum { GDN_SCALE = 0, GDN_WORDS = 8 };
struct GuideArgs {
    float* logits = nullptr;
    int64_t ld = 0;
    const uint32_t* prm = nullptr;
    float* cand_val = nullptr; int32_t* cand_idx = nullptr;
    float* cand_sum = nullptr;
    const int32_t* blk_snap = nullptr;
};
void launch_dec_guidance(const GuideArgs& g, int P , hipStream_t s);
void launch_dec_compact(const DecArgs& a, int B, const LoopArgs& loop, hipStream_t s);
void launch_dec_load_rows(const DecArgs& a, int B, const float* in, int64_t ld, const int32_t* row_ids, int T_last,
                          int n_src , hipStream_t s);
void launch_pack_weight16(const float* w, int N, int K, float* out, hipStream_t s);
void launch_pack_weight16n(const float* w, int N, int K, float* out, hipStream_t s);
void set_kernel_debug_buffer(uint64_t* p);
void set_gemm_debug_buffer(uint64_t* p);

void launch_resample(const float* x, int n_clips, int64_t n_in, const float* wT, int orig, int nw, int klen, int width,
                     float* out, int64_t n_out, hipStream_t s);
void launch_reflect_pad(const float* wav, int n_clips, int64_t n_samples, float* out, int64_t padded_len, int pad,
                        hipStream_t s);
void launch_fold_patch_embed(const float* logmel_bn, int n_src, int src_frames, int n_crops, int crop_hop,
                             int crop_len, const float* conv_w, const float* conv_b, const float* ln_w,
                             const float* ln_b, float* x0, hipStream_t s);

void launch_layernorm(const float* in, float* out, int M, int C, const float* w, const float* b,
                      const int32_t* row_map, int ntok, hipStream_t s);
void launch_merge_layernorm(const float* in, float* out, int n, int R, int C, const float* w, const float* b,
                            hipStream_t s);
void launch_stft_fft_power(const float* wpad, int fpc, int64_t clip_stride, int hop, int M, const float* win, const float* tw1,
                           const float* tw2, float* power, hipStream_t s);
void launch_rmsnorm(const float* in, float* out, int M, int C, const float* w, float eps, hipStream_t s);
void launch_layernorm_apb(const float* in, void* out_apb, int M, int C, const float* w, const float* b, const int32_t* row_map,
                          int ntok, hipStream_t s, void* out_scales = nullptr);
void launch_rmsnorm_apb(const float* in, void* out_apb, int M, int C, const float* w, float eps, hipStream_t s, void* out_scales = nullptr);

void launch_window_attention(const float* qkv, float* out, int M, int C, int nH, const float* bias_exp,
                             const float* mask, int nW, hipStream_t s, void* out_apb = nullptr, bool qkv16 = false);

void launch_tail_latent_im2col(const float* y, int n, float* latent, int64_t latent_stride, float* a_ts,
                               hipStream_t s);
void launch_crop_average(const float* in, int n, int n_crops, int64_t len, int64_t in_stride, float* out,
                         int64_t out_stride, hipStream_t s);
void launch_gelu(const float* in, float* out, int64_t n, hipStream_t s);
void launch_prefix_assemble(const float* proj33, const float* embed, const int32_t* ids, int B, int text_len,
                            int sep_id, int vocab, float* prefix, unsigned long long* bad_id_word, hipStream_t s);
void launch_prefix_assemble_q(const float* proj33, const float* embed, const int32_t* ids, int B, int Q, int text_len, int P,
                              int sep_id, int vocab, float* head, float* tail, unsigned long long* bad_id_word, hipStream_t s);
void launch_gather_rows(const float* table, int width, const int32_t* ids, int n, int n_rows, float* out, hipStream_t s);
void launch_gather_span(const float* in, int B, int T, int from_pos, int n, float* out, hipStream_t s);
void launch_clear_page_slots(float* cache, int64_t pages, int Tmax, int t0, int t1, hipStream_t s, bool pages16 = false);
void launch_downsample33(const float* proj33, int n, float* out, hipStream_t s);

void launch_prefill_attention(const float* q, const float* k_cache, const float* v_cache, float* o, void* o_apb, int B, int T,
                              int Tmax, bool x3, hipStream_t s, void* o_scales = nullptr, bool bf16_once = false, bool pages16 = false);
void launch_prefill_attention_past(const float* q, const float* k_cache, const float* v_cache, float* o, void* o_apb, int B, int T,
                                   int Tmax, int q0, bool x3, hipStream_t s);
void launch_lse_merge(const float2* part_ms, const int32_t* part_arg, int64_t ld, int groups, int rows, const int32_t* targets,
                      const float* tgt_logit, int vocab, float* out_logprob, int32_t* out_argmax, float* out_lse, float* out_max,
                      unsigned long long* bad_word, hipStream_t s);
// ... 8 lines not shown
```

mellow_amd/csrc/sample.hip:

```cpp
#include "common.h"
#include "kernels.h"

namespace mellow {

namespace {

constexpr int SMP_THREADS = 1024, SMP_WAVES = SMP_THREADS / 64;
constexpr int SMP_NV4 = SAMPLE_MAX_V / 4 / SMP_THREADS;
static_assert(SMP_NV4 * 4 * SMP_THREADS == SAMPLE_MAX_V, "row tiling");

__device__ __forceinline__ int64_t f32_idx(int rb, int K8, int m, int k) {
    return ((int64_t)rb * K8 + (k >> 3)) * 64 + m + 32 * ((k >> 2) & 1);
}

__device__ __forceinline__ uint32_t okey(float z) {
    const uint32_t u = __float_as_uint(z);
    return (u & 0x80000000u) ? ~u : (u | 0x80000000u);
}

__device__ __forceinline__ float opaque(float x) {
    asm volatile("" : "+v"(x));
    return x;
}

__device__ __forceinline__ void philox4x32_10(uint32_t c0, uint32_t c1, uint32_t c2, uint32_t c3, uint32_t k0, uint32_t k1,
                                              uint32_t out[4]) {
#pragma unroll
    for (int r = 0; r < 10; ++r) {
        const uint32_t hi0 = __umulhi(0xD2511F53u, c0), lo0 = 0xD2511F53u * c0;
        const uint32_t hi1 = __umulhi(0xCD9E8D57u, c2), lo1 = 0xCD9E8D57u * c2;
        c0 = hi1 ^ c1 ^ k0; c1 = lo1; c2 = hi0 ^ c3 ^ k1; c3 = lo0;
        k0 += 0x9E3779B9u; k1 += 0xBB67AE85u;
    }
    out[0] = c0; out[1] = c1; out[2] = c2; out[3] = c3;
}

struct SelScratch {
    unsigned long long hist[SMP_WAVES][256];
    unsigned long long bin[256];
    uint32_t digit;
    unsigned long long above, mass;
};

template <typename KeyF, typename WF, typename ThrF>
__device__ __forceinline__ bool radix_select(KeyF key_of, WF w_of, ThrF thr_of, int shift_hi, SelScratch& sh, uint32_t& out_key,
                                             unsigned long long& out_above, unsigned long long& out_mass,
                                             unsigned long long& out_thr) {
    const int tid = threadIdx.x, wave = tid >> 6, lane = tid & 63;
    uint32_t prefix = 0, pmask = shift_hi + 8 >= 32 ? 0u : ~0u << (shift_hi + 8);
    unsigned long long above = 0, mass = 0, thr = 0;
    for (int shift = shift_hi; shift >= 0; shift -= 8) {
        for (int i = tid; i < SMP_WAVES * 256; i += SMP_THREADS) (&sh.hist[0][0])[i] = 0ull;
        __syncthreads();
#pragma unroll
        for (int k = 0; k < SMP_NV4; ++k)
#pragma unroll
            for (int j = 0; j < 4; ++j) {
                uint32_t key;
                if (key_of(k, j, key) && (key & pmask) == prefix) {
                    const unsigned long long w = w_of(k, j);
                    if (w) atomicAdd(&sh.hist[wave][(key >> shift) & 255u], w);
                }
            }
        __syncthreads();
        if (tid < 256) {
            unsigned long long s = 0;
            for (int w = 0; w < SMP_WAVES; ++w) s += sh.hist[w][tid];
            sh.bin[tid] = s;
        }
        __syncthreads();
        if (shift == shift_hi) {
            unsigned long long total = 0;
            for (int i = 0; i < 256; ++i) total += sh.bin[i];
            thr = thr_of(total);
            if (thr >= total) { __syncthreads(); return false; }
        }
        if (wave == 0) {
            unsigned long long v[4], tot = 0;
#pragma unroll
            for (int s = 0; s < 4; ++s) { v[s] = sh.bin[255 - 4 * lane - s]; tot += v[s]; }
            unsigned long long inc = tot;
#pragma unroll
            for (int off = 1; off < 64; off <<= 1) {
                const unsigned long long o = __shfl_up(inc, off, 64);
                if (lane >= off) inc += o;
            }
            unsigned long long run = above + (inc - tot);
#pragma unroll
            for (int s = 0; s < 4; ++s) {
                if (run <= thr && thr < run + v[s]) { sh.digit = 255u - 4u * lane - s; sh.above = run; sh.mass = v[s]; }
                run += v[s];
            }
        }
        __syncthreads();
        prefix |= sh.digit << shift;
        pmask |= 255u << shift;
// ... 57 lines not shown
    uint32_t kstar = 0;
    int idx_cut = 0x7fffffff;
    if (!keep_all) {
        unsigned long long above, mass, thr;
        keep_all = !radix_select([&](int k, int j, uint32_t& key) { key = okey(opaque(z[k][j])); return true; }, q_of,
                                 [&](unsigned long long S) { return top_p > 0.0f ? (unsigned long long)((double)top_p * (double)S) : 0ull; },
                                 24, sh, kstar, above, mass, thr);
        if (!keep_all) {
#pragma unroll
            for (int k = 0; k < SMP_NV4; ++k)
#pragma unroll
                for (int j = 0; j < 4; ++j)
                    if (okey(opaque(z[k][j])) == kstar) qtie_s = (uint32_t)q_of(k, j);
            __syncthreads();
            const unsigned long long qt = qtie_s;
            const unsigned long long n_tie = mass / qt, c = (thr - above) / qt + 1;
            if (c < n_tie) {
                uint32_t kidx;
                unsigned long long a2, m2, t2;
                radix_select([&](int k, int j, uint32_t& key) {
                                 key = 0xFFFFu - (uint32_t)(4 * (k * SMP_THREADS + tid) + j);
                                 return okey(opaque(z[k][j])) == kstar; },
                             [](int, int) { return 1ull; }, [c](unsigned long long) { return c - 1; }, 8, sh, kidx, a2, m2, t2);
                idx_cut = (int)(0xFFFFu - kidx);
            }
        }
    }

    float best = -INFINITY;
    int bidx = 0x7fffffff;
#pragma unroll
    for (int k = 0; k < SMP_NV4; ++k) {
        const int i4 = k * SMP_THREADS + tid;
        bool kept[4], any = false;
#pragma unroll
        for (int j = 0; j < 4; ++j) {
            const uint32_t key = okey(opaque(z[k][j]));
            kept[j] = (keep_all || key > kstar || (key == kstar && 4 * i4 + j <= idx_cut));
            any |= kept[j];
        }
        if (any) {
            uint32_t x[4];
            philox4x32_10((uint32_t)i4, step, grow, 0u, seed_lo, seed_hi, x);
#pragma unroll
            for (int j = 0; j < 4; ++j)
                if (kept[j]) {
                    const float u = (float)(2u * (x[j] >> 9) + 1u) * 0x1p-24f;
                    const float s = z[k][j] - logf(-logf(u));
                    const int id = 4 * i4 + j;
                    if (s > best || (s == best && id < bidx)) { best = s; bidx = id; }
                }
        }
    }
#pragma unroll
    for (int off = 32; off > 0; off >>= 1) {
        const float ob = __shfl_xor(best, off, 64);
        const int oi = __shfl_xor(bidx, off, 64);
        if (ob > best || (ob == best && oi < bidx)) { best = ob; bidx = oi; }
    }
    if ((tid & 63) == 0) { red_f[tid >> 6] = best; red_i[tid >> 6] = bidx; }
    __syncthreads();
    best = red_f[0]; bidx = red_i[0];
    for (int w = 1; w < SMP_WAVES; ++w)
        if (red_f[w] > best || (red_f[w] == best && red_i[w] < bidx)) { best = red_f[w]; bidx = red_i[w]; }
    __syncthreads();
    return min(max(bidx, 0), SAMPLE_MAX_V - 1);
}

}

template <bool LSE>
__global__ __launch_bounds__(SMP_THREADS) void dec_sample_kernel(const SampleArgs sa, const DecArgs a, int32_t* __restrict__ tokens,
                                                                 const float* __restrict__ embed, int write_x, const LoopArgs lp) {
    __shared__ int tok_s;
    __shared__ float lse_sh[4];
    const int b = blockIdx.x, tid = threadIdx.x;
    const int row = lp.row_of_slot ? lp.row_of_slot[b] : b;
    const bool dead = (lp.blk_snap && lp.blk_snap[b >> 5] == 0) || row < 0;
    int idx = 0;
    if (!dead) {
        const int step = lp.out_tokens ? *a.d_pos - lp.T0 + 1 : (int)sa.prm[SMP_STEP];
        idx = sample_row(sa.logits + (int64_t)b * sa.ld, sa.prm, sa.prm[SMP_ROW_OFF] + ((uint32_t)row >> sa.row_shift), (uint32_t)step);
    }
    float lse = 0.f;
    if constexpr (LSE) {
        if (!dead) {
            const int n = (int)(sa.ld >> 5);
            const float M = dec_lse_max(a.cand_val + (int64_t)b * n, n, lse_sh);
            lse = dec_lse_value(M, dec_lse_sum(a.cand_val + (int64_t)b * n, a.cand_sum + (int64_t)b * n, n, M, lse_sh));
        }
    }
    if (tid == 0) {
        if (!dead) {
            tokens[b] = idx;
            tok_s = idx;
        }
        if (lp.out_tokens) {
            if (!dead) {
                const int max_len = lp.params[0], stop_id = lp.params[1];
                const int step = *a.d_pos - lp.T0 + 1;
                if (step >= 0 && step < max_len) lp.out_tokens[(int64_t)row * max_len + step] = idx;
                if constexpr (LSE) {
                    if (step >= 0 && step < max_len) lp.out_logprob[(int64_t)row * max_len + step] = sa.logits[(int64_t)b * sa.ld + idx] - lse;
                }
                if (idx == stop_id && lp.seen_stop[row] == 0) {
                    lp.seen_stop[row] = 1;
                    atomicAdd(lp.n_seen, 1);
                    if (lp.blk_left && atomicSub(lp.blk_left + (b >> 5), 1) == 1) lp.blk_live[b >> 5] = 0;
                }
            }
            asm volatile("s_waitcnt vmcnt(0)" ::: "memory");
            if (atomicAdd(lp.arrive, 1) == (int)gridDim.x - 1) {
                *lp.arrive = 0;
                const int t = *lp.ticket + 1;
                *lp.ticket = t;
                const int ns = atomicAdd(lp.n_seen, 0);
                __hip_atomic_store(lp.host_progress, ((unsigned long long)(unsigned)t << 32) | (unsigned)ns, __ATOMIC_RELAXED,
                                   __HIP_MEMORY_SCOPE_SYSTEM);
            }
        }
    }
    if (dead) return;
    if (write_x) {
        __syncthreads();
        if (tid < 144) {
            const float4 e = reinterpret_cast<const float4*>(embed + (int64_t)tok_s * 576)[tid];
            reinterpret_cast<float4*>(a.xmidF)[f32_idx(b >> 5, 72, b & 31, tid * 4)] = e;
        }
    }
}

__global__ __launch_bounds__(SMP_THREADS) void sample_logits_kernel(const SampleArgs sa, int32_t* __restrict__ tokens) {
    const int b = blockIdx.x;
    const uint32_t grow = sa.prm[SMP_ROW_OFF] + (uint32_t)(sa.row_ids ? sa.row_ids[b] : b);
    const int idx = sample_row(sa.logits + (int64_t)b * sa.ld, sa.prm, grow, sa.prm[SMP_STEP]);
    if (threadIdx.x == 0) tokens[b] = idx;
}

void launch_dec_sample(const SampleArgs& sa, const DecArgs& a, int B, int32_t* tokens, const float* embed, int write_x,
                       const LoopArgs& loop, hipStream_t s) {
    if (loop.out_logprob != nullptr && a.cand_sum != nullptr)
        hipLaunchKernelGGL(dec_sample_kernel<true>, dim3(B), dim3(SMP_THREADS), 0, s, sa, a, tokens, embed, write_x, loop);
    else
        hipLaunchKernelGGL(dec_sample_kernel<false>, dim3(B), dim3(SMP_THREADS), 0, s, sa, a, tokens, embed, write_x, loop);
}

void launch_sample_logits(const SampleArgs& sa, int B, int32_t* tokens, hipStream_t s) {
    hipLaunchKernelGGL(sample_logits_kernel, dim3(B), dim3(SMP_THREADS), 0, s, sa, tokens);
}

}
```

Baseline: 459.0.

## Precompute layer-0 q/k/v per token id and skip decode's first qkv launch

At load time the layer-0 q/k/v projection and the RMS sum of squares are computed for every vocabulary token and stored in a table. The sampling and beam kernels then gather the table row straight into the pq/ssq1 buffers, stage the next RoPE row and advance d_pos. Layer 0's attention can then run in a table form without a dec_qkv GEMM launch. The cost is a large extra device allocation and longer load time, in exchange for one fewer launch and GEMM per decode step. The option defaults to on and is described as bit-identical.

```diff
diff --git a/mellow_amd/csrc/beam.hip b/mellow_amd/csrc/beam.hip
--- a/mellow_amd/csrc/beam.hip
+++ b/mellow_amd/csrc/beam.hip
@@ -1,5 +1,6 @@
 #include "common.h"
 #include "kernels.h"
+#include "dec_token.h"
 
 namespace mellow {
 
@@ -10,9 +11,6 @@
 static_assert(BM_NV4 * 4 * BM_THREADS == SAMPLE_MAX_V, "row tiling");
 static_assert(BEAM_MAX_K * BEAM_MAX_K <= 64, "one wave ranks an example's survivors");
 
-__device__ __forceinline__ int64_t f32_idx(int rb, int K8, int m, int k) {
-    return ((int64_t)rb * K8 + (k >> 3)) * 64 + m + 32 * ((k >> 2) & 1);
-}
 
 __device__ __forceinline__ uint32_t ckey(float c) {
     if (c != c) return 0xFFFFFFFFu;
@@ -134,7 +132,9 @@
         return;
     } else {
         const int max_len = lp.params[0], stop_id = lp.params[1];
-        const int step = *a.d_pos - lp.T0 + 1;
+        const int pos = *a.d_pos;
+        const int step = pos - lp.T0 + 1;
+        if (a.tok_tab && b == 0 && lane < 32) dec_stage_next_rope(a, lane);
         int fin = 0;
         if (lane < k) {
             const int row = b * k + lane;
@@ -158,14 +158,12 @@
                 const int ns = atomicExch(lp.n_seen, 0);
                 __hip_atomic_store(lp.host_progress, ((unsigned long long)(unsigned)t << 32) | (unsigned)ns, __ATOMIC_RELAXED,
                                    __HIP_MEMORY_SCOPE_SYSTEM);
+                if (a.tok_tab) *a.d_pos = pos + 1;
             }
         }
         for (int j = 0; j < k; ++j) {
             const int row = b * k + j, t = min(max(sel_tok[j], 0), SAMPLE_MAX_V - 1);
-            for (int i = lane; i < 144; i += 64) {
-                const float4 e = reinterpret_cast<const float4*>(embed + (int64_t)t * 576)[i];
-                reinterpret_cast<float4*>(a.xmidF)[f32_idx(row >> 5, 72, row & 31, i * 4)] = e;
-            }
+            dec_token_gather(a, embed, row, t, lane, 64);
         }
     }
 }
@@ -174,8 +172,8 @@
 __global__ __launch_bounds__(256) void beam_kv_move_kernel(float4* __restrict__ kpages, float4* __restrict__ vpages, float4* __restrict__ kst,
                                                            float4* __restrict__ vst, const int32_t* __restrict__ parent_tab,
                                                            const int32_t* __restrict__ d_pos, const int32_t* __restrict__ params, int T0,
-                                                           int layers, int N, int k, int Bp, int Tmax) {
-    const int max_len = params[0], step = *d_pos - T0 + 1;
+                                                           int layers, int N, int k, int Bp, int Tmax, int pos_adv) {
+    const int max_len = params[0], step = *d_pos - pos_adv - T0 + 1;
     if (step <= 0 || step >= max_len || T0 + step > Tmax) return;
     const int64_t c16 = (int64_t)step * 16, ML16 = (int64_t)max_len * 16, Tmax16 = (int64_t)Tmax * 16;
     const int64_t total = (int64_t)layers * N * 3 * c16;
@@ -209,13 +207,13 @@
 }
 
 void launch_beam_reorder(float* k_pages, float* v_pages, float* k_stage, float* v_stage, const int32_t* parent_tab, const int32_t* d_pos,
-                         const int32_t* params, int T0, int layers, int N, int k, int Bp, int Tmax, hipStream_t s) {
+                         const int32_t* params, int T0, int layers, int N, int k, int Bp, int Tmax, int pos_adv, hipStream_t s) {
     if (layers <= 0 || N <= 0 || k < 2 || N % k != 0 || N > Bp) return;
     constexpr int blocks = 1024;
     hipLaunchKernelGGL(beam_kv_move_kernel<true>, dim3(blocks), dim3(256), 0, s, reinterpret_cast<float4*>(k_pages), reinterpret_cast<float4*>(v_pages),
-                       reinterpret_cast<float4*>(k_stage), reinterpret_cast<float4*>(v_stage), parent_tab, d_pos, params, T0, layers, N, k, Bp, Tmax);
+                       reinterpret_cast<float4*>(k_stage), reinterpret_cast<float4*>(v_stage), parent_tab, d_pos, params, T0, layers, N, k, Bp, Tmax, pos_adv);
     hipLaunchKernelGGL(beam_kv_move_kernel<false>, dim3(blocks), dim3(256), 0, s, reinterpret_cast<float4*>(k_pages), reinterpret_cast<float4*>(v_pages),
-                       reinterpret_cast<float4*>(k_stage), reinterpret_cast<float4*>(v_stage), parent_tab, d_pos, params, T0, layers, N, k, Bp, Tmax);
-}
-
-}
+                       reinterpret_cast<float4*>(k_stage), reinterpret_cast<float4*>(v_stage), parent_tab, d_pos, params, T0, layers, N, k, Bp, Tmax, pos_adv);
+}
+
+}
diff --git a/mellow_amd/csrc/build.py b/mellow_amd/csrc/build.py
--- a/mellow_amd/csrc/build.py
+++ b/mellow_amd/csrc/build.py
@@ -13,7 +13,7 @@
 OBJDIR = os.path.join(HERE, "build")
 LIB = os.path.join(LIBDIR, "libmellow_hip.so")
 SOURCES = ["gemm_f32.hip", "gemm_fp8.hip", "gemm_bf16x3.hip", "decode.hip", "prefill_attn.hip", "encoder.hip", "stft_fft.hip", "sample.hip", "score.hip", "beam.hip", "logit_rules.hip", "guidance.hip", "engine.cpp", "engine_weights.cpp", "engine_encoder.cpp", "engine_lm.cpp", "engine_generate.cpp", "engine_dev.cpp"]
-HEADERS = ["common.h", "kernels.h", "gemm_epilogue.h", "prefill_attn_f32.inc", "engine_internal.h", os.path.join("..", "..", "include", "mellow_hip.h")]
+HEADERS = ["common.h", "kernels.h", "dec_token.h", "gemm_epilogue.h", "prefill_attn_f32.inc", "engine_internal.h", os.path.join("..", "..", "include", "mellow_hip.h")]
 ARCH = "gfx950"
 FLAGS = (["-DMELLOW_KDEBUG"] if os.environ.get("MELLOW_KDEBUG") else []) + os.environ.get("MELLOW_EXTRA_FLAGS", "").split() + ["-O3", "-std=c++17", "-fPIC", "-fvisibility=hidden", f"--offload-arch={ARCH}", "-Wall", "-Wno-unused-function",
          "-Wno-unused-variable", "-x", "hip"]
diff --git a/mellow_amd/csrc/dec_token.h b/mellow_amd/csrc/dec_token.h
--- /dev/null
+++ b/mellow_amd/csrc/dec_token.h
@@ -0,0 +1,28 @@
+#pragma once
+#include "kernels.h"
+
+namespace mellow {
+
+__device__ __forceinline__ void dec_token_gather(const DecArgs& a, const float* __restrict__ embed, int slot, int tok, int i0, int stride) {
+    const float4* erow = reinterpret_cast<const float4*>(embed + (int64_t)tok * 576);
+    const int64_t fbase = ((int64_t)(slot >> 5) * 72) * 64 + (slot & 31);
+    for (int i = i0; i < 144; i += stride) {
+        const float4 e = erow[i];
+        reinterpret_cast<float4*>(a.xmidF)[fbase + (i >> 1) * 64 + 32 * (i & 1)] = e;
+        if (a.tok_tab) reinterpret_cast<float4*>(a.xnewR + (int64_t)slot * 576)[i] = e;
+    }
+    if (a.tok_tab) {
+        const float4* trow = reinterpret_cast<const float4*>(a.tok_tab + (int64_t)tok * 960);
+        for (int i = i0; i < 240; i += stride) reinterpret_cast<float4*>(a.pq + (int64_t)slot * 960)[i] = trow[i];
+        if (i0 == 0) a.ssq1[(int64_t)slot * DEC_KC_QKV] = a.tok_ssq[tok];
+    }
+}
+
+__device__ __forceinline__ void dec_stage_next_rope(const DecArgs& a, int lane32) {
+    const int p = min(*a.d_pos + 1, a.Tmax - 1);
+    const float c = a.rope_cos[(int64_t)p * 32 + lane32], sn = a.rope_sin[(int64_t)p * 32 + lane32];
+    a.rope_cur[lane32] = c;
+    a.rope_cur[32 + lane32] = sn;
+}
+
+}
diff --git a/mellow_amd/csrc/decode.hip b/mellow_amd/csrc/decode.hip
--- a/mellow_amd/csrc/decode.hip
+++ b/mellow_amd/csrc/decode.hip
@@ -1,5 +1,6 @@
 #include "common.h"
 #include "kernels.h"
+#include "dec_token.h"
 #include <cstdio>
 #include <mutex>
 #include <set>
@@ -315,7 +316,7 @@
     if constexpr (KV16) reinterpret_cast<__bf16*>(page)[elem] = static_cast<__bf16>(v);
     else page[elem] = v;
 }
-template <bool BLK, bool FUSED, bool ONE, bool KV16, int NW, int TS>
+template <bool BLK, bool FUSED, bool ONE, bool KV16, int NW, int TS, bool TAB = false>
 __global__ __launch_bounds__(NW * 64, ONE ? 2 : (KV16 && MELLOW_DA16_MFMA && DA_MINW > 1 ? MELLOW_DA16_MINW : DA_MINW)) void dec_attn_kernel(float* __restrict__ k_cache, float* __restrict__ v_cache,
                                                                   const int32_t* __restrict__ d_pos_p, const float* __restrict__ pq_p,
                                                                   const float* __restrict__ xmidF_p, int Tmax_p, int gs_p, int rows_p,
@@ -360,13 +361,17 @@
     const int r = tid < 80 ? tid : 0;
     const int pcol = r < 48 ? (3 * g + (r >> 4)) * 64 + 4 * (r & 15) : r < 64 ? 576 + g * 64 + 4 * (r - 48) : 768 + g * 64 + 4 * (r - 64);
     const float* prow = pq_p + (int64_t)b * 960 + pcol;
-    constexpr int NPQ = FUSED ? Q2_NPQ : DEC_KC_QKV;
+    static_assert(!(TAB && FUSED), "the table row stands in for dec_qkv_kernel's slabs");
+    constexpr int NPQ = FUSED ? Q2_NPQ : TAB ? 1 : DEC_KC_QKV;
     float4 sl4[NPQ], sq4[2];
+    float sq1 = 0.f;
     if (tid < 80) {
 #pragma unroll
         for (int s = 0; s < NPQ; ++s)
             sl4[s] = (MELLOW_DA_ABL & 4) ? make_float4(0.1f * s, 0.2f, 0.3f, 0.4f) : *reinterpret_cast<const float4*>(prow + (int64_t)s * rows_p * 960);
-        if (!FUSED) {
+        if (TAB) {
+            sq1 = a.ssq1[(int64_t)b * DEC_KC_QKV];
+        } else if (!FUSED) {
             sq4[0] = reinterpret_cast<const float4*>(a.ssq1 + (int64_t)b * DEC_KC_QKV)[0];
             sq4[1] = reinterpret_cast<const float4*>(a.ssq1 + (int64_t)b * DEC_KC_QKV)[1];
         }
@@ -446,8 +451,8 @@
     } else if (tid < 80) {
         float4 x = sl4[0];
 #pragma unroll
-        for (int s = 1; s < DEC_KC_QKV; ++s) x = f4add(x, sl4[s]);
-        const float ssum = ((sq4[0].x + sq4[0].y) + (sq4[0].z + sq4[0].w)) + ((sq4[1].x + sq4[1].y) + (sq4[1].z + sq4[1].w));
+        for (int s = 1; s < NPQ; ++s) x = f4add(x, sl4[s]);
+        const float ssum = TAB ? sq1 : ((sq4[0].x + sq4[0].y) + (sq4[0].z + sq4[0].w)) + ((sq4[1].x + sq4[1].y) + (sq4[1].z + sq4[1].w));
         const float rscale = 1.0f / sqrtf(ssum / 576.0f + a.eps);
         *reinterpret_cast<float4*>(xs + 4 * tid) = make_float4(x.x * rscale, x.y * rscale, x.z * rscale, x.w * rscale);
     }
@@ -1725,6 +1730,7 @@
     const int b = blockIdx.x, tid = threadIdx.x;
     const int row = lp.row_of_slot ? lp.row_of_slot[b] : b;
     const bool dead = (lp.blk_snap && lp.blk_snap[b >> 5] == 0) || row < 0;
+    if (lp.out_tokens && a.tok_tab && b == 0 && tid < 32) dec_stage_next_rope(a, tid);
     float best = -INFINITY;
     int idx = 0x7fffffff;
     if (!dead) {
@@ -1762,9 +1768,10 @@
             tok_s = idx;
         }
         if (lp.out_tokens) {
+            const int pos = *a.d_pos;
             if (!dead) {
                 const int max_len = lp.params[0], stop_id = lp.params[1];
-                const int step = *a.d_pos - lp.T0 + 1;
+                const int step = pos - lp.T0 + 1;
                 if (step >= 0 && step < max_len) lp.out_tokens[(int64_t)row * max_len + step] = idx;
                 if constexpr (LSE) {
                     if (step >= 0 && step < max_len) lp.out_logprob[(int64_t)row * max_len + step] = -dec_lse_log(S);
@@ -1783,16 +1790,14 @@
                 const int ns = atomicAdd(lp.n_seen, 0);
                 __hip_atomic_store(lp.host_progress, ((unsigned long long)(unsigned)t << 32) | (unsigned)ns, __ATOMIC_RELAXED,
                                    __HIP_MEMORY_SCOPE_SYSTEM);
+                if (a.tok_tab) *a.d_pos = pos + 1;
             }
         }
     }
     if (dead) return;
     if (write_x) {
         __syncthreads();
-        if (tid < 144) {
-            const float4 e = reinterpret_cast<const float4*>(embed + (int64_t)tok_s * 576)[tid];
-            reinterpret_cast<float4*>(a.xmidF)[f32_idx(b >> 5, 72, b & 31, tid * 4)] = e;
-        }
+        dec_token_gather(a, embed, b, tok_s, tid, 256);
     }
     kspan(a.dbg_seq, 1);
 }
@@ -1913,6 +1918,33 @@
     }
 }
 
+__global__ __launch_bounds__(256) void dec_load_tokens_kernel(const DecArgs a, const float* __restrict__ embed, const int32_t* __restrict__ ids,
+                                                              int vocab) {
+    const int b = blockIdx.x, tid = threadIdx.x;
+    if (b == 0 && tid < 32) {
+        const int p = *a.d_pos + 1;
+        dec_stage_next_rope(a, tid);
+        if (tid == 0) *a.d_pos = p;
+    }
+    dec_token_gather(a, embed, b, min(max(ids[b], 0), vocab - 1), tid, 256);
+}
+__global__ __launch_bounds__(256) void tok_table_reduce_kernel(const float* __restrict__ pq, const float* __restrict__ ssq1, int rows_p, int rows,
+                                                               float* __restrict__ tab, float* __restrict__ tab_ssq) {
+    static_assert(DEC_KC_QKV == 8, "fixed summation order below");
+    const int r = blockIdx.x, tid = threadIdx.x;
+    if (r >= rows) return;
+    if (tid < 240) {
+        float4 x = reinterpret_cast<const float4*>(pq + (int64_t)r * 960)[tid];
+#pragma unroll
+        for (int s = 1; s < DEC_KC_QKV; ++s) x = f4add(x, reinterpret_cast<const float4*>(pq + ((int64_t)s * rows_p + r) * 960)[tid]);
+        reinterpret_cast<float4*>(tab + (int64_t)r * 960)[tid] = x;
+    }
+    if (tid == 0) {
+        const float4 s0 = reinterpret_cast<const float4*>(ssq1 + (int64_t)r * DEC_KC_QKV)[0], s1 = reinterpret_cast<const float4*>(ssq1 + (int64_t)r * DEC_KC_QKV)[1];
+        tab_ssq[r] = ((s0.x + s0.y) + (s0.z + s0.w)) + ((s1.x + s1.y) + (s1.z + s1.w));
+    }
+}
+
 void set_max_dynamic_lds(const void* fn, size_t bytes) {
     if (bytes <= 64 * 1024) return;
     static std::mutex mu;
@@ -1944,18 +1976,29 @@
                            (const float*)a.dslabF, K8p, a, wscale);
     }); }); });
 }
-void launch_dec_attn(const DecArgs& a, float* k_cache, float* v_cache, bool fused, hipStream_t s) {
+void launch_dec_attn(const DecArgs& a, float* k_cache, float* v_cache, bool fused, hipStream_t s, bool tab) {
     const dim3 grid(3, a.rows, a.ts);
     const bool one = a.RB == 1 && !a.blk_live;
     if (a.ts != DEC_TS && (one || a.kv16 || a.ts != DEC_TS_MULTI)) {
         fprintf(stderr, "mellow: decode attention launched with %d key splits at RB = %d\n", a.ts, a.RB);
         abort();
     }
+    if (tab && (fused || a.kv16)) {
+        fprintf(stderr, "mellow: decode attention asked for the token-table form with fused = %d, kv16 = %d\n", (int)fused, a.kv16);
+        abort();
+    }
     auto launch = [&](auto blk, auto one_c) { with_bool(fused, [&](auto fused_c) { with_bool(a.kv16 != 0, [&](auto kv16) {
         constexpr bool ONE = one_c.value, KV16 = kv16.value;
         constexpr int NW = !KV16 ? DA_WAVES : MELLOW_DA16_MFMA && DA_WAVES == 8 && !ONE ? MELLOW_DA16_NW : DA_WAVES;
         constexpr int TSM = ONE || KV16 ? DEC_TS : DEC_TS_MULTI;
         with_int<DEC_TS, TSM>(a.ts, [&](auto ts) {
+            if constexpr (!fused_c.value && !KV16) {
+                if (tab) {
+                    hipLaunchKernelGGL((dec_attn_kernel<blk.value, false, ONE, false, NW, ts.value, true>), grid, dim3(NW * 64), 0, s, k_cache, v_cache,
+                                       (const int32_t*)a.d_pos, (const float*)a.pq, (const float*)a.xmidF, a.Tmax, a.gs, a.rows, a);
+                    return;
+                }
+            }
             hipLaunchKernelGGL((dec_attn_kernel<blk.value, fused_c.value, ONE, KV16, NW, ts.value>), grid, dim3(NW * 64), 0, s, k_cache, v_cache,
                                (const int32_t*)a.d_pos, (const float*)a.pq, (const float*)a.xmidF, a.Tmax, a.gs, a.rows, a);
         });
@@ -2132,6 +2175,12 @@
 void launch_dec_lse_tap(const DecArgs& a, int B, int n_tiles, float* out_lse, float* out_max, hipStream_t s) {
     hipLaunchKernelGGL(dec_lse_tap_kernel, dim3(B), dim3(256), 0, s, (const float*)a.cand_val, (const float*)a.cand_sum, n_tiles, out_lse, out_max);
 }
+void launch_dec_load_tokens(const DecArgs& a, int B, const float* embed, const int32_t* ids, int vocab, hipStream_t s) {
+    hipLaunchKernelGGL(dec_load_tokens_kernel, dim3(B), dim3(256), 0, s, a, embed, ids, vocab);
+}
+void launch_tok_table_reduce(const DecArgs& a, int rows, float* tab, float* tab_ssq, hipStream_t s) {
+    hipLaunchKernelGGL(tok_table_reduce_kernel, dim3(rows), dim3(256), 0, s, (const float*)a.pq, (const float*)a.ssq1, a.rows, rows, tab, tab_ssq);
+}
 void launch_dec_load_rows(const DecArgs& a, int B, const float* in, int64_t ld, const int32_t* row_ids, int T_last,
                           int n_src, hipStream_t s) {
     hipLaunchKernelGGL(dec_load_rows_kernel, dim3(B), dim3(192), 0, s, a, in, ld, row_ids, T_last, n_src);
diff --git a/mellow_amd/csrc/engine.cpp b/mellow_amd/csrc/engine.cpp
--- a/mellow_amd/csrc/engine.cpp
+++ b/mellow_amd/csrc/engine.cpp
@@ -354,6 +354,7 @@
     {"prefill_fuse_norm", "1", true, "f32x3: norm-free LM prefill (GEMM epilogues emit split output + RMS partials); 0 = a normalisation launch per GEMM input"},
     {"decode_fuse", "1", true, "down projection of layer l fused with q/k/v of layer l + 1 through the load-time product W'Wd; 0 = five launches per layer"},
     {"decode_fuse_max_rb", "1", true, "largest number of 32-row blocks that runs the fused down + q/k/v launch on fp32 weights"},
+    {"dec_token_table", "1", false, "f32 / f32x3: layer 0's q/k/v row and sum of squares per token id formed at load time by the step's own kernel (189 MB), so a decode step has no dec_qkv launch; bit-identical; no effect in fp8 mode"},
     {"splitk", "8", true, "f32x3 encoder: largest split count of the split-K launches (0 = never split; a summation order)"},
     {"enc_apb", "0x1CC", false, "f32x3 encoder: Swin stages whose producers hand over pre-split (bit st, 4 + st, 8 + st); bit-identical"},
     {"graph", "1", false, "decode steps as hipGraph replays (0 = eager launches)"},
@@ -387,6 +388,7 @@
     e->opt.prefill_fuse_norm = opt_val(e, "prefill_fuse_norm") != 0;
     e->opt.decode_fuse = opt_val(e, "decode_fuse") != 0;
     e->opt.dec_fuse_max_rb = (int)opt_val(e, "decode_fuse_max_rb");
+    e->opt.dec_token_table = opt_val(e, "dec_token_table") != 0 && mode != MELLOW_PRECISION_FP8;
     e->opt.sk_max = (int)opt_val(e, "splitk");
     e->opt.enc_apb_stages = (int)opt_val(e, "enc_apb");
     e->use_graph = opt_val(e, "graph") != 0;
@@ -433,6 +435,8 @@
     s += e->finalized ? "true" : "false";
     s += ", \"stft_is_fft\": ";
     s += e->w.fft_win ? "true" : "false";
+    s += ", \"dec_token_table_in_use\": ";
+    s += e->w.tok_tab ? "true" : "false";
     s += ", \"non_default\": [";
     bool first = true;
     for (const auto& o : kOptions)
diff --git a/mellow_amd/csrc/engine_internal.h b/mellow_amd/csrc/engine_internal.h
--- a/mellow_amd/csrc/engine_internal.h
+++ b/mellow_amd/csrc/engine_internal.h
@@ -157,6 +157,7 @@
         int enc_apb_stages = 0x1CC;
         int sk_max = 8;
         int dec_fuse_max_rb = 1;
+        bool dec_token_table = true;
     };
     struct Fp8W { uint8_t* w8; float* scale; };
     struct LOCAL Weights {
@@ -177,13 +178,14 @@
         float* final_norm = nullptr;
         float *rope_cos = nullptr, *rope_sin = nullptr;
         float *head8 = nullptr, *head_sc = nullptr;
+        float *tok_tab = nullptr, *tok_ssq = nullptr;
         DecW head_w() const { return head8 ? DecW{head8, head_sc} : DecW{lm_head.p, nullptr}; }
         std::unordered_map<const float*, void*> bf_w;
         std::unordered_map<const float*, Fp8W> fp8_w;
     };
     struct LOCAL StepGraphs {
         struct Key {
-            std::array<uintptr_t, 18> v{};
+            std::array<uintptr_t, 19> v{};
             static Key of(const mellow_engine* e, int B);
             bool operator==(const Key& k) const { return v == k.v; }
         };
@@ -265,6 +267,7 @@
     StepGraphs graphs;
 
     bool taps_on = false;
+    bool tap_l0 = false;
     std::map<std::string, Buf> taps;
     std::map<std::string, int64_t> tap_numel;
 
@@ -300,7 +303,8 @@
                 (uintptr_t)e->mode.rules,
                 (uintptr_t)(e->mode.rules ? e->rules_bias.p : nullptr),
                 (uintptr_t)(e->mode.rules && e->mode.beam ? e->rules_hist.p : nullptr),
-                (uintptr_t)e->mode.guide}};
+                (uintptr_t)e->mode.guide,
+                (uintptr_t)e->da.tok_tab}};
 }
 static_assert(!std::is_copy_constructible<mellow_engine::Buf>::value, "a Buf owns its device memory: it moves, it is never copied");
 static_assert(std::is_copy_assignable<mellow_engine::Weights>::value && std::is_copy_assignable<mellow_engine::Options>::value, "a fork copies these by assignment: no owning member (Buf, StepGraphs) belongs in them");
diff --git a/mellow_amd/csrc/engine_lm.cpp b/mellow_amd/csrc/engine_lm.cpp
--- a/mellow_amd/csrc/engine_lm.cpp
+++ b/mellow_amd/csrc/engine_lm.cpp
@@ -95,6 +95,9 @@
     a.blk_live = m.early_exit ? e->d_blk_live : nullptr;
     a.blk_snap = e->d_blk_live + 32;
     a.row_of_slot = m.migrate ? e->d_row_of_slot : nullptr;
+    const bool tab = e->w.tok_tab != nullptr && !m.migrate && !e->opt.kv16;
+    a.tok_tab = tab ? e->w.tok_tab : nullptr;
+    a.tok_ssq = tab ? e->w.tok_ssq : nullptr;
 }
 
 int clear_page_tails(mellow_engine* e, int T, int t_end) {
@@ -385,12 +388,17 @@
         a.dbg_seq = sq;
         a.first = l == l_begin ? 1 : 0;
         a.inc_pos = (inc_pos && l == l_begin) ? 1 : 0;
-        if (!(skip & 1) && !fused_in)
+        const bool tab_in = l == 0 && l == l_begin && inc_pos && e->da.tok_tab != nullptr && !same_w;
+        if (!(skip & 1) && !fused_in && !tab_in)
         { ProfScope ps(e, PF_SKINNY, 2.0 * Bp * 576.0 * 960.0, 576.0 * 960.0 * 4);
           launch_dec_qkv(a, qkv.p, w.qkv_f.KP / 8, kcd, s, qkv.scale); }
+        if (l == 0 && e->tap_l0) {
+            CHK(tap(e, "dec_l0_pq", e->da.pq, (int64_t)DEC_KC_QKV * Bp * 960));
+            CHK(tap(e, "dec_l0_ssq", e->da.ssq1, (int64_t)Bp * DEC_KC_QKV));
+        }
         if (!(skip & 2))
         { ProfScope ps(e, PF_DECODE_ATTN, 4.0 * 64 * 9 * (double)B * (e->cur_pos + 1), 2.0 * (double)B * 3 * 64 * 4 * (e->cur_pos + 1));
-          launch_dec_attn(da(1), kc, vc, fused_in, s); }
+          launch_dec_attn(da(1), kc, vc, fused_in, s, tab_in); }
         if (!(skip & 4))
         { ProfScope ps(e, PF_SKINNY, 2.0 * Bp * 576.0 * 576.0, 576.0 * 576.0 * 4);
           launch_dec_oproj(da(2), o.p, s, o.scale); }
@@ -417,7 +425,7 @@
     if (e->mode.beam > 1) {
         ProfScope ps(e, PF_MISC, 0, 0);
         launch_beam_reorder(e->kcache.p, e->vcache.p, e->kstage.p, e->vstage.p, beam_args(e, B, e->mode.beam).out_parent, e->d_pos, e->d_params,
-                            e->cfg.prefix_len, e->cfg.num_layers, B, e->mode.beam, e->kv_B, e->kv_Tmax, e->stream);
+                            e->cfg.prefix_len, e->cfg.num_layers, B, e->mode.beam, e->kv_B, e->kv_Tmax, e->da.tok_tab ? 1 : 0, e->stream);
     }
     return 0;
 }
@@ -523,8 +531,12 @@
     if (e->cur_pos + 1 > e->kv_Tmax) return fail("KV pages exhausted (reserve too small)");
     HIPCHK(hipSetDevice(e->device));
     const int B = e->cur_B;
-    launch_dec_load_rows(e->da, B, e->w.embed, 576, token_ids, 0, e->cfg.vocab_size, e->stream);
-    CHK(enqueue_decode_layers(e, B, nullptr));
+    if (e->da.tok_tab) launch_dec_load_tokens(e->da, B, e->w.embed, token_ids, e->cfg.vocab_size, e->stream);
+    else launch_dec_load_rows(e->da, B, e->w.embed, 576, token_ids, 0, e->cfg.vocab_size, e->stream);
+    e->tap_l0 = true;
+    const int rc_step = enqueue_decode_layers(e, B, nullptr);
+    e->tap_l0 = false;
+    CHK(rc_step);
     e->cur_pos += 1;
     if (logits)
         HIPCHK(hipMemcpyAsync(logits, e->dlogits.p, (size_t)B * e->cfg.vocab_size * 4, hipMemcpyDeviceToDevice, e->stream));
diff --git a/mellow_amd/csrc/engine_weights.cpp b/mellow_amd/csrc/engine_weights.cpp
--- a/mellow_amd/csrc/engine_weights.cpp
+++ b/mellow_amd/csrc/engine_weights.cpp
@@ -109,6 +109,44 @@
     const HostTensor* t = get(e, k);
     CHK(expect_shape(t, k, {N, K}));
     return make_packed(e, t->f(), nullptr, N, K, out);
+}
+
+static int build_token_table(mellow_engine* e) {
+    const int V = e->cfg.vocab_size;
+    if (!e->opt.dec_token_table || e->opt.fp8 || e->cfg.hidden_size != 576 || V % 32 != 0 || e->w.layers.empty()) return 0;
+    const LMLayerW& w0 = e->w.layers[0];
+    if (!w0.qkv_f.p || w0.qkv8) return 0;
+    constexpr int RB = 32, R = RB * 32;
+    const size_t o_xmid = 0, o_xnew = (size_t)R * 576, o_ssq = 2 * (size_t)R * 576, o_pq = o_ssq + (size_t)R * DEC_KC_QKV;
+    const size_t ws_floats = o_pq + (size_t)DEC_KC_QKV * R * 960;
+    void *tab = nullptr, *ssq = nullptr, *ws = nullptr;
+    if (hipMalloc(&tab, (size_t)V * 960 * sizeof(float)) != hipSuccess || hipMalloc(&ssq, (size_t)V * sizeof(float)) != hipSuccess ||
+        hipMalloc(&ws, ws_floats * sizeof(float)) != hipSuccess) {
+        (void)hipGetLastError();
+        if (tab) (void)hipFree(tab);
+        if (ssq) (void)hipFree(ssq);
+        if (ws) (void)hipFree(ws);
+        return 0;
+    }
+    e->allocs.push_back(tab);
+    e->allocs.push_back(ssq);
+    struct Scratch { void* p; ~Scratch() { (void)hipFree(p); } } scratch{ws};
+    float* p = reinterpret_cast<float*>(ws);
+    DecArgs a;
+    a.rows = R; a.eps = e->cfg.rms_norm_eps; a.dbg_seq = -1000;
+    a.xmidF = p + o_xmid; a.xnewR = p + o_xnew; a.dslabF = p + o_xmid; a.ssq1 = p + o_ssq; a.pq = p + o_pq;
+    for (int r0 = 0; r0 < V; r0 += R) {
+        const int n = V - r0 < R ? V - r0 : R;
+        a.RB = n / 32;
+        launch_dec_load_rows(a, n, e->w.embed + (size_t)r0 * 576, 576, nullptr, 1, 0, e->stream);
+        launch_dec_qkv(a, w0.qkv_f.p, w0.qkv_f.KP / 8, 0, e->stream);
+        launch_tok_table_reduce(a, n, reinterpret_cast<float*>(tab) + (size_t)r0 * 960, reinterpret_cast<float*>(ssq) + r0, e->stream);
+    }
+    HIPCHK(hipGetLastError());
+    HIPCHK(hipStreamSynchronize(e->stream));
+    e->w.tok_tab = reinterpret_cast<float*>(tab);
+    e->w.tok_ssq = reinterpret_cast<float*>(ssq);
+    return 0;
 }
 
 extern "C" int mellow_engine_finalize(mellow_engine_t* e) {
@@ -374,6 +412,7 @@
         CHK(upload(e, &e->w.rope_cos, c.data(), c.size()));
         CHK(upload(e, &e->w.rope_sin, s.data(), s.size()));
     }
+    CHK(build_token_table(e));
     CHK(alloc_state_words(e));
     e->host.clear();
     e->finalized = true;
diff --git a/mellow_amd/csrc/kernels.h b/mellow_amd/csrc/kernels.h
--- a/mellow_amd/csrc/kernels.h
+++ b/mellow_amd/csrc/kernels.h
@@ -144,10 +144,14 @@
     float* logits = nullptr;
     float* cand_val = nullptr; int32_t* cand_idx = nullptr;
     float* cand_sum = nullptr;
+    const float* tok_tab = nullptr;
+    const float* tok_ssq = nullptr;
 };
 void launch_dec_qkv(const DecArgs& a, const float* Wp_folded, int K8p, int kcd, hipStream_t s, const float* wscale = nullptr);
 void launch_pack_dec_fp8(const float* Wp, int tiles, int slots_per_tile, int rows_per_tile, void* out, float* scale, hipStream_t s);
-void launch_dec_attn(const DecArgs& a, float* k_cache, float* v_cache, bool fused, hipStream_t s);
+void launch_dec_attn(const DecArgs& a, float* k_cache, float* v_cache, bool fused, hipStream_t s, bool tab = false);
+void launch_tok_table_reduce(const DecArgs& a, int rows, float* tab, float* tab_ssq, hipStream_t s);
+void launch_dec_load_tokens(const DecArgs& a, int B, const float* embed, const int32_t* ids, int vocab, hipStream_t s);
 void launch_kv_to_bf16(const float* src, void* dst, int64_t n, hipStream_t s);
 void launch_kv_fanout(const float* k_prefix, const float* v_prefix, float* k_pages, float* v_pages, int layers, int B, int n, int Bp,
                       int T, int Tp, int Tmax, hipStream_t s);
@@ -211,7 +215,7 @@
 };
 void launch_beam_select(const BeamArgs& g, int B, const DecArgs& a, int32_t* tokens, const float* embed, const LoopArgs* loop, hipStream_t s);
 void launch_beam_reorder(float* k_pages, float* v_pages, float* k_stage, float* v_stage, const int32_t* parent_tab, const int32_t* d_pos,
-                         const int32_t* params, int T0, int layers, int N, int k, int Bp, int Tmax, hipStream_t s);
+                         const int32_t* params, int T0, int layers, int N, int k, int Bp, int Tmax, int pos_adv, hipStream_t s);
 enum { RUL_THETA = 0, RUL_NGRAM, RUL_MIN_NEW, RUL_BIAS_ON, RUL_STOP, RUL_WORDS = 8 };
 constexpr int RULES_MAX_HIST = 8192;
 struct RulesArgs {
diff --git a/mellow_amd/csrc/sample.hip b/mellow_amd/csrc/sample.hip
--- a/mellow_amd/csrc/sample.hip
+++ b/mellow_amd/csrc/sample.hip
@@ -1,5 +1,6 @@
 #include "common.h"
 #include "kernels.h"
+#include "dec_token.h"
 
 namespace mellow {
 
@@ -9,9 +10,6 @@
 constexpr int SMP_NV4 = SAMPLE_MAX_V / 4 / SMP_THREADS;
 static_assert(SMP_NV4 * 4 * SMP_THREADS == SAMPLE_MAX_V, "row tiling");
 
-__device__ __forceinline__ int64_t f32_idx(int rb, int K8, int m, int k) {
-    return ((int64_t)rb * K8 + (k >> 3)) * 64 + m + 32 * ((k >> 2) & 1);
-}
 
 __device__ __forceinline__ uint32_t okey(float z) {
     const uint32_t u = __float_as_uint(z);
@@ -235,6 +233,7 @@
         const int step = lp.out_tokens ? *a.d_pos - lp.T0 + 1 : (int)sa.prm[SMP_STEP];
         idx = sample_row(sa.logits + (int64_t)b * sa.ld, sa.prm, sa.prm[SMP_ROW_OFF] + ((uint32_t)row >> sa.row_shift), (uint32_t)step);
     }
+    if (lp.out_tokens && a.tok_tab && b == 0 && tid < 32) dec_stage_next_rope(a, tid);
     float lse = 0.f;
     if constexpr (LSE) {
         if (!dead) {
@@ -249,9 +248,10 @@
             tok_s = idx;
         }
         if (lp.out_tokens) {
+            const int pos = *a.d_pos;
             if (!dead) {
                 const int max_len = lp.params[0], stop_id = lp.params[1];
-                const int step = *a.d_pos - lp.T0 + 1;
+                const int step = pos - lp.T0 + 1;
                 if (step >= 0 && step < max_len) lp.out_tokens[(int64_t)row * max_len + step] = idx;
                 if constexpr (LSE) {
                     if (step >= 0 && step < max_len) lp.out_logprob[(int64_t)row * max_len + step] = sa.logits[(int64_t)b * sa.ld + idx] - lse;
@@ -270,16 +270,14 @@
                 const int ns = atomicAdd(lp.n_seen, 0);
                 __hip_atomic_store(lp.host_progress, ((unsigned long long)(unsigned)t << 32) | (unsigned)ns, __ATOMIC_RELAXED,
                                    __HIP_MEMORY_SCOPE_SYSTEM);
+                if (a.tok_tab) *a.d_pos = pos + 1;
             }
         }
     }
     if (dead) return;
     if (write_x) {
         __syncthreads();
-        if (tid < 144) {
-            const float4 e = reinterpret_cast<const float4*>(embed + (int64_t)tok_s * 576)[tid];
-            reinterpret_cast<float4*>(a.xmidF)[f32_idx(b >> 5, 72, b & 31, tid * 4)] = e;
-        }
+        if (tid < 256) dec_token_gather(a, embed, b, tok_s, tid, 256);
     }
 }
 
```

New measurement: 460.1 (median of 3 runs). About the same (+0.3%).
